# keep-starknet-strange/frieda

Hardware: AMD Instinct MI355X
Metric: M31 field-elems/s committed (NTT+FRI+Merkle) (higher is better)
Workload: dtype u32

## Files before the change

### frieda_amd/csrc/codec.hip

```cpp
#include <hip/hip_runtime.h>

#include <cstdlib>

#include "kernels.h"

namespace frieda {
namespace k {

namespace {

__device__ __forceinline__ uint32_t load_dword_guarded(const uint8_t* in, size_t len, size_t d) {
    size_t b = d * 4;
    if (b + 4 <= len) return *reinterpret_cast<const uint32_t*>(in + b);
    uint32_t v = 0;
    for (int i = 0; i < 4; i++)
        if (b + i < len) v |= (uint32_t)in[b + i] << (8 * i);
    return v;
}

template <int O>
__device__ __forceinline__ uint4 extract4(const uint32_t (&w)[5]) {
    uint32_t f[4];
#pragma unroll
    for (int j = 0; j < 4; j++) {
        const int pos = O + 30 * j, q = pos >> 5, r = pos & 31;
        uint64_t pair = ((uint64_t)w[q + 1] << 32) | w[q];
        f[j] = (uint32_t)(pair >> r) & 0x3fffffffu;
    }
    return make_uint4(f[0], f[1], f[2], f[3]);
}

template <int T>
__global__ __launch_bounds__(256) void unpack30_aligned_kernel(const uint8_t* __restrict__ in, size_t len,
                                                               uint32_t* __restrict__ out, size_t n_quads, size_t in_bstride,
                                                               size_t out_bstride) {
    in += blockIdx.y * in_bstride;
    out = reinterpret_cast<uint32_t*>(reinterpret_cast<char*>(out) + blockIdx.y * out_bstride);
    constexpr uint32_t DW = 960u * T;
    __shared__ __attribute__((aligned(16))) uint32_t stage[DW + 4];
    const size_t d_base = (size_t)blockIdx.x * DW;
    if ((reinterpret_cast<uintptr_t>(in) & 15) == 0 && (d_base + DW + 4) * 4 <= len) {
        const uint4* src = reinterpret_cast<const uint4*>(in + 4 * d_base);
#pragma unroll
        for (uint32_t u = threadIdx.x; u < 240u * T; u += 256) reinterpret_cast<uint4*>(stage)[u] = src[u];
        if (threadIdx.x < 4) stage[DW + threadIdx.x] = reinterpret_cast<const uint32_t*>(in)[d_base + DW + threadIdx.x];
    } else {
        for (uint32_t i = threadIdx.x; i < DW + 4; i += 256) stage[i] = load_dword_guarded(in, len, d_base + i);
    }
    __syncthreads();
#pragma unroll
    for (int i = 0; i < T; i++) {
        const uint32_t local = (uint32_t)i * 256u + threadIdx.x;
        const size_t t = (size_t)blockIdx.x * (256u * T) + local;
        if (t >= n_quads) return;
        const uint32_t byte0 = 15u * local;
        const uint32_t d0 = byte0 >> 2;
        uint32_t w[5];
#pragma unroll
        for (int j = 0; j < 5; j++) w[j] = stage[d0 + j];
        uint4 v;
        switch (byte0 & 3) {
            case 0: v = extract4<0>(w); break;
            case 1: v = extract4<8>(w); break;
            case 2: v = extract4<16>(w); break;
            default: v = extract4<24>(w); break;
        }
        reinterpret_cast<uint4*>(out)[t] = v;
    }
}

__global__ __launch_bounds__(256) void unpack30_bytes_kernel(const uint8_t* __restrict__ in, size_t len,
                                                             uint32_t* __restrict__ out, size_t n_out, size_t in_bstride,
                                                             size_t out_bstride) {
    in += blockIdx.y * in_bstride;
    out = reinterpret_cast<uint32_t*>(reinterpret_cast<char*>(out) + blockIdx.y * out_bstride);
    size_t kf = (size_t)blockIdx.x * blockDim.x + threadIdx.x;
    if (kf >= n_out) return;
    size_t bit0 = 30 * kf, byte0 = bit0 >> 3;
    uint32_t sh = (uint32_t)(bit0 & 7);
    uint64_t acc = 0;
    for (int i = 0; i < 5; i++)
        if (byte0 + i < len) acc |= (uint64_t)in[byte0 + i] << (8 * i);
    out[kf] = (uint32_t)(acc >> sh) & 0x3fffffffu;
}

}

void unpack30(const Launch& L, const uint8_t* d_bytes, size_t len, uint32_t* d_out, size_t n_out, size_t src_bstride) {
    if (n_out == 0) return;
    hipStream_t s = L.stream;
    Scope scope(L, "unpack30", (double)len + 4.0 * (double)n_out);
    bool aligned = ((reinterpret_cast<uintptr_t>(d_bytes) & 3) == 0) && ((reinterpret_cast<uintptr_t>(d_out) & 15) == 0) &&
                   (n_out % 4 == 0) && (src_bstride % 4 == 0) && (L.bstride % 16 == 0);
    if (aligned) {
        size_t quads = n_out / 4;
        const int tiles = (int)L.tune->unpack_tiles;
        const int T = quads >= 8192 ? tiles : 1;
        dim3 grid((unsigned)((quads + 256 * (size_t)T - 1) / (256 * (size_t)T)), L.batch);
        if (T == 8)
            unpack30_aligned_kernel<8><<<grid, 256, 0, s>>>(d_bytes, len, d_out, quads, src_bstride, L.bstride);
        else if (T == 4)
            unpack30_aligned_kernel<4><<<grid, 256, 0, s>>>(d_bytes, len, d_out, quads, src_bstride, L.bstride);
        else if (T == 2)
            unpack30_aligned_kernel<2><<<grid, 256, 0, s>>>(d_bytes, len, d_out, quads, src_bstride, L.bstride);
        else
            unpack30_aligned_kernel<1><<<grid, 256, 0, s>>>(d_bytes, len, d_out, quads, src_bstride, L.bstride);
    } else {
        dim3 grid((unsigned)((n_out + 255) / 256), L.batch);
        unpack30_bytes_kernel<<<grid, 256, 0, s>>>(d_bytes, len, d_out, n_out, src_bstride, L.bstride);
    }
}

}
}
```

### frieda_amd/csrc/context.cpp

```cpp
#include <cstring>
#include <cstdlib>
#include <string.h>

#include <cstdio>

#include <algorithm>
#include <mutex>

#include "host.h"

extern char** environ;

namespace frieda {

static constexpr uint32_t IDX_MASK = 0x7fffffffu;

CPoint point_from_index(uint32_t index) {
    static const std::array<CPoint, 31> pow2 = [] {
        std::array<CPoint, 31> t{};
        CPoint cur{CIRCLE_GEN_X, CIRCLE_GEN_Y};
        for (auto& e : t) {
            e = cur;
            cur = cp_double(cur);
        }
        return t;
    }();
    CPoint res{1, 0};
    index &= IDX_MASK;
    for (uint32_t b = 0; index; b++, index >>= 1)
        if (index & 1u) res = cp_add(res, pow2[b]);
    return res;
}

Coset Coset::half_odds(uint32_t log_size) {
    Coset c;
    c.initial = 1u << (31 - (log_size + 2));
    c.step = log_size == 0 ? 0u : (1u << (31 - log_size));
    c.log_size = log_size;
    return c;
}
Coset Coset::doubled() const { return Coset{(initial * 2u) & IDX_MASK, (step * 2u) & IDX_MASK, log_size - 1}; }
uint32_t Coset::index_at(uint32_t i) const { return (initial + (uint32_t)((uint64_t)step * i)) & IDX_MASK; }
CPoint Coset::at(uint32_t i) const { return point_from_index(index_at(i)); }

Coset line_coset(uint32_t n, uint32_t m) {
    Coset c = Coset::half_odds(n - 1);
    while (c.log_size > m) c = c.doubled();
    return c;
}

CodecShape codec_shape(size_t len) {
    CodecShape s;
    s.n_felts = (8 * len + 29) / 30;
    uint32_t e = 2;
    while (((size_t)1 << e) < s.n_felts) e++;
    s.n_padded = (size_t)1 << e;
    s.log_size = e - 2;
    return s;
}

struct KernelTimerImpl {
    struct Span {
        const char* name;
        double alg_bytes;
        hipEvent_t start, stop;
    };
    std::vector<Span> spans;
    std::vector<hipEvent_t> pool;
    size_t used = 0;
    hipEvent_t next() {
        if (used == pool.size()) {
            hipEvent_t e;
            (void)hipEventCreate(&e);
            pool.push_back(e);
        }
        return pool[used++];
    }
    ~KernelTimerImpl() {
        for (auto e : pool) (void)hipEventDestroy(e);
    }
};

namespace k {
void timer_begin(KernelTimer* t, hipStream_t s, const char* name, double alg_bytes) {
    auto* ti = reinterpret_cast<KernelTimerImpl*>(t);
    KernelTimerImpl::Span sp{name, alg_bytes, ti->next(), ti->next()};
    (void)hipEventRecord(sp.start, s);
    ti->spans.push_back(sp);
}
void timer_end(KernelTimer* t, hipStream_t s) {
    auto* ti = reinterpret_cast<KernelTimerImpl*>(t);
    (void)hipEventRecord(ti->spans.back().stop, s);
}
}

k::Launch Ctx::launch() const {
    k::Launch l{stream, reinterpret_cast<k::KernelTimer*>(timer)};
    l.tune = &tuning;
    return l;
}

namespace k {
namespace {
struct KnobDesc {
    const char* name;
    long lo, hi;
    bool (*set)(Tuning&, long);
};
const KnobDesc KNOBS[] = {
    {"FRIEDA_T5_WIDE_LOG", 16, 24, [](Tuning& t, long v) { t.t5_wide_log = (uint32_t)v; return true; }},
    {"FRIEDA_T5_REG3_LOG", 0, 30, [](Tuning& t, long v) { t.t5_reg3_log = (uint32_t)v; return true; }},
    {"FRIEDA_T9_MAX_LOG", 8, 19, [](Tuning& t, long v) { t.t9_max_log = (uint32_t)v; return true; }},
    {"FRIEDA_TOP_MAX_LOG", 9, 11, [](Tuning& t, long v) { t.top_max_log = (uint32_t)v; return true; }},
    {"FRIEDA_NTT_CPW", 1, 4, [](Tuning& t, long v) {
         if (v == 4 && !t.lds_opt_in_ok) return false;
         t.ntt_cpw = (uint32_t)v;
         return true;
     }},
    {"FRIEDA_NTT_CPW_SMALL", 1, 4, [](Tuning& t, long v) { t.ntt_cpw_small = (uint32_t)v; return true; }},
    {"FRIEDA_NTT_REP", 0, 2, [](Tuning& t, long v) { t.ntt_rep = (uint32_t)v; return true; }},
    {"FRIEDA_NTT_NO_CP", 0, 1, [](Tuning& t, long v) { t.ntt_no_cp = v != 0; return true; }},
    {"FRIEDA_NTT_NO_PAD8", 0, 1, [](Tuning& t, long v) { t.ntt_no_pad8 = v != 0; return true; }},
    {"FRIEDA_NTT_TREE_REG_ONLY", 0, 1, [](Tuning& t, long v) { t.ntt_tree_reg_only = v != 0; return true; }},
    {"FRIEDA_NO_ENCODE_TREE_FUSION", 0, 1, [](Tuning& t, long v) { t.no_encode_tree_fusion = v != 0; return true; }},
    {"FRIEDA_ENCODE_TREE_FUSION_PROVE", 0, 1, [](Tuning& t, long v) { t.encode_tree_fusion_prove = v != 0; return true; }},
    {"FRIEDA_NO_SMALL_FUSED", 0, 1, [](Tuning& t, long v) { t.no_small_fused = v != 0; return true; }},
    {"FRIEDA_UNPACK_TILES", 1, 8, [](Tuning& t, long v) {
         if (v != 1 && v != 2 && v != 4 && v != 8) return false;
         t.unpack_tiles = (uint32_t)v;
         return true;
     }},
    {"FRIEDA_INTT_GENERIC", 0, 1, [](Tuning& t, long v) { t.intt_generic = v != 0; return true; }},
    {"FRIEDA_ERASURE_TREE_MIN_LOG", 6, 32, [](Tuning& t, long v) { t.erasure_tree_min_log = (uint32_t)v; return true; }},
    {"FRIEDA_TAIL_RUN_LOG", 4, 11, [](Tuning& t, long v) { t.tail_run_log = (uint32_t)v; return true; }},
    {"FRIEDA_HOST_DECOMMIT", 0, 1, [](Tuning& t, long v) { t.host_decommit = v != 0; return true; }},
    {"FRIEDA_GATHER_COPY", 0, 1, [](Tuning& t, long v) { t.gather_copy = v != 0; return true; }},
    {"FRIEDA_VERIFY_DEVICE_MIN", 0, 2147483648L, [](Tuning& t, long v) { t.verify_device_min = (uint32_t)v; return true; }},
    {"FRIEDA_OPEN_SMALL_MAX", 0, 512, [](Tuning& t, long v) { t.open_small_max = (uint32_t)v; return true; }},
    {"FRIEDA_TREE_SKIP_LOG", 10, 40, [](Tuning& t, long v) { t.tree_skip_log = (uint32_t)v; return true; }},
    {"FRIEDA_TREE_SKIP_LONE_LOG", 10, 40, [](Tuning& t, long v) { t.tree_skip_lone_log = (uint32_t)v; return true; }},
    {"FRIEDA_SEEDS_FOLD_GROUP", 0, 64, [](Tuning& t, long v) { t.seeds_fold_group = (uint32_t)v; return true; }},
    {"FRIEDA_TP_MIN_WGS", 0, 1 << 30, [](Tuning& t, long v) { t.tp_min_wgs = (uint32_t)v; return true; }},
    {"FRIEDA_GRIND_ITERS", 0, 64, [](Tuning& t, long v) { t.grind_iters = (uint32_t)v; return true; }},
    {"FRIEDA_BATCH_BUDGET_MB", 0, 262144, [](Tuning& t, long v) { t.batch_budget_mb = (uint32_t)v; return true; }},
    {"FRIEDA_BATCH_CALLS_PER_CTX", 1, 64, [](Tuning& t, long v) { t.batch_calls_per_ctx = (uint32_t)v; return true; }},
};
}

bool tuning_set(Tuning& t, const char* name, long value) {
    if (!name) return false;
    for (const KnobDesc& k : KNOBS) {
        if (strcmp(k.name, name) == 0) {
            if (value < k.lo || value > k.hi) return false;
            return k.set(t, value);
        }
    }
    return false;
}

static const char* const PROCESS_VARS[] = {"FRIEDA_HIP_LIB", "FRIEDA_RCCL_PATH", "FRIEDA_MULTI_FORCE_RCCL", "FRIEDA_MULTI_NO_PREFETCH",
                                           "FRIEDA_MULTI_NO_NUMA_PIN", "FRIEDA_BENCH_FORCE_DIST", "FRIEDA_BENCH_CPU_THREADS", "FRIEDA_TEST_"};
static void warn_unknown_env_once() {
    static std::once_flag once;
    std::call_once(once, [] {
        for (char** e = ::environ; e && *e; e++) {
            if (strncmp(*e, "FRIEDA_", 7) != 0) continue;
            const char* eq = strchr(*e, '=');
            const size_t len = eq ? (size_t)(eq - *e) : strlen(*e);
            bool known = false;
            for (const KnobDesc& k : KNOBS) known = known || (strlen(k.name) == len && strncmp(k.name, *e, len) == 0);
            for (const char* pv : PROCESS_VARS) known = known || strncmp(pv, *e, strlen(pv)) == 0;
            if (!known) fprintf(stderr, "libfrieda_hip: note: environment variable %.*s is not an option of this library (ignored)\n", (int)len, *e);
        }
    });
}

Tuning tuning_from_env() {
    Tuning t;
    warn_unknown_env_once();
    for (const KnobDesc& k : KNOBS) {
        const char* e = getenv(k.name);
        if (!e) continue;
        char* end = nullptr;
        long v = strtol(e, &end, 10);
        if (end == e) v = 1;
        (void)tuning_set(t, k.name, v);
    }
    return t;
}

const Tuning& tuning_defaults() {
    static const Tuning d;
    return d;
}
}

int Ctx::set_kernel_timing(bool enabled) {
    if (enabled && !timer) timer = new KernelTimerImpl();
    if (!enabled && timer) {
        (void)hipStreamSynchronize(stream);
        delete timer;
        timer = nullptr;
    }
    return FRIEDA_OK;
}

std::string Ctx::kernel_timing_report(bool reset) {
    std::string out = "{\"kernels\": [";
    if (timer) {
        (void)hipStreamSynchronize(stream);
        struct Agg {
            const char* name;
            size_t launches;
            double ms, bytes;
        };
        std::vector<Agg> agg;
        for (auto& sp : timer->spans) {
            float ms = 0.f;
            if (hipEventElapsedTime(&ms, sp.start, sp.stop) != hipSuccess) continue;
            Agg* a = nullptr;
            for (auto& x : agg)
                if (strcmp(x.name, sp.name) == 0) a = &x;
            if (!a) {
                agg.push_back(Agg{sp.name, 0, 0.0, 0.0});
                a = &agg.back();
            }
            a->launches++;
            a->ms += ms;
            a->bytes += sp.alg_bytes;
        }
        bool first = true;
        for (auto& a : agg) {
            char buf[256];
            snprintf(buf, sizeof buf, "%s{\"name\": \"%s\", \"launches\": %zu, \"total_ms\": %.6f, \"alg_bytes\": %.1f}", first ? "" : ", ",
                     a.name, a.launches, a.ms, a.bytes);
            out += buf;
            first = false;
        }
        if (reset) {
            timer->spans.clear();
            timer->used = 0;
        }
    }
    out += "]}";
    return out;
}

int Ctx::fail(int code, const std::string& what) {
    err = what;
    return code;
}
int Ctx::hip_fail(hipError_t e, const char* what) {
    err = std::string(what) + ": " + hipGetErrorString(e);
    return FRIEDA_ERR_HIP;
}

int Ctx::ensure_arena(size_t bytes) {
    if (tuning.test_arena_limit && bytes > tuning.test_arena_limit) {
        err = "workspace of " + std::to_string(bytes) + " B refused by the test limit";
        return FRIEDA_ERR_NOMEM;
    }
    if (bytes <= arena_bytes) return FRIEDA_OK;
    if (arena) {
        FR_HIP(this, hipStreamSynchronize(stream));
        FR_HIP(this, hipFree(arena));
        arena = nullptr;
        arena_bytes = 0;
    }
    size_t want = (bytes + ((size_t)1 << 20) - 1) & ~(((size_t)1 << 20) - 1);
    hipError_t e = hipMalloc((void**)&arena, want);
    if (e != hipSuccess) {
        err = std::string("hipMalloc(workspace ") + std::to_string(want) + " B): " + hipGetErrorString(e);
        return FRIEDA_ERR_NOMEM;
    }
    arena_bytes = want;
    return FRIEDA_OK;
}

void Ctx::drop_twiddles() {
    for (auto& kv : twiddles) {
        if (kv.second.d_tw) (void)hipFree(kv.second.d_tw);
        if (kv.second.d_itw) (void)hipFree(kv.second.d_itw);
        if (kv.second.d_scratch) (void)hipFree(kv.second.d_scratch);
    }
    twiddles.clear();
}

int Ctx::get_twiddles(uint32_t n, TwiddleSet& out) {
    auto it = twiddles.find(n);
    if (it != twiddles.end() && cache_twiddles) {
        out = it->second;
        return FRIEDA_OK;
    }
    TwiddleSet ts;
    if (it != twiddles.end()) {
        ts = it->second;
    } else {
        size_t bytes = sizeof(uint32_t) << (n - 1);
        hipError_t e = hipMalloc((void**)&ts.d_tw, bytes);
        if (e == hipSuccess) e = hipMalloc((void**)&ts.d_itw, bytes);
        if (e == hipSuccess) e = hipMalloc((void**)&ts.d_scratch, 8192);
        if (e != hipSuccess) {
            if (ts.d_tw) (void)hipFree(ts.d_tw);
            if (ts.d_itw) (void)hipFree(ts.d_itw);
            err = std::string("hipMalloc(twiddles, 2 x ") + std::to_string(bytes) + " B): " + hipGetErrorString(e);
            return FRIEDA_ERR_NOMEM;
        }
        twiddles[n] = ts;
    }
    Coset h = Coset::half_odds(n - 1);
    k::TwiddleSeeds seeds;
    memset(&seeds, 0, sizeof seeds);
    seeds.p0 = point_from_index(h.initial);
    if (n >= 3) {
        CPoint sp = point_from_index(h.step);
        for (uint32_t b = 0; b + 2 < n; b++) {
            seeds.step[b] = sp;
            sp = cp_double(sp);
        }
    }
    ts.ds.init_x = seeds.p0.x;
    ts.ds.init_y = seeds.p0.y;
    ts.ds.inv_init_x = m31_inv(seeds.p0.x);
    ts.ds.inv_init_y = m31_inv(seeds.p0.y);
    k::gen_twiddles(launch(), n, seeds, ts.d_tw, ts.d_itw, ts.d_scratch);
    if (const hipError_t e = hipGetLastError(); e != hipSuccess) {
        (void)hipStreamSynchronize(stream);
        (void)hipFree(ts.d_tw);
        (void)hipFree(ts.d_itw);
        (void)hipFree(ts.d_scratch);
        twiddles.erase(n);
        return hip_fail(e, "gen_twiddles");
    }
    twiddles[n] = ts;
    out = ts;
    return FRIEDA_OK;
}

Ctx::~Ctx() {
    (void)hipSetDevice(device);
    if (stream) (void)hipStreamSynchronize(stream);
    drop_twiddles();
    delete timer;
    if (arena) (void)hipFree(arena);
    if (pinned) (void)hipHostFree(pinned);
    if (pinned_in) (void)hipHostFree(pinned_in);
    if (own_stream && stream) (void)hipStreamDestroy(stream);
}

}
```

### frieda_amd/csrc/kernels.h

```cpp
#pragma once
#include <hip/hip_runtime.h>
#include <stddef.h>
#include <stdint.h>

#include "field.h"

namespace frieda {
namespace k {

inline size_t tw_level_offset(uint32_t n, uint32_t lv) { return ((size_t)1 << (n - 1)) - ((size_t)1 << (n - 1 - lv)); }
__device__ __forceinline__ size_t tw_level_offset_dev(uint32_t n, uint32_t lv) {
    return ((size_t)1 << (n - 1)) - ((size_t)1 << (n - 1 - lv));
}

struct KernelTimer;
struct Tuning {
    uint32_t t5_wide_log = 18;
    uint32_t t5_reg3_log = 0;
    uint32_t t9_max_log = 17;
    uint32_t top_max_log = 9;
    uint32_t ntt_cpw = 4;
    uint32_t ntt_cpw_small = 1;
    uint32_t ntt_rep = 2;
    bool ntt_no_pad8 = false;
    bool ntt_no_cp = false;
    bool ntt_tree_reg_only = false;
    bool no_encode_tree_fusion = false;
    bool encode_tree_fusion_prove = false;
    bool no_small_fused = false;
    uint32_t unpack_tiles = 4;
    bool intt_generic = false;
    uint32_t erasure_tree_min_log = 15;
    uint32_t tail_run_log = 9;
    bool host_decommit = false;
    bool gather_copy = false;
    uint32_t verify_device_min = 1;
    uint32_t open_small_max = 512;
    uint32_t test_grind_first_log = 0;
    uint32_t batch_budget_mb = 0;
    uint32_t tree_skip_log = 18;
    uint32_t tree_skip_lone_log = 23;
    uint32_t tp_min_wgs = 768;
    uint32_t grind_iters = 0;
    uint32_t seeds_fold_group = 0;
    uint32_t batch_calls_per_ctx = 1;
    uint64_t device_mem_bytes = 0;
    bool lds_opt_in_ok = true;
    uint64_t test_arena_limit = 0;
};
inline uint32_t tree_skip_threshold(const Tuning& t, uint32_t batch) {
    return batch >= 2 ? t.tree_skip_log : (t.tree_skip_lone_log > t.tree_skip_log ? t.tree_skip_lone_log : t.tree_skip_log);
}
Tuning tuning_from_env();
bool tuning_set(Tuning& t, const char* name, long value);
const Tuning& tuning_defaults();

struct Launch {
    hipStream_t stream;
    KernelTimer* timer;
    uint32_t batch = 1;
    size_t bstride = 0;
    const Tuning* tune = &tuning_defaults();
};
void timer_begin(KernelTimer* t, hipStream_t s, const char* name, double alg_bytes);
void timer_end(KernelTimer* t, hipStream_t s);
struct Scope {
    const Launch& l;
    Scope(const Launch& l_, const char* name, double alg_bytes) : l(l_) {
        if (l.timer) timer_begin(l.timer, l.stream, name, alg_bytes * l.batch);
    }
    ~Scope() {
        if (l.timer) timer_end(l.timer, l.stream);
    }
};

struct DomainScalars {
    uint32_t init_x, init_y;
    uint32_t inv_init_x, inv_init_y;
};

void unpack30(const Launch& L, const uint8_t* d_bytes, size_t len, uint32_t* d_out, size_t n_out, size_t src_bstride = 0);

int blake2s_ceiling(hipStream_t s, uint32_t* d_scratch, double* leaf_per_s, double* node_per_s, double* clock = nullptr);
size_t blake2s_ceiling_scratch_bytes();

void bit_reverse_columns(const Launch& L, uint32_t* d_cols, size_t stride, uint32_t ncols, uint32_t log_size);

struct TwiddleSeeds {
    CPoint p0;
    CPoint step[32];
};
void gen_twiddles(const Launch& L, uint32_t n, const TwiddleSeeds& seeds, uint32_t* d_tw, uint32_t* d_itw, void* d_scratch8k);

void circle_evaluate(const Launch& L_, const uint32_t* d_coef, size_t coef_stride, uint32_t ncols, uint32_t L, uint32_t n,
                     const uint32_t* d_tw, DomainScalars ds, uint32_t* d_out, size_t out_stride);
void circle_evaluate_prefix(const Launch& L_, const uint32_t* d_coef, size_t coef_stride, uint32_t ncols, uint32_t L, uint32_t n, uint32_t out_log,
                            const uint32_t* d_tw, DomainScalars ds, uint32_t* d_out, size_t out_stride);

struct EncodeTreeSink {
    uint8_t* layers;
    uint8_t* last_out;
};
constexpr uint32_t ENCODE_TREE_LEVELS = 7;
hipError_t ntt_opt_in_dynamic_lds();
struct EncodeFoldSink {
    const uint32_t* itw;
    uint32_t alpha0[4], alpha1[4];
    bool accumulate;
    uint32_t* line1;
    uint32_t* line2;
};
bool circle_evaluate_fold2(const Launch& L_, const uint32_t* d_coef, size_t coef_stride, uint32_t L, uint32_t n, const uint32_t* d_tw,
                           DomainScalars ds, uint32_t* d_out, size_t out_stride, const EncodeFoldSink& fs, hipError_t* err);
uint32_t circle_evaluate_into_tree(const Launch& L_, const uint32_t* d_coef, size_t coef_stride, uint32_t ncols, uint32_t L, uint32_t n,
                               const uint32_t* d_tw, DomainScalars ds, uint32_t* d_out, size_t out_stride, const EncodeTreeSink* sink);

void circle_interpolate_block(const Launch& L_, const uint32_t* d_block, size_t in_stride, uint32_t ncols, uint32_t L, uint32_t n,
                              uint32_t block, const uint32_t* d_itw, DomainScalars ds, uint32_t* d_coef, size_t out_stride);
void cells_combine(const Launch& L_, const uint32_t* d_w, const uint32_t* d_vinv, uint32_t R, uint32_t ncols, uint32_t m, uint32_t* d_coef,
                   size_t coef_stride, size_t vinv_pitch = 0);
size_t cells_inverse_scratch_bytes(uint32_t R);
uint32_t* cells_inverse_index_buffer(uint8_t* d_scratch, uint32_t R);
void cells_matrix_inverse_device(const Launch& L_, const uint32_t* d_cell_index, uint32_t R, uint32_t j_bits, uint32_t m, uint32_t n,
                                 const uint32_t* d_tw, uint8_t* d_scratch, const uint32_t** d_vinv_out, size_t* pitch_out,
                                 const uint32_t** d_state_out);
void pack30(const Launch& L_, const uint32_t* d_felts, size_t n_felts, uint8_t* d_out, size_t len);

struct ErasureDomain {
    CPoint init;
    CPoint step_pow[32];
    uint32_t n;
};
void erasure_points(const Launch& L_, const ErasureDomain& g, const uint32_t* d_pos, uint32_t count, uint32_t* d_px, uint32_t* d_py);
void erasure_lines(const Launch& L_, const ErasureDomain& g, const uint32_t* d_pos, uint32_t n_lines, uint32_t* d_la, uint32_t* d_lb,
                   uint32_t* d_lc);
size_t erasure_zpart_chunks(uint32_t count, uint32_t n_lines);
void erasure_zeval(const Launch& L_, const uint32_t* d_px, const uint32_t* d_py, uint32_t count, const uint32_t* d_la, const uint32_t* d_lb,
                   const uint32_t* d_lc, uint32_t n_lines, bool own, uint32_t* d_zpart, uint32_t* d_z);
void erasure_known_weights(const Launch& L_, const uint32_t* d_px, const uint32_t* d_py, uint32_t count, uint32_t n, uint32_t* d_z);
void erasure_cellconst(const Launch& L_, const ErasureDomain& g, const uint32_t* d_cell_pos, uint32_t n_cells, uint32_t m, uint32_t* d_kc);
void erasure_zeval_cells(const Launch& L_, const uint32_t* d_px, uint32_t count, uint32_t m, const uint32_t* d_kc, uint32_t n_cells, bool own,
                         uint32_t* d_zpart, uint32_t* d_z);
void erasure_known_weights_cells(const Launch& L_, const uint32_t* d_px, uint32_t count, uint32_t n, uint32_t m, uint32_t* d_z);
size_t erasure_sample_lists_chunks(uint32_t n_cells);
hipError_t erasure_sample_lists(const Launch& L_, const uint32_t* d_idx, uint32_t n_cells, uint32_t domain_cells, uint32_t ncols, uint32_t log_cell,
                          uint32_t* d_owner, uint32_t* d_chunk_sum, uint32_t* d_chunk_off, uint32_t* d_first_cell, uint32_t* d_first_row,
                          uint32_t* d_state, uint32_t* d_pos, uint32_t* d_src);
void erasure_cell_firsts(const Launch& L_, const uint32_t* d_pos, uint32_t n_cells, uint32_t log_cell, uint32_t* d_out);
void erasure_lines32(const Launch& L_, const uint32_t* d_px128, const uint32_t* d_py128, const uint32_t* d_la, const uint32_t* d_lb, const uint32_t* d_lc,
                     uint32_t n_lines, uint32_t nodes, uint32_t* d_out);
void erasure_pairmul(const Launch& L_, const uint32_t* d_ext, uint32_t n_nodes, uint32_t size, uint32_t* d_out);
void erasure_ze(const Launch& L_, const ErasureDomain& g1, const uint32_t* d_zs, uint32_t count, uint32_t n, uint32_t* d_ze);
void erasure_fold_prefix(const Launch& L_, const uint32_t* d_in, size_t in_stride, uint32_t ncols, uint32_t out_log, uint32_t cnt, const uint32_t* d_tw,
                         uint32_t dom_n, uint32_t* d_out, size_t out_stride);
void erasure_gather(const Launch& L_, const uint32_t* d_src, const uint32_t* d_pos, uint32_t count, uint32_t* d_out);
void erasure_scatter(const Launch& L_, const uint32_t* d_cells, const uint32_t* d_src, const uint32_t* d_pos, const uint32_t* d_z, uint32_t count,
                     uint32_t ncols, uint32_t log_cell, uint32_t* d_w, size_t w_stride);
void erasure_divide(const Launch& L_, const uint32_t* d_ev, size_t ev_stride, const uint32_t* d_z, const uint32_t* d_px, uint32_t count, uint32_t ncols,
                    uint32_t n, uint32_t* d_block, size_t block_stride);
void erasure_check(const Launch& L_, const uint32_t* d_cells, const uint32_t* d_src, const uint32_t* d_pos, uint32_t count, uint32_t ncols,
                   uint32_t log_cell, const uint32_t* d_ev, size_t ev_stride, uint32_t* d_mismatch);

void merkle_leaf4(const Launch& L, const uint32_t* c0, const uint32_t* c1, const uint32_t* c2, const uint32_t* c3, size_t n,
                  uint8_t* d_out);
void merkle_node(const Launch& L, const uint8_t* d_prev, size_t n, uint8_t* d_out);
void merkle_layer_generic(const Launch& L, const uint8_t* d_prev, const uint32_t* const* d_col_ptrs, uint32_t ncols, size_t n,
                          uint8_t* d_out);
void merkle_tree4(const Launch& L, const uint32_t* c0, const uint32_t* c1, const uint32_t* c2, const uint32_t* c3, uint32_t m,
                  uint8_t* d_layers);
size_t merkle_root_scratch_bytes(uint32_t m);
void merkle_root4(const Launch& L, const uint32_t* c0, const uint32_t* c1, const uint32_t* c2, const uint32_t* c3, uint32_t m,
                  uint8_t* d_scratch, uint8_t* d_root);
inline size_t merkle_layer_offset(uint32_t log_size, uint32_t layer_log) {
    return ((size_t)64 << log_size) - ((size_t)64 << layer_log);
}

}
struct DevTranscript;
namespace k {
void tree_first_layer(const Launch& L, const uint32_t* cols, size_t stride, uint32_t m, uint8_t* d_layers, DevTranscript* tr,
                      const DevTranscript* tr_init = nullptr, size_t tr_init_pitch = 0);
bool small_domain_shape(const Tuning& tn, uint32_t Lc, uint32_t n);
bool small_first_opt_in();
void small_encode_and_first_tree(const Launch& L, const uint8_t* d_data, size_t len, size_t data_stride, uint32_t Lc, uint32_t n,
                                 const uint32_t* d_tw, DomainScalars ds, uint32_t* d_eval, size_t eval_stride, uint8_t* d_layers,
                                 uint8_t* d_scratch, uint8_t* d_root, DevTranscript* tr, const DevTranscript* tr_init, size_t tr_init_pitch);
void encode_and_first_tree(const Launch& L, const uint32_t* d_coef, size_t coef_stride, uint32_t Lc, uint32_t n, const uint32_t* d_tw,
                           DomainScalars ds, uint32_t* d_eval, size_t eval_stride, uint8_t* d_layers, uint8_t* d_scratch, uint8_t* d_root,
                           DevTranscript* tr, const DevTranscript* tr_init = nullptr, size_t tr_init_pitch = 0);
void fold_and_tree(const Launch& L, bool circle, const uint32_t* src, size_t src_stride, uint32_t src_log, uint32_t n,
                   const uint32_t* d_itw, DomainScalars ds, uint32_t* dst_vals, uint8_t* d_layers, DevTranscript* tr, bool shared_src = false,
                   uint32_t seeds_group = 0);
void channel_after_shared_root(const Launch& L, const uint8_t* d_root, DevTranscript* tr, const DevTranscript* tr_init, size_t tr_init_pitch);
constexpr uint32_t TAIL_LOG = 11;
void fri_tail(const Launch& L, const uint32_t* src, size_t src_stride, uint32_t src_log, bool src_is_circle, uint32_t n,
              const uint32_t* d_itw, DomainScalars ds, uint32_t last_log, uint32_t last, uint32_t n_layers, uint32_t* const* vals,
              uint8_t* const* trees, DevTranscript* tr, uint32_t* d_gnext = nullptr, bool shared_src = false);
constexpr uint32_t GRIND_NEXT_STRIDE = 32;
void grind_dev(const Launch& L, DevTranscript* tr, uint32_t* d_next, uint32_t pow_bits, uint64_t base, uint64_t count,
               bool next_zeroed = false);

constexpr uint32_t DECOMMIT_MAX_QUERIES = 1024;
constexpr uint32_t DECOMMIT_MAX_LOG_DOMAIN = 27;
constexpr uint32_t DECOMMIT_MAX_LAYERS = 40;
constexpr uint32_t DECOMMIT_HEADER_BYTES = 256;
enum DecommitStatus : uint32_t { DECOMMIT_OK = 0, DECOMMIT_NO_NONCE = 1, DECOMMIT_OVERFLOW = 2 };
struct DecommitArgs {
    const DevTranscript* tr;
    uint32_t n, n_layers, n_queries;
    size_t bstride;
    uint8_t* out;
    size_t out_stride;
    size_t words_off, hashes_off;
    uint32_t max_words, max_hashes;
    const uint32_t* vals[DECOMMIT_MAX_LAYERS];
    const uint8_t* trees[DECOMMIT_MAX_LAYERS];
    uint32_t skip_log;
    uint32_t first_shared, skip_log0;
};
void decommit(const Launch& L, const DecommitArgs& a, uint32_t wgs_per_blob);

constexpr uint32_t VERIFY_MAX_QUERIES = DECOMMIT_MAX_QUERIES;
enum VerifyStatus : uint32_t { VERIFY_REJECTED = 0, VERIFY_ACCEPTED = 1, VERIFY_INVARIANT = 2, VERIFY_WRONG_COMMITMENT = 3 };
struct VerifyHeader {
    uint32_t off_words;
    uint32_t n, n_inner, n_queries, pow_bits;
    uint32_t has_seed, seed_lo, seed_hi, nonce_lo, nonce_hi;
    uint32_t n_last, n_evals;
    uint32_t off_last, off_evals;
    uint32_t pad_[2];
};
struct VerifyArgs {
    const uint32_t* img;
    uint32_t* out;
    uint32_t q_cap;
};
size_t verify_many_lds_bytes(uint32_t q_cap);
hipError_t verify_many_init(const CPoint (&gen_pow2)[31]);
void verify_many(const Launch& L, const VerifyArgs& a, uint32_t n_proofs);

constexpr uint32_t OPEN_BAD_WORD = 0xFFFFFFFFu;
constexpr uint32_t OPEN_BAD_COUNT = 0xFFFFFFFFu;
constexpr uint32_t OPEN_MAX_LOG = 28;
constexpr uint32_t OPEN_SMALL_MAX_LIMIT = 512;
void gather_rows(const Launch& L, const uint32_t* d_cols, size_t stride, uint32_t ncols, const uint64_t* d_idx, size_t n, uint32_t* d_out);
void gather_hashes(const Launch& L, const uint8_t* d_layer, size_t layer_len, const uint64_t* d_idx, size_t n, uint8_t* d_out);
struct OpenTree {
    const uint8_t* layers[OPEN_MAX_LOG + 1];
};
struct DecommitOpen {
    OpenTree tree;
    uint32_t log_size, n, ncols;
    const uint32_t* pos;
    const uint32_t* cols;
    size_t stride;
    uint32_t* values;
    uint4* hashes;
    uint64_t max_hashes;
    uint32_t* count;
};
uint64_t decommit_hash_bound(uint64_t n_pos, uint32_t log_size);
bool decommit_small_route(uint32_t n_pos, uint32_t log_size, uint32_t small_max);
size_t decommit_scratch_bytes(uint32_t n_pos, uint32_t log_size);
void merkle_decommit(const Launch& L, const DecommitOpen& a, uint32_t small_max, void* d_scratch);

struct EvalFactors {
    QM31 f[32];
};
void circle_extend(const Launch& L, const uint32_t* d_coef, uint32_t ncols, uint32_t log_coef, uint32_t log_size, uint32_t* d_out);
size_t eval_at_point_scratch_bytes(uint32_t ncols, uint32_t log_coef);
const uint32_t* circle_eval_at_point(const Launch& L, const uint32_t* d_coef, uint32_t ncols, uint32_t log_coef, const EvalFactors& f, uint32_t* d_scratch);
size_t decompose_scratch_bytes(uint32_t log_size);
void fri_decompose(const Launch& L, const uint32_t* d_eval, uint32_t log_size, uint32_t* d_g, uint32_t* d_scratch);

struct Alpha {
    uint32_t v[4];
};
void fold_circle_into_line(const Launch& L, uint32_t* d_dst, size_t dst_stride, const uint32_t* d_src, size_t src_stride,
                           uint32_t n, const uint32_t* d_itw, DomainScalars ds, Alpha alpha);
void fold_line(const Launch& L, const uint32_t* d_src, size_t src_stride, uint32_t m, uint32_t n, const uint32_t* d_itw,
               DomainScalars ds, Alpha alpha, uint32_t* d_dst, size_t dst_stride);
constexpr uint64_t GATHER_ALT = (uint64_t)1 << 63;
void gather(const Launch& L, const uint32_t* d_base, const uint64_t* d_word_idx, size_t n_words, uint32_t* d_out_words,
            const uint64_t* d_hash_idx, size_t n_hashes, uint8_t* d_out_hashes, const uint32_t* d_alt_words = nullptr,
            const uint8_t* d_alt_hashes = nullptr);
void grind_scan(const Launch& L, const uint32_t digest[8], uint32_t pow_bits, uint64_t base, uint64_t count,
                unsigned long long* d_result);

}
}
```

### frieda_amd/csrc/ntt.hip

```cpp
#include <hip/hip_runtime.h>

#include <type_traits>

#include <cstdlib>

#include "clock_stamps.h"
#include "kernels.h"
#include "tree_dev.h"

namespace frieda {
namespace k {

namespace {
using namespace treedev;

constexpr int NTT_THREADS = 256;
constexpr uint32_t TILE_LOG = 12;
#ifndef FRIEDA_NTT_PAD32
constexpr uint32_t TILE_WORDS = (1u << TILE_LOG) + (1u << (TILE_LOG - 4));
#else
constexpr uint32_t TILE_WORDS = (1u << TILE_LOG) + (1u << (TILE_LOG - 5));
#endif
constexpr uint32_t MAX_COLS_PER_WG = 4;
constexpr uint32_t MID_LOG_W = 4;

#ifndef FRIEDA_NTT_PAD32
__device__ __forceinline__ uint32_t pad(uint32_t e) { return e + (e >> 4); }
#else
__device__ __forceinline__ uint32_t pad(uint32_t e) { return e + (e >> 5); }
#endif
__device__ __forceinline__ uint32_t stage_group_base(uint32_t g, uint32_t lo) {
#ifdef FRIEDA_NTT_PAD32
    if (lo == 4) {
        const uint32_t t = g >> 4;
        const uint32_t h = (t & ~3u) | ((t & 1u) << 1) | ((t >> 1) & 1u);
        return (h << 8) | (g & 15u);
    }
#endif
    return ((g >> lo) << (lo + 4)) | (g & ((1u << lo) - 1));
}

#ifndef FRIEDA_NTT_IDLE
#define FRIEDA_NTT_IDLE 0x200
#endif
#ifndef FRIEDA_NTT_GROUP
#define FRIEDA_NTT_GROUP 8
#endif
#ifndef FRIEDA_NTT_GROUP_FUSED
#define FRIEDA_NTT_GROUP_FUSED 4
#endif
#ifndef FRIEDA_NTT_OUTER_PRIO
#define FRIEDA_NTT_OUTER_PRIO 3
#endif
__device__ __forceinline__ void ntt_enter() {
    if constexpr (FRIEDA_NTT_OUTER_PRIO != 0 && ((FRIEDA_NTT_IDLE >> 8) & 3) != 0) __builtin_amdgcn_s_setprio(FRIEDA_NTT_OUTER_PRIO);
}
template <int N, int G, int SET = -1>
__device__ __forceinline__ void ntt_pin(uint32_t (&a)[G]) {
    static_assert(N >= 0 && N <= 5 && (G == 4 || G == 8) && SET >= -1 && SET <= 3, "idle states 0 .. 5, groups of 4 or 8, priorities 0 .. 3");
#define FR_PIN_OPS4 "+v"(a[0]), "+v"(a[1]), "+v"(a[2]), "+v"(a[3])
#define FR_PIN_OPS8 "+v"(a[0]), "+v"(a[1]), "+v"(a[2]), "+v"(a[3]), "+v"(a[4]), "+v"(a[5]), "+v"(a[6]), "+v"(a[7])
#define FR_PIN_N(PRE, ...)                                               \
    do {                                                                 \
        if constexpr (N <= 1) asm volatile(PRE : __VA_ARGS__);           \
        if constexpr (N == 2) asm volatile(PRE "s_nop 0" : __VA_ARGS__); \
        if constexpr (N == 3) asm volatile(PRE "s_nop 1" : __VA_ARGS__); \
        if constexpr (N == 4) asm volatile(PRE "s_nop 2" : __VA_ARGS__); \
        if constexpr (N == 5) asm volatile(PRE "s_nop 3" : __VA_ARGS__); \
    } while (0)
#define FR_PIN_SET(...)                                                   \
    do {                                                                  \
        if constexpr (SET < 0 && N >= 1) FR_PIN_N("", __VA_ARGS__);       \
        if constexpr (SET == 0) FR_PIN_N("s_setprio 0\n\t", __VA_ARGS__); \
        if constexpr (SET == 1) FR_PIN_N("s_setprio 1\n\t", __VA_ARGS__); \
        if constexpr (SET == 2) FR_PIN_N("s_setprio 2\n\t", __VA_ARGS__); \
        if constexpr (SET == 3) FR_PIN_N("s_setprio 3\n\t", __VA_ARGS__); \
    } while (0)
    if constexpr (G == 8)
        FR_PIN_SET(FR_PIN_OPS8);
    else
        FR_PIN_SET(FR_PIN_OPS4);
#undef FR_PIN_SET
#undef FR_PIN_N
#undef FR_PIN_OPS4
#undef FR_PIN_OPS8
}
template <int IDLE, int Q, int G, int K0, typename TW>
__device__ __forceinline__ void radix16_group(uint32_t (&x)[16], const TW& tw) {
    constexpr int bit = 3 - Q, NA = (IDLE >> 4) & 15, NB = IDLE & 15, PRIO = (IDLE >> 8) & 3;
    constexpr int LO = PRIO ? 0 : -1, HI = PRIO ? PRIO : -1;
    constexpr int LOW[4][8] = {{0, 1, 2, 3, 4, 5, 6, 7}, {0, 1, 2, 3, 8, 9, 10, 11}, {0, 1, 4, 5, 8, 9, 12, 13}, {0, 2, 4, 6, 8, 10, 12, 14}};
    uint32_t hi[G], lo[G], d[G];
#pragma unroll
    for (int k = 0; k < G; k++) {
        const int r = LOW[Q][K0 + k];
        const uint64_t p = (uint64_t)x[r | (1 << bit)] * tw[(1 << Q) - 1 + (r >> (bit + 1))];
        hi[k] = (uint32_t)(p >> 32);
        lo[k] = (uint32_t)p;
    }
    ntt_pin<NA, G, LO>(hi);
#pragma unroll
    for (int k = 0; k < G; k++) {
        lo[k] >>= 1;
        lo[k] += hi[k];
        hi[k] = lo[k] - P31;
    }
    ntt_pin<NB, G, HI>(hi);
#pragma unroll
    for (int k = 0; k < G; k++) lo[k] = umin32(lo[k], hi[k]);
    ntt_pin<NA, G, LO>(lo);
#pragma unroll
    for (int k = 0; k < G; k++) {
        const int r = LOW[Q][K0 + k];
        const uint32_t w = x[r];
        d[k] = w - lo[k];
        x[r] = w + lo[k];
        hi[k] = d[k] + P31;
        lo[k] = x[r] - P31;
    }
    ntt_pin<NB, G, HI>(lo);
#pragma unroll
    for (int k = 0; k < G; k++) {
        const int r = LOW[Q][K0 + k];
        x[r] = umin32(x[r], lo[k]);
        x[r | (1 << bit)] = umin32(d[k], hi[k]);
    }
}
template <int IDLE, int Q, int G, typename TW>
__device__ __forceinline__ void radix16_layer(uint32_t (&x)[16], const TW& tw) {
    radix16_group<IDLE, Q, G, 0>(x, tw);
    if constexpr (G == 4) radix16_group<IDLE, Q, G, 4>(x, tw);
}
template <int G = FRIEDA_NTT_GROUP, typename TW>
__device__ __forceinline__ void radix16_stage(uint32_t (&x)[16], const TW& tw) {
    if constexpr (FRIEDA_NTT_IDLE != 0) {
        radix16_layer<FRIEDA_NTT_IDLE, 0, G>(x, tw);
        radix16_layer<FRIEDA_NTT_IDLE, 1, G>(x, tw);
        radix16_layer<FRIEDA_NTT_IDLE, 2, G>(x, tw);
        radix16_layer<FRIEDA_NTT_IDLE, 3, G>(x, tw);
        if constexpr (((FRIEDA_NTT_IDLE >> 8) & 3) != 0) {
            if constexpr (FRIEDA_NTT_OUTER_PRIO == 0) asm volatile("s_setprio 0" : "+v"(x[0]), "+v"(x[8]), "+v"(x[7]), "+v"(x[15]));
            if constexpr (FRIEDA_NTT_OUTER_PRIO == 1) asm volatile("s_setprio 1" : "+v"(x[0]), "+v"(x[8]), "+v"(x[7]), "+v"(x[15]));
            if constexpr (FRIEDA_NTT_OUTER_PRIO == 2) asm volatile("s_setprio 2" : "+v"(x[0]), "+v"(x[8]), "+v"(x[7]), "+v"(x[15]));
            if constexpr (FRIEDA_NTT_OUTER_PRIO == 3) asm volatile("s_setprio 3" : "+v"(x[0]), "+v"(x[8]), "+v"(x[7]), "+v"(x[15]));
        }
    } else {
#pragma unroll
        for (int q = 0; q < 4; q++) {
            const int bit = 3 - q;
#pragma unroll
            for (int r = 0; r < 16; r++) {
                if (r & (1 << bit)) continue;
                const int u = r >> (bit + 1);
                const uint32_t t = m31_mul(x[r | (1 << bit)], tw[(1 << q) - 1 + u] >> 1);
                const uint32_t v = x[r];
                x[r] = m31_add(v, t);
                x[r | (1 << bit)] = m31_sub(v, t);
            }
        }
    }
}

__device__ __forceinline__ uint32_t circle_twiddle(const uint32_t* __restrict__ tw, uint32_t n, uint32_t h, uint32_t init_y) {
    if (n < 3) return (h & 1u) ? m31_neg(init_y) : init_y;
    uint32_t j = h >> 2, r = h & 3u;
    uint32_t v = tw[2 * j + (r < 2 ? 1 : 0)];
    return (r == 1 || r == 2) ? m31_neg(v) : v;
}

struct NttArgs {
    const uint32_t* in;
    size_t in_stride;
    uint32_t in_mask;
    uint32_t in_limit;
    uint32_t* out;
    size_t out_stride;
    const uint32_t* tw;
    uint32_t n, i_hi, i_lo, log_w, init_y;
    uint32_t ncols;
    uint32_t n_stages;
    uint32_t stage_r[3];
    size_t bstride_w;
    uint32_t rep_log;
};

template <int R, int LO>
__device__ __forceinline__ void run_stage(uint32_t* lds, const NttArgs& a, uint32_t tb, uint32_t lo_rt, uint32_t hblk) {
    constexpr int E = 1 << R;
    const uint32_t lo = LO >= 0 ? (uint32_t)LO : lo_rt;
    const uint32_t n_groups = 1u << (tb - R);
    for (uint32_t g = threadIdx.x; g < n_groups; g += NTT_THREADS) {
        const uint32_t base = ((g >> lo) << (lo + R)) | (g & ((1u << lo) - 1));
        const uint32_t pbase = pad(base);
        uint32_t twd[E - 1];
#pragma unroll
        for (int q = 0; q < R; q++) {
            const uint32_t b = lo + R - 1 - q;
            const uint32_t i = a.i_lo + b - a.log_w;
            const uint32_t hbase = (hblk << (a.i_hi - i)) | (base >> (b + 1));
            if (i >= 1) {
                const uint32_t* lvl = a.tw + tw_level_offset_dev(a.n, i - 1) + hbase;
#pragma unroll
                for (int u = 0; u < (1 << q); u++) twd[(1 << q) - 1 + u] = lvl[u];
            } else {
#pragma unroll
                for (int u = 0; u < (1 << q); u++) twd[(1 << q) - 1 + u] = circle_twiddle(a.tw, a.n, hbase + (uint32_t)u, a.init_y);
            }
        }
        for (uint32_t c = 0; c < a.ncols; c++) {
            uint32_t* col = lds + c * TILE_WORDS + pbase;
            uint32_t x[E];
#pragma unroll
            for (int r = 0; r < E; r++) x[r] = col[pad((uint32_t)r << lo)];
#pragma unroll
            for (int q = 0; q < R; q++) {
                const int bit = R - 1 - q;
#pragma unroll
                for (int r = 0; r < E; r++) {
                    if (r & (1 << bit)) continue;
                    const int u = r >> (bit + 1);
                    const uint32_t t = m31_mul(x[r | (1 << bit)], twd[(1 << q) - 1 + u]);
                    const uint32_t v = x[r];
                    x[r] = m31_add(v, t);
                    x[r | (1 << bit)] = m31_sub(v, t);
                }
            }
#pragma unroll
            for (int r = 0; r < E; r++) col[pad((uint32_t)r << lo)] = x[r];
        }
    }
}

__global__ __launch_bounds__(NTT_THREADS) void ntt_tile_kernel(NttArgs a) {
    extern __shared__ uint32_t lds[];
    const uint32_t t = a.i_hi - a.i_lo + 1;
    const uint32_t tb = t + a.log_w;
    const uint32_t tile = 1u << tb;
    const uint32_t wmask = (1u << a.log_w) - 1;
    const uint32_t nwb_log = a.i_lo - a.log_w;
    const uint32_t wblk = blockIdx.x & ((1u << nwb_log) - 1);
    const uint32_t hblk = blockIdx.x >> nwb_log;
    const uint32_t gbase = (hblk << (a.i_hi + 1)) | (wblk << a.log_w);
    const size_t col0 = (size_t)blockIdx.y * a.ncols;
    const uint32_t* in = a.in + col0 * a.in_stride + blockIdx.z * a.bstride_w;
    uint32_t* out = a.out + col0 * a.out_stride + blockIdx.z * a.bstride_w;
    const bool vec = tb >= 2 && (a.log_w == 0 || a.log_w >= 2) && ((a.in_stride | a.out_stride) & 3) == 0 &&
                     ((reinterpret_cast<uintptr_t>(a.in) | reinterpret_cast<uintptr_t>(a.out)) & 15) == 0 && (a.in_mask & 3u) == 3u &&
                     (a.bstride_w & 3) == 0;

    for (uint32_t c = 0; c < a.ncols; c++) {
        uint32_t* col = lds + c * TILE_WORDS;
        const uint32_t* src = in + c * a.in_stride;
        if (vec) {
            for (uint32_t e = 4 * threadIdx.x; e < tile; e += 4 * NTT_THREADS) {
                uint32_t g = gbase | ((e >> a.log_w) << a.i_lo) | (e & wmask);
                uint4 v = *reinterpret_cast<const uint4*>(src + (g & a.in_mask));
                uint32_t p = pad(e);
                col[p] = v.x;
                col[p + 1] = v.y;
                col[p + 2] = v.z;
                col[p + 3] = v.w;
            }
        } else {
            for (uint32_t e = threadIdx.x; e < tile; e += NTT_THREADS) {
                uint32_t g = gbase | ((e >> a.log_w) << a.i_lo) | (e & wmask);
                col[pad(e)] = src[g & a.in_mask];
            }
        }
    }
    __syncthreads();

    uint32_t top = tb;
    for (uint32_t s = 0; s < a.n_stages; s++) {
        const uint32_t r = a.stage_r[s], lo = top - r;
        if (r == 4 && lo == 8)
            run_stage<4, 8>(lds, a, tb, lo, hblk);
        else if (r == 4 && lo == 4)
            run_stage<4, 4>(lds, a, tb, lo, hblk);
        else if (r == 4 && lo == 0)
            run_stage<4, 0>(lds, a, tb, lo, hblk);
        else if (r == 4)
            run_stage<4, -1>(lds, a, tb, lo, hblk);
        else if (r == 3)
            run_stage<3, -1>(lds, a, tb, lo, hblk);
        else if (r == 2)
            run_stage<2, -1>(lds, a, tb, lo, hblk);
        else
            run_stage<1, -1>(lds, a, tb, lo, hblk);
        top = lo;
        __syncthreads();
    }

    for (uint32_t c = 0; c < a.ncols; c++) {
        const uint32_t* col = lds + c * TILE_WORDS;
        uint32_t* dst = out + c * a.out_stride;
        if (vec) {
            for (uint32_t e = 4 * threadIdx.x; e < tile; e += 4 * NTT_THREADS) {
                uint32_t g = gbase | ((e >> a.log_w) << a.i_lo) | (e & wmask);
                uint32_t p = pad(e);
                *reinterpret_cast<uint4*>(dst + g) = make_uint4(col[p], col[p + 1], col[p + 2], col[p + 3]);
            }
        } else {
            for (uint32_t e = threadIdx.x; e < tile; e += NTT_THREADS) {
                uint32_t g = gbase | ((e >> a.log_w) << a.i_lo) | (e & wmask);
                dst[g] = col[pad(e)];
            }
        }
    }
}

template <int NS, int LOG_W>
__global__ __launch_bounds__(NTT_THREADS) void ntt_tile12_kernel(NttArgs a) {
    ntt_enter();
    __shared__ uint32_t lds[TILE_WORDS];
    const uint32_t g = threadIdx.x;
    const uint32_t nwb_log = a.i_lo - LOG_W;
    const uint32_t wblk = blockIdx.x & ((1u << nwb_log) - 1);
    const uint32_t hblk = blockIdx.x >> nwb_log;
    const uint32_t gbase = (hblk << (a.i_hi + 1)) | (wblk << LOG_W);
    constexpr uint32_t wmask = (1u << LOG_W) - 1;
    const size_t col0 = (size_t)blockIdx.y * a.ncols;
    const uint32_t* in = a.in + col0 * a.in_stride + blockIdx.z * a.bstride_w;
    uint32_t* out = a.out + col0 * a.out_stride + blockIdx.z * a.bstride_w;

    uint32_t pbase[NS];
    uint32_t twd[NS][15];
#pragma unroll
    for (int s = 0; s < NS; s++) {
        const uint32_t lo = 8 - 4 * s;
        const uint32_t base = stage_group_base(g, lo);
        pbase[s] = pad(base);
#pragma unroll
        for (int q = 0; q < 4; q++) {
            const uint32_t b = lo + 3 - q;
            const uint32_t i = a.i_lo + b - LOG_W;
            const uint32_t hbase = (hblk << (a.i_hi - i)) | (base >> (b + 1));
            if (LOG_W == 0 && s == NS - 1 && q == 3) {
#pragma unroll
                for (int u = 0; u < 8; u++) twd[s][7 + u] = 2u * circle_twiddle(a.tw, a.n, hbase + (uint32_t)u, a.init_y);
            } else {
                const uint32_t* lvl = a.tw + tw_level_offset_dev(a.n, i - 1) + hbase;
#pragma unroll
                for (int u = 0; u < (1 << q); u++) {
                    uint32_t v = lvl[u];
                    if (s == 0) v = (uint32_t)__builtin_amdgcn_readfirstlane((int)v);
                    twd[s][(1 << q) - 1 + u] = 2u * v;
                }
            }
        }
    }

    auto piece_e = [&](int kk) { return 4u * g + 1024u * (uint32_t)kk; };
    auto global_of = [&](uint32_t e) { return gbase | ((e >> LOG_W) << a.i_lo) | (e & wmask); };

    auto load4 = [&](const uint32_t* src, uint32_t gidx) {
        const uint32_t idx = gidx & a.in_mask;
        return idx < a.in_limit ? *reinterpret_cast<const uint4*>(src + idx) : make_uint4(0u, 0u, 0u, 0u);
    };
    uint4 pre[4];
#pragma unroll
    for (int kk = 0; kk < 4; kk++) pre[kk] = load4(in, global_of(piece_e(kk)));

    for (uint32_t c = 0; c < a.ncols; c++) {
#pragma unroll
        for (int kk = 0; kk < 4; kk++) {
            const uint32_t p = pad(piece_e(kk));
            lds[p] = pre[kk].x;
            lds[p + 1] = pre[kk].y;
            lds[p + 2] = pre[kk].z;
            lds[p + 3] = pre[kk].w;
        }
        __syncthreads();
        if (c + 1 < a.ncols) {
            const uint32_t* src = in + (size_t)(c + 1) * a.in_stride;
#pragma unroll
            for (int kk = 0; kk < 4; kk++) pre[kk] = load4(src, global_of(piece_e(kk)));
        }
        uint32_t x[16];
#pragma unroll
        for (int s = 0; s < NS; s++) {
            const uint32_t lo = 8 - 4 * s;
            uint32_t* col = lds + pbase[s];
#pragma unroll
            for (int r = 0; r < 16; r++) x[r] = col[pad((uint32_t)r << lo)];
            radix16_stage(x, twd[s]);
            if (s + 1 < NS || LOG_W != 0) {
#pragma unroll
                for (int r = 0; r < 16; r++) col[pad((uint32_t)r << lo)] = x[r];
            }
            if (LOG_W == 0 && NS == 3 && s == 1)
                __builtin_amdgcn_wave_barrier();
            else
                __syncthreads();
        }
        uint32_t* dst = out + (size_t)c * a.out_stride;
        if (LOG_W == 0) {
            uint4* o = reinterpret_cast<uint4*>(dst + gbase + 16u * g);
            o[0] = make_uint4(x[0], x[1], x[2], x[3]);
            o[1] = make_uint4(x[4], x[5], x[6], x[7]);
            o[2] = make_uint4(x[8], x[9], x[10], x[11]);
            o[3] = make_uint4(x[12], x[13], x[14], x[15]);
        } else {
#pragma unroll
            for (int kk = 0; kk < 4; kk++) {
                const uint32_t e = piece_e(kk), p = pad(e);
                *reinterpret_cast<uint4*>(dst + global_of(e)) = make_uint4(lds[p], lds[p + 1], lds[p + 2], lds[p + 3]);
            }
            __syncthreads();
        }
    }
}

template <int COLS>
__global__ __launch_bounds__(NTT_THREADS) void ntt_tile12_rep_kernel(NttArgs a) {
    ntt_enter();
    constexpr int NS = 2;
    constexpr uint32_t LOG_W = MID_LOG_W;
    __shared__ uint32_t lds[TILE_WORDS];
    const uint32_t g = threadIdx.x;
    const uint32_t nwb_log = a.i_lo - LOG_W;
    const uint32_t wblk = blockIdx.x & ((1u << nwb_log) - 1);
    const uint32_t hblk0 = (blockIdx.x >> nwb_log) << a.rep_log;
    constexpr uint32_t wmask = (1u << LOG_W) - 1;
    const size_t col0 = (size_t)blockIdx.y * COLS;
    const uint32_t* in = a.in + col0 * a.in_stride + blockIdx.z * a.bstride_w;
    uint32_t* out = a.out + col0 * a.out_stride + blockIdx.z * a.bstride_w;

    auto piece_e = [&](int kk) { return 4u * g + 1024u * (uint32_t)kk; };
    auto low_of = [&](uint32_t e) { return (wblk << LOG_W) | ((e >> LOG_W) << a.i_lo) | (e & wmask); };

    uint4 src[COLS][4];
#pragma unroll
    for (int c = 0; c < COLS; c++) {
#pragma unroll
        for (int kk = 0; kk < 4; kk++) {
            const uint32_t idx = low_of(piece_e(kk)) & a.in_mask;
            src[c][kk] = idx < a.in_limit ? *reinterpret_cast<const uint4*>(in + (size_t)c * a.in_stride + idx) : make_uint4(0u, 0u, 0u, 0u);
        }
    }
    uint32_t pbase[NS];
#pragma unroll
    for (int s = 0; s < NS; s++) {
        const uint32_t lo = 8 - 4 * s;
        pbase[s] = pad(stage_group_base(g, lo));
    }

#pragma unroll 1
    for (uint32_t h = 0; h < (1u << a.rep_log); h++) {
        const uint32_t hblk = hblk0 + h;
        const uint32_t gbase = hblk << (a.i_hi + 1);
        uint32_t twd[NS][15];
#pragma unroll
        for (int s = 0; s < NS; s++) {
            const uint32_t lo = 8 - 4 * s;
            const uint32_t base = stage_group_base(g, lo);
#pragma unroll
            for (int q = 0; q < 4; q++) {
                const uint32_t b = lo + 3 - q;
                const uint32_t i = a.i_lo + b - LOG_W;
                const uint32_t hbase = (hblk << (a.i_hi - i)) | (base >> (b + 1));
                const uint32_t* lvl = a.tw + tw_level_offset_dev(a.n, i - 1) + hbase;
#pragma unroll
                for (int u = 0; u < (1 << q); u++) {
                    uint32_t v = lvl[u];
                    if (s == 0) v = (uint32_t)__builtin_amdgcn_readfirstlane((int)v);
                    twd[s][(1 << q) - 1 + u] = 2u * v;
                }
            }
        }
#pragma unroll
        for (int c = 0; c < COLS; c++) {
#pragma unroll
            for (int kk = 0; kk < 4; kk++) {
                const uint32_t p = pad(piece_e(kk));
                lds[p] = src[c][kk].x;
                lds[p + 1] = src[c][kk].y;
                lds[p + 2] = src[c][kk].z;
                lds[p + 3] = src[c][kk].w;
            }
            __syncthreads();
            uint32_t x[16];
#pragma unroll
            for (int s = 0; s < NS; s++) {
                const uint32_t lo = 8 - 4 * s;
                uint32_t* col = lds + pbase[s];
#pragma unroll
                for (int r = 0; r < 16; r++) x[r] = col[pad((uint32_t)r << lo)];
                radix16_stage(x, twd[s]);
#pragma unroll
                for (int r = 0; r < 16; r++) col[pad((uint32_t)r << lo)] = x[r];
                __syncthreads();
            }
            uint32_t* dst = out + (size_t)c * a.out_stride + gbase;
#pragma unroll
            for (int kk = 0; kk < 4; kk++) {
                const uint32_t e = piece_e(kk), p = pad(e);
                *reinterpret_cast<uint4*>(dst + low_of(e)) = make_uint4(lds[p], lds[p + 1], lds[p + 2], lds[p + 3]);
            }
            __syncthreads();
        }
    }
}

struct NttTreeArgs {
    NttArgs a;
    uint8_t* layers;
    uint8_t* last_out;
    size_t bstride;
};


template <bool STORE_ALL>
__device__ __forceinline__ void last_pass_four_columns(const NttArgs& a, uint32_t* lds, uint32_t g, uint32_t hblk, const uint32_t* in, uint32_t* out,
                                                       uint32_t (&v)[4][16]) {
    const uint32_t gbase = hblk << TILE_LOG;
    uint32_t pbase[3];
    uint32_t twd[3][15];
#pragma unroll
    for (int s = 0; s < 3; s++) {
        const uint32_t lo = 8 - 4 * s;
        const uint32_t base = stage_group_base(g, lo);
        pbase[s] = pad(base);
#pragma unroll
        for (int q = 0; q < 4; q++) {
            const uint32_t b = lo + 3 - q;
            const uint32_t hbase = (hblk << (11 - b)) | (base >> (b + 1));
            if (s == 2 && q == 3) {
#pragma unroll
                for (int u = 0; u < 8; u++) twd[s][7 + u] = 2u * circle_twiddle(a.tw, a.n, hbase + (uint32_t)u, a.init_y);
            } else {
                const uint32_t* lvl = a.tw + tw_level_offset_dev(a.n, b - 1) + hbase;
#pragma unroll
                for (int u = 0; u < (1 << q); u++) {
                    uint32_t v = lvl[u];
                    if (s == 0) v = (uint32_t)__builtin_amdgcn_readfirstlane((int)v);
                    twd[s][(1 << q) - 1 + u] = 2u * v;
                }
            }
        }
    }
    auto piece_e = [&](int kk) { return 4u * g + 1024u * (uint32_t)kk; };

    uint4 pre[4];
#pragma unroll
    for (int kk = 0; kk < 4; kk++) pre[kk] = *reinterpret_cast<const uint4*>(in + ((gbase | piece_e(kk)) & a.in_mask));

#pragma unroll
    for (int c = 0; c < 4; c++) {
#pragma unroll
        for (int kk = 0; kk < 4; kk++) {
            const uint32_t p = pad(piece_e(kk));
            lds[p] = pre[kk].x;
            lds[p + 1] = pre[kk].y;
            lds[p + 2] = pre[kk].z;
            lds[p + 3] = pre[kk].w;
        }
        __syncthreads();
        if (c + 1 < 4) {
            const uint32_t* src = in + (size_t)(c + 1) * a.in_stride;
#pragma unroll
            for (int kk = 0; kk < 4; kk++) pre[kk] = *reinterpret_cast<const uint4*>(src + ((gbase | piece_e(kk)) & a.in_mask));
        }
#pragma unroll
        for (int s = 0; s < 3; s++) {
            const uint32_t lo = 8 - 4 * s;
            uint32_t* col = lds + pbase[s];
            uint32_t* x = v[c];
#pragma unroll
            for (int r = 0; r < 16; r++) x[r] = col[pad((uint32_t)r << lo)];
            radix16_stage<FRIEDA_NTT_GROUP_FUSED>(*reinterpret_cast<uint32_t(*)[16]>(x), twd[s]);
            if (s < 2) {
#pragma unroll
                for (int r = 0; r < 16; r++) col[pad((uint32_t)r << lo)] = x[r];
            }
            if (s == 1)
                __builtin_amdgcn_wave_barrier();
            else
                __syncthreads();
        }
        if (STORE_ALL) {
            uint4* o = reinterpret_cast<uint4*>(out + (size_t)c * a.out_stride + gbase + 16u * g);
            o[0] = make_uint4(v[c][0], v[c][1], v[c][2], v[c][3]);
            o[1] = make_uint4(v[c][4], v[c][5], v[c][6], v[c][7]);
            o[2] = make_uint4(v[c][8], v[c][9], v[c][10], v[c][11]);
            o[3] = make_uint4(v[c][12], v[c][13], v[c][14], v[c][15]);
        }
    }

}

FR_CLOCK_DECL(g_clock_ntt_last_tree)
template <bool STORE_ALL, bool REG_ONLY, bool TP>
__global__ __launch_bounds__(NTT_THREADS) void ntt_last_tree_kernel(NttTreeArgs A) {
    ntt_enter();
    __shared__ uint32_t lds[TILE_WORDS];
    __shared__ __attribute__((aligned(16))) uint32_t RC[8 * (256 + 4)];
    __shared__ __attribute__((aligned(16))) uint32_t RD[8 * (128 + 4)];
    const NttArgs& a = A.a;
    uint32_t g_tie = threadIdx.x;
    FR_CLOCK_BEGIN(g_tie)
    const uint32_t g = g_tie;
    const uint32_t hblk = blockIdx.x;
    const uint32_t gbase = hblk << TILE_LOG;
    const uint32_t* in = a.in + blockIdx.z * a.bstride_w;
    uint32_t* out = a.out + blockIdx.z * a.bstride_w;

    uint32_t v[4][16];
    last_pass_four_columns<STORE_ALL>(a, lds, g, hblk, in, out, v);

    const uint32_t m = a.n;
    uint8_t* layers = A.layers + blockIdx.z * A.bstride;
    uint8_t* out_b = STORE_ALL ? layers + layer_off(m, m - 1) : nullptr;
    uint8_t* out_c = STORE_ALL ? layers + layer_off(m, m - 2) : nullptr;
    uint8_t* out_d = STORE_ALL ? layers + layer_off(m, m - 3) : nullptr;
    uint8_t* out_e = STORE_ALL ? layers + layer_off(m, m - 4) : (REG_ONLY ? A.last_out + blockIdx.z * A.bstride : nullptr);
    const size_t leaf0 = (size_t)gbase + 16u * g;
    uint32_t hprev[8], hdprev[8];
#pragma unroll 1
    for (int it = 0; it < 4; it++) {
        const size_t l0 = leaf0 + 4u * (uint32_t)it;
        uint32_t hb[2][8];
        auto half_ab = [&](auto half_c) {
            constexpr int half = decltype(half_c)::value;
            uint32_t ha[2][8];
            leaf_hash<TP ? FRIEDA_B2_IDLE_NTT_LEAF : B2_LAT>(v[0][2 * half], v[1][2 * half], v[2][2 * half], v[3][2 * half], ha[0]);
            leaf_hash<TP ? FRIEDA_B2_IDLE_NTT_LEAF : B2_LAT>(v[0][2 * half + 1], v[1][2 * half + 1], v[2][2 * half + 1], v[3][2 * half + 1], ha[1]);
            uint32_t mm[16];
#pragma unroll
            for (int w = 0; w < 8; w++) mm[w] = ha[0][w], mm[8 + w] = ha[1][w];
            b2_merkle_block<TP ? FRIEDA_B2_IDLE_NTT_NODE : B2_LAT>(mm, hb[half]);
        };
        half_ab(std::integral_constant<int, 0>{});
        half_ab(std::integral_constant<int, 1>{});
        if (STORE_ALL) {
            store_hash(out_b, l0 >> 1, hb[0]);
            store_hash(out_b, (l0 >> 1) + 1, hb[1]);
        }
        uint32_t hc[8];
        {
            uint32_t mm[16];
#pragma unroll
            for (int w = 0; w < 8; w++) mm[w] = hb[0][w], mm[8 + w] = hb[1][w];
            b2_merkle_block<TP ? FRIEDA_B2_IDLE_NTT_NODE : B2_LAT>(mm, hc);
        }
        if (STORE_ALL) store_hash(out_c, l0 >> 2, hc);
        if ((it & 1) == 0) {
#pragma unroll
            for (int w = 0; w < 8; w++) hprev[w] = hc[w];
        } else {
            uint32_t hd[8], mm[16];
#pragma unroll
            for (int w = 0; w < 8; w++) mm[w] = hprev[w], mm[8 + w] = hc[w];
            b2_merkle_block<TP ? FRIEDA_B2_IDLE_NTT_NODE : B2_LAT>(mm, hd);
            if (STORE_ALL) store_hash(out_d, l0 >> 3, hd);
            if (it == 1) {
#pragma unroll
                for (int w = 0; w < 8; w++) hdprev[w] = hd[w];
            } else {
                uint32_t he[8];
#pragma unroll
                for (int w = 0; w < 8; w++) mm[w] = hdprev[w], mm[8 + w] = hd[w];
                b2_merkle_block<TP ? FRIEDA_B2_IDLE_NTT_NODE : B2_LAT>(mm, he);
                if (STORE_ALL || REG_ONLY) store_hash(out_e, l0 >> 4, he);
                if (!REG_ONLY) lds_put(RC, 256 + 4, g, he);
            }
        }
#pragma unroll
        for (int c = 0; c < 4; c++) {
#pragma unroll
            for (int r = 0; r < 12; r++) v[c][r] = v[c][r + 4];
        }
    }
    if (REG_ONLY) return;
    __syncthreads();
    const size_t wg_e = (size_t)gbase >> 4;
    if (g < 128) {
        uint32_t mm[16], h[8];
        lds_children(RC, 256 + 4, g, mm);
        b2_merkle_block<TP ? FRIEDA_B2_IDLE_NTT_NODE : B2_LAT>(mm, h);
        if (STORE_ALL) store_hash(layers + layer_off(m, m - 5), (wg_e >> 1) + g, h);
        lds_put(RD, 128 + 4, g, h);
    }
    __syncthreads();
    if (g < 64) {
        uint32_t mm[16], h[8];
        lds_children(RD, 128 + 4, g, mm);
        b2_merkle_block<TP ? FRIEDA_B2_IDLE_NTT_NODE : B2_LAT>(mm, h);
        uint8_t* dst = STORE_ALL ? layers + layer_off(m, m - 6) : A.last_out + blockIdx.z * A.bstride;
        store_hash(dst, (wg_e >> 2) + g, h);
        FR_CLOCK_END(g_clock_ntt_last_tree, h[0])
    }
}

__global__ void ntt_broadcast_kernel(const uint32_t* __restrict__ in, size_t in_stride, uint32_t* __restrict__ out,
                                     size_t out_stride, size_t n_out, size_t bstride_w) {
    size_t i = (size_t)blockIdx.x * blockDim.x + threadIdx.x;
    if (i < n_out) out[blockIdx.z * bstride_w + (size_t)blockIdx.y * out_stride + i] = in[blockIdx.z * bstride_w + (size_t)blockIdx.y * in_stride];
}

void set_stages(NttArgs& a, uint32_t t) {
    uint32_t ns = (t + 3) / 4;
    a.n_stages = ns;
    uint32_t left = t;
    for (uint32_t s = 0; s < ns; s++) {
        uint32_t r = (left + (ns - s) - 1) / (ns - s);
        a.stage_r[s] = r;
        left -= r;
    }
}

struct NttFoldArgs {
    NttArgs a;
    const uint32_t* itw;
    uint32_t inv_init_y;
    uint32_t alpha0[4], alpha1[4];
    uint32_t* line1;
    uint32_t* line2;
};

template <bool ACC>
__global__ __launch_bounds__(NTT_THREADS) void ntt_last_fold_kernel(NttFoldArgs A) {
    ntt_enter();
    __shared__ uint32_t lds[TILE_WORDS];
    const NttArgs& a = A.a;
    const uint32_t g = threadIdx.x, hblk = blockIdx.x;
    uint32_t v[4][16];
    last_pass_four_columns<true>(a, lds, g, hblk, a.in, a.out, v);
    const uint32_t n = a.n;
    const size_t e0 = ((size_t)hblk << TILE_LOG) + 16u * g;
    const QM31Mat am0 = qm_matrix({A.alpha0[0], A.alpha0[1], A.alpha0[2], A.alpha0[3]});
    const QM31Mat am1 = qm_matrix({A.alpha1[0], A.alpha1[1], A.alpha1[2], A.alpha1[3]});
    const uint4 t0 = *reinterpret_cast<const uint4*>(A.itw + (e0 >> 2));
    const uint32_t ix[2] = {t0.x, t0.z}, iy[2] = {t0.y, t0.w};
    const uint32_t il[4] = {t0.x, t0.y, t0.z, t0.w};
    const size_t s1 = (size_t)1 << (n - 1), s2 = (size_t)1 << (n - 2);
    QM31 l1[8];
#pragma unroll
    for (int k = 0; k < 8; k++) {
        const int pr = k >> 2, r = k & 3;
        const uint32_t it = r == 0 ? iy[pr] : (r == 1 ? m31_neg(iy[pr]) : (r == 2 ? m31_neg(ix[pr]) : ix[pr]));
        l1[k] = qm_fold_pair(QM31{v[0][2 * k], v[1][2 * k], v[2][2 * k], v[3][2 * k]},
                             QM31{v[0][2 * k + 1], v[1][2 * k + 1], v[2][2 * k + 1], v[3][2 * k + 1]}, it, am0);
    }
    uint32_t* d1 = A.line1 + (e0 >> 1);
    if (ACC) {
        const QM31 al = {A.alpha0[0], A.alpha0[1], A.alpha0[2], A.alpha0[3]};
        const QM31 asq = qm_mul(al, al);
        uint4 o[4][2];
#pragma unroll
        for (int c = 0; c < 4; c++) o[c][0] = reinterpret_cast<const uint4*>(d1 + c * s1)[0], o[c][1] = reinterpret_cast<const uint4*>(d1 + c * s1)[1];
#pragma unroll
        for (int k = 0; k < 8; k++) {
            auto w = [&](int c) { const uint4 q4 = o[c][k >> 2]; return (k & 3) == 0 ? q4.x : ((k & 3) == 1 ? q4.y : ((k & 3) == 2 ? q4.z : q4.w)); };
            l1[k] = qm_add(qm_mul(QM31{w(0), w(1), w(2), w(3)}, asq), l1[k]);
        }
    }
    {
        uint4* p0 = reinterpret_cast<uint4*>(d1);
        uint4* p1 = reinterpret_cast<uint4*>(d1 + s1);
        uint4* p2 = reinterpret_cast<uint4*>(d1 + 2 * s1);
        uint4* p3 = reinterpret_cast<uint4*>(d1 + 3 * s1);
        p0[0] = make_uint4(l1[0].a, l1[1].a, l1[2].a, l1[3].a), p0[1] = make_uint4(l1[4].a, l1[5].a, l1[6].a, l1[7].a);
        p1[0] = make_uint4(l1[0].b, l1[1].b, l1[2].b, l1[3].b), p1[1] = make_uint4(l1[4].b, l1[5].b, l1[6].b, l1[7].b);
        p2[0] = make_uint4(l1[0].c, l1[1].c, l1[2].c, l1[3].c), p2[1] = make_uint4(l1[4].c, l1[5].c, l1[6].c, l1[7].c);
        p3[0] = make_uint4(l1[0].d, l1[1].d, l1[2].d, l1[3].d), p3[1] = make_uint4(l1[4].d, l1[5].d, l1[6].d, l1[7].d);
    }
    QM31 l2[4];
#pragma unroll
    for (int k = 0; k < 4; k++) l2[k] = qm_fold_pair(l1[2 * k], l1[2 * k + 1], il[k], am1);
    uint32_t* d2 = A.line2 + (e0 >> 2);
    *reinterpret_cast<uint4*>(d2) = make_uint4(l2[0].a, l2[1].a, l2[2].a, l2[3].a);
    *reinterpret_cast<uint4*>(d2 + s2) = make_uint4(l2[0].b, l2[1].b, l2[2].b, l2[3].b);
    *reinterpret_cast<uint4*>(d2 + 2 * s2) = make_uint4(l2[0].c, l2[1].c, l2[2].c, l2[3].c);
    *reinterpret_cast<uint4*>(d2 + 3 * s2) = make_uint4(l2[0].d, l2[1].d, l2[2].d, l2[3].d);
}

constexpr int NTT_CP_THREADS = 1024;
template <bool ACC>
__global__ __launch_bounds__(NTT_CP_THREADS) void ntt_last_fold_cp_kernel(NttFoldArgs A) {
    ntt_enter();
    extern __shared__ uint32_t cp_lds[];
    const NttArgs& a = A.a;
    const uint32_t c = threadIdx.x >> 8, g = threadIdx.x & 255u, hblk = blockIdx.x;
    const uint32_t gbase = hblk << TILE_LOG;
    uint32_t* lds = cp_lds + c * TILE_WORDS;
    const uint32_t* in = a.in + (size_t)c * a.in_stride;
    uint4 pre[4];
#pragma unroll
    for (int kk = 0; kk < 4; kk++) pre[kk] = *reinterpret_cast<const uint4*>(in + ((gbase | (4u * g + 1024u * (uint32_t)kk)) & a.in_mask));
    uint32_t twd[3][15], pbase[3];
#pragma unroll
    for (int s = 0; s < 3; s++) {
        const uint32_t lo = 8 - 4 * s;
        const uint32_t base = stage_group_base(g, lo);
        pbase[s] = pad(base);
#pragma unroll
        for (int q = 0; q < 4; q++) {
            const uint32_t b = lo + 3 - q;
            const uint32_t hbase = (hblk << (11 - b)) | (base >> (b + 1));
            if (s == 2 && q == 3) {
#pragma unroll
                for (int u = 0; u < 8; u++) twd[s][7 + u] = 2u * circle_twiddle(a.tw, a.n, hbase + (uint32_t)u, a.init_y);
            } else {
                const uint32_t* lvl = a.tw + tw_level_offset_dev(a.n, b - 1) + hbase;
#pragma unroll
                for (int u = 0; u < (1 << q); u++) twd[s][(1 << q) - 1 + u] = 2u * lvl[u];
            }
        }
    }
#pragma unroll
    for (int kk = 0; kk < 4; kk++) {
        const uint32_t p = pad(4u * g + 1024u * (uint32_t)kk);
        lds[p] = pre[kk].x;
        lds[p + 1] = pre[kk].y;
        lds[p + 2] = pre[kk].z;
        lds[p + 3] = pre[kk].w;
    }
    __syncthreads();
    uint32_t x[16];
#pragma unroll
    for (int s = 0; s < 3; s++) {
        const uint32_t lo = 8 - 4 * s;
        uint32_t* col = lds + pbase[s];
#pragma unroll
        for (int r = 0; r < 16; r++) x[r] = col[pad((uint32_t)r << lo)];
        radix16_stage<FRIEDA_NTT_GROUP_FUSED>(x, twd[s]);
        if (s < 2) {
#pragma unroll
            for (int r = 0; r < 16; r++) col[pad((uint32_t)r << lo)] = x[r];
        }
        if (s == 1)
            __builtin_amdgcn_wave_barrier();
        else if (s == 0)
            __syncthreads();
    }
    {
        uint4* o = reinterpret_cast<uint4*>(a.out + (size_t)c * a.out_stride + gbase + 16u * g);
        o[0] = make_uint4(x[0], x[1], x[2], x[3]);
        o[1] = make_uint4(x[4], x[5], x[6], x[7]);
        o[2] = make_uint4(x[8], x[9], x[10], x[11]);
        o[3] = make_uint4(x[12], x[13], x[14], x[15]);
        uint32_t* mine = lds + pad(16u * g);
#pragma unroll
        for (int r = 0; r < 16; r++) mine[r] = x[r];
    }
    __syncthreads();
    const uint32_t T = threadIdx.x, n = a.n;
    const size_t e0 = (size_t)gbase + 4u * T;
    uint32_t v[4][4];
#pragma unroll
    for (int cc = 0; cc < 4; cc++) {
        const uint32_t* t4 = cp_lds + cc * TILE_WORDS + pad(4u * T);
#pragma unroll
        for (int k = 0; k < 4; k++) v[cc][k] = t4[k];
    }
    const QM31Mat am0 = qm_matrix({A.alpha0[0], A.alpha0[1], A.alpha0[2], A.alpha0[3]});
    const QM31Mat am1 = qm_matrix({A.alpha1[0], A.alpha1[1], A.alpha1[2], A.alpha1[3]});
    const size_t i0 = e0 >> 1;
    const uint2 xy = *reinterpret_cast<const uint2*>(A.itw + 2 * (i0 >> 2));
    const uint32_t it0 = (i0 & 2) ? m31_neg(xy.x) : xy.y, it1 = (i0 & 2) ? xy.x : m31_neg(xy.y);
    const uint32_t il = A.itw[e0 >> 2];
    QM31 l1[2];
    l1[0] = qm_fold_pair(QM31{v[0][0], v[1][0], v[2][0], v[3][0]}, QM31{v[0][1], v[1][1], v[2][1], v[3][1]}, it0, am0);
    l1[1] = qm_fold_pair(QM31{v[0][2], v[1][2], v[2][2], v[3][2]}, QM31{v[0][3], v[1][3], v[2][3], v[3][3]}, it1, am0);
    const size_t s1 = (size_t)1 << (n - 1), s2 = (size_t)1 << (n - 2);
    uint32_t* d1 = A.line1 + i0;
    if (ACC) {
        const QM31 al = {A.alpha0[0], A.alpha0[1], A.alpha0[2], A.alpha0[3]};
        const QM31 asq = qm_mul(al, al);
        uint2 o[4];
#pragma unroll
        for (int cc = 0; cc < 4; cc++) o[cc] = *reinterpret_cast<const uint2*>(d1 + cc * s1);
        l1[0] = qm_add(qm_mul(QM31{o[0].x, o[1].x, o[2].x, o[3].x}, asq), l1[0]);
        l1[1] = qm_add(qm_mul(QM31{o[0].y, o[1].y, o[2].y, o[3].y}, asq), l1[1]);
    }
    *reinterpret_cast<uint2*>(d1) = make_uint2(l1[0].a, l1[1].a);
    *reinterpret_cast<uint2*>(d1 + s1) = make_uint2(l1[0].b, l1[1].b);
    *reinterpret_cast<uint2*>(d1 + 2 * s1) = make_uint2(l1[0].c, l1[1].c);
    *reinterpret_cast<uint2*>(d1 + 3 * s1) = make_uint2(l1[0].d, l1[1].d);
    const QM31 l2 = qm_fold_pair(l1[0], l1[1], il, am1);
    uint32_t* d2 = A.line2 + (e0 >> 2);
    d2[0] = l2.a;
    d2[s2] = l2.b;
    d2[2 * s2] = l2.c;
    d2[3 * s2] = l2.d;
}

}

FR_CLOCK_READER(frieda_debug_clock_ntt_last_tree, g_clock_ntt_last_tree)

namespace {
uint32_t evaluate_plan(const Launch& L_, const uint32_t* d_coef, size_t coef_stride, uint32_t ncols, uint32_t L, uint32_t n, uint32_t out_log,
                       const uint32_t* d_tw, DomainScalars ds, uint32_t* d_out, size_t out_stride, const EncodeTreeSink* sink,
                       const EncodeFoldSink* fsink = nullptr);
}

void circle_evaluate(const Launch& L_, const uint32_t* d_coef, size_t coef_stride, uint32_t ncols, uint32_t L, uint32_t n,
                     const uint32_t* d_tw, DomainScalars ds, uint32_t* d_out, size_t out_stride) {
    (void)evaluate_plan(L_, d_coef, coef_stride, ncols, L, n, n, d_tw, ds, d_out, out_stride, nullptr);
}

void circle_evaluate_prefix(const Launch& L_, const uint32_t* d_coef, size_t coef_stride, uint32_t ncols, uint32_t L, uint32_t n, uint32_t out_log,
                            const uint32_t* d_tw, DomainScalars ds, uint32_t* d_out, size_t out_stride) {
    (void)evaluate_plan(L_, d_coef, coef_stride, ncols, L, n, out_log < L ? L : (out_log > n ? n : out_log), d_tw, ds, d_out, out_stride, nullptr);
}

uint32_t circle_evaluate_into_tree(const Launch& L_, const uint32_t* d_coef, size_t coef_stride, uint32_t ncols, uint32_t L, uint32_t n,
                               const uint32_t* d_tw, DomainScalars ds, uint32_t* d_out, size_t out_stride, const EncodeTreeSink* sink) {
    return evaluate_plan(L_, d_coef, coef_stride, ncols, L, n, n, d_tw, ds, d_out, out_stride, sink);
}

hipError_t ntt_opt_in_dynamic_lds() {
    const int bytes = (int)(MAX_COLS_PER_WG * TILE_WORDS * sizeof(uint32_t));
    hipError_t e = hipFuncSetAttribute(reinterpret_cast<const void*>(ntt_tile_kernel), hipFuncAttributeMaxDynamicSharedMemorySize, bytes);
    if (e != hipSuccess) return e;
    e = hipFuncSetAttribute(reinterpret_cast<const void*>(ntt_last_fold_cp_kernel<false>), hipFuncAttributeMaxDynamicSharedMemorySize, bytes);
    if (e != hipSuccess) return e;
    return hipFuncSetAttribute(reinterpret_cast<const void*>(ntt_last_fold_cp_kernel<true>), hipFuncAttributeMaxDynamicSharedMemorySize, bytes);
}

bool circle_evaluate_fold2(const Launch& L_, const uint32_t* d_coef, size_t coef_stride, uint32_t L, uint32_t n, const uint32_t* d_tw,
                           DomainScalars ds, uint32_t* d_out, size_t out_stride, const EncodeFoldSink& fs, hipError_t* err) {
    *err = hipSuccess;
    if (evaluate_plan(L_, d_coef, coef_stride, 4, L, n, n, d_tw, ds, d_out, out_stride, nullptr, &fs)) return true;
    if (!fs.accumulate) {
        *err = hipMemsetAsync(fs.line1, 0, sizeof(uint32_t) * ((size_t)4 << (n - 1)), L_.stream);
        if (*err != hipSuccess) return false;
    }
    fold_circle_into_line(L_, fs.line1, (size_t)1 << (n - 1), d_out, out_stride, n, fs.itw, ds, Alpha{{fs.alpha0[0], fs.alpha0[1], fs.alpha0[2], fs.alpha0[3]}});
    fold_line(L_, fs.line1, (size_t)1 << (n - 1), n - 1, n, fs.itw, ds, Alpha{{fs.alpha1[0], fs.alpha1[1], fs.alpha1[2], fs.alpha1[3]}}, fs.line2,
              (size_t)1 << (n - 2));
    return false;
}

namespace {
uint32_t evaluate_plan(const Launch& L_, const uint32_t* d_coef, size_t coef_stride, uint32_t ncols, uint32_t L, uint32_t n, uint32_t out_log,
                       const uint32_t* d_tw, DomainScalars ds, uint32_t* d_out, size_t out_stride, const EncodeTreeSink* sink,
                       const EncodeFoldSink* fsink) {
    const size_t N = (size_t)1 << out_log;
    hipStream_t s = L_.stream;
    const double enc_bytes = 4.0 * ncols * ((double)N + (double)((size_t)1 << L));
    if (L == 0) {
        Scope scope(L_, "ntt_broadcast", enc_bytes);
        dim3 grid((unsigned)((N + 255) / 256), ncols, L_.batch);
        ntt_broadcast_kernel<<<grid, 256, 0, s>>>(d_coef, coef_stride, d_out, out_stride, N, L_.bstride / 4);
        return 0;
    }
    const uint32_t cpw_max = L_.tune->ntt_cpw <= MAX_COLS_PER_WG ? L_.tune->ntt_cpw : MAX_COLS_PER_WG;
    uint32_t cpw = cpw_max;
    while (ncols % cpw) cpw--;
    const size_t lds_bytes = (size_t)cpw * TILE_WORDS * sizeof(uint32_t);

    const uint32_t last_t = L < TILE_LOG ? L : TILE_LOG;
    uint32_t rest = L - last_t;
    const uint32_t mid_max = TILE_LOG - MID_LOG_W;
    const uint32_t n_mid_generic = (rest + mid_max - 1) / mid_max;
    uint32_t n_mid_fast = 0;
    NttArgs a{};
    a.in = d_coef;
    a.in_stride = coef_stride;
    a.in_mask = (uint32_t)(((size_t)1 << L) - 1);
    a.out = d_out;
    a.out_stride = out_stride;
    a.tw = d_tw;
    a.n = n;
    a.init_y = ds.init_y;
    a.bstride_w = L_.bstride / 4;
    uint32_t cpw4 = MAX_COLS_PER_WG;
    const uint32_t cpw_small = L_.tune->ntt_cpw_small;
    if ((N >> TILE_LOG) * (size_t)L_.batch < 512) cpw4 = cpw_small;
    while (ncols % cpw4) cpw4--;
    uint32_t fused_levels = 0;
    auto launch_pass = [&](uint32_t t, const char* name) {
        const bool aligned = ((a.in_stride | a.out_stride) & 3) == 0 && (a.in_mask & 3u) == 3u &&
                             ((reinterpret_cast<uintptr_t>(a.in) | reinterpret_cast<uintptr_t>(a.out) | L_.bstride) & 15) == 0;
        if (sink && aligned && a.log_w == 0 && t == 12 && ncols == 4 && n >= TILE_LOG && out_log == n) {
            NttTreeArgs ta{};
            ta.a = a;
            ta.a.ncols = 4;
            ta.layers = sink->layers;
            ta.last_out = sink->last_out;
            ta.bstride = L_.bstride;
            const bool reg_only = L_.tune->ntt_tree_reg_only;
            const uint32_t levels = reg_only ? 5u : ENCODE_TREE_LEVELS;
            double bytes = enc_bytes / ((n_mid_fast ? n_mid_fast : n_mid_generic) + 1) + 48.0 * (double)N;
            for (uint32_t l = 1; l < levels; l++) bytes += 96.0 * (double)(N >> l);
            Scope scope(L_, reg_only ? "ntt_last_tree5" : "ntt_last_tree7", bytes);
            const dim3 grid((unsigned)(N >> TILE_LOG), 1, L_.batch);
            const bool tp = (size_t)grid.x * grid.z >= L_.tune->tp_min_wgs;
#define FR_LAUNCH_LAST_TREE(SA, RO)                                                      \
    do {                                                                                 \
        if (tp)                                                                          \
            ntt_last_tree_kernel<SA, RO, true><<<grid, NTT_THREADS, 0, s>>>(ta);         \
        else                                                                             \
            ntt_last_tree_kernel<SA, RO, false><<<grid, NTT_THREADS, 0, s>>>(ta);        \
    } while (0)
            if (sink->layers && reg_only)
                FR_LAUNCH_LAST_TREE(true, true);
            else if (sink->layers)
                FR_LAUNCH_LAST_TREE(true, false);
            else if (reg_only)
                FR_LAUNCH_LAST_TREE(false, true);
            else
                FR_LAUNCH_LAST_TREE(false, false);
#undef FR_LAUNCH_LAST_TREE
            fused_levels = levels;
            return;
        }
        if (fsink && aligned && a.log_w == 0 && t == 12 && ncols == 4 && n >= TILE_LOG + 2 && out_log == n && L_.batch == 1 &&
            ((reinterpret_cast<uintptr_t>(fsink->line1) | reinterpret_cast<uintptr_t>(fsink->line2) | reinterpret_cast<uintptr_t>(fsink->itw)) & 15) == 0) {
            NttFoldArgs fa{};
            fa.a = a;
            fa.a.ncols = 4;
            fa.itw = fsink->itw;
            fa.inv_init_y = ds.inv_init_y;
            for (int i = 0; i < 4; i++) fa.alpha0[i] = fsink->alpha0[i], fa.alpha1[i] = fsink->alpha1[i];
            fa.line1 = fsink->line1;
            fa.line2 = fsink->line2;
            Scope scope(L_, "ntt_last_fold2", enc_bytes / ((n_mid_fast ? n_mid_fast : n_mid_generic) + 1) + 36.0 * (double)N);
            const dim3 grid((unsigned)(N >> TILE_LOG), 1, 1);
            const bool side_by_side = (N >> TILE_LOG) < 512 && L_.tune->lds_opt_in_ok && L_.tune->ntt_cpw == 4 && !L_.tune->ntt_no_cp;
            const size_t cp_lds = (size_t)4 * TILE_WORDS * sizeof(uint32_t);
            if (side_by_side && fsink->accumulate)
                ntt_last_fold_cp_kernel<true><<<grid, NTT_CP_THREADS, cp_lds, s>>>(fa);
            else if (side_by_side)
                ntt_last_fold_cp_kernel<false><<<grid, NTT_CP_THREADS, cp_lds, s>>>(fa);
            else if (fsink->accumulate)
                ntt_last_fold_kernel<true><<<grid, NTT_THREADS, 0, s>>>(fa);
            else
                ntt_last_fold_kernel<false><<<grid, NTT_THREADS, 0, s>>>(fa);
            fused_levels = 1;
            return;
        }
        Scope scope(L_, name, enc_bytes / ((n_mid_fast ? n_mid_fast : n_mid_generic) + 1));
        const uint32_t hb_log = n - 1 - a.i_hi;
        const uint64_t rep_wgs = (uint64_t)((N >> TILE_LOG) >> (hb_log < 3 ? hb_log : 3)) * (ncols / 2) * L_.batch;
        const bool use_rep = L_.tune->ntt_rep == 1 || (L_.tune->ntt_rep == 2 && rep_wgs >= 1024);
        if (use_rep && out_log == n && aligned && t == 8 && a.log_w == MID_LOG_W && hb_log >= 1 && ((uint64_t)a.in_mask >> (a.i_hi + 1)) == 0 && ncols % 2 == 0) {
            a.rep_log = hb_log < 3 ? hb_log : 3;
            a.ncols = 2;
            dim3 grid((unsigned)((N >> TILE_LOG) >> a.rep_log), ncols / 2, L_.batch);
            ntt_tile12_rep_kernel<2><<<grid, NTT_THREADS, 0, s>>>(a);
            a.rep_log = 0;
        } else if (aligned && t + a.log_w == TILE_LOG && (t == 12 || t == 8 || t == 4)) {
            a.ncols = cpw4;
            dim3 grid((unsigned)(N >> TILE_LOG), ncols / cpw4, L_.batch);
            if (t == 12)
                ntt_tile12_kernel<3, 0><<<grid, NTT_THREADS, 0, s>>>(a);
            else if (t == 8)
                ntt_tile12_kernel<2, MID_LOG_W><<<grid, NTT_THREADS, 0, s>>>(a);
            else
                ntt_tile12_kernel<1, 8><<<grid, NTT_THREADS, 0, s>>>(a);
        } else {
            a.ncols = cpw;
            set_stages(a, t);
            dim3 grid((unsigned)(N >> (t + a.log_w)), ncols / cpw, L_.batch);
            ntt_tile_kernel<<<grid, NTT_THREADS, lds_bytes, s>>>(a);
        }
    };
    a.in_limit = a.in_mask + 1;
    uint32_t i_hi = L - 1;
    const bool no_pad8 = L_.tune->ntt_no_pad8;
    const uint32_t units = (rest + 3) / 4, padz = 4 * units - rest;
    const bool base_aligned = ((a.in_stride | a.out_stride) & 3) == 0 &&
                              ((reinterpret_cast<uintptr_t>(a.in) | reinterpret_cast<uintptr_t>(a.out) | L_.bstride) & 15) == 0;
    if (rest > 0 && base_aligned && padz <= out_log - L && L >= 4 && (!no_pad8 || (padz == 0 && (units & 1) == 0))) {
        n_mid_fast = (units + 1) / 2;
        uint32_t top = L - 1 + padz, left = units;
        bool first = true;
        while (left) {
            const uint32_t t = (left & 1) ? 4u : 8u;
            a.i_hi = top;
            a.i_lo = top + 1 - t;
            a.log_w = TILE_LOG - t;
            if (first) {
                a.in_mask = (uint32_t)(((size_t)1 << (L + padz)) - 1);
                a.in_limit = (uint32_t)1 << L;
            }
            launch_pass(t, "ntt_pass_mid");
            a.in = d_out;
            a.in_stride = out_stride;
            a.in_mask = (uint32_t)(N - 1);
            a.in_limit = (uint32_t)N;
            top -= t;
            left -= t / 4;
            first = false;
        }
        rest = 0;
        i_hi = last_t - 1;
    }
    const uint32_t n_mid = n_mid_generic;
    for (uint32_t p = 0; p < n_mid && rest; p++) {
        uint32_t t = (rest + (n_mid - p) - 1) / (n_mid - p);
        a.i_hi = i_hi;
        a.i_lo = i_hi + 1 - t;
        a.log_w = t >= mid_max ? MID_LOG_W : TILE_LOG - t;
        launch_pass(t, "ntt_pass_mid");
        a.in = d_out;
        a.in_stride = out_stride;
        a.in_mask = (uint32_t)(N - 1);
        a.in_limit = (uint32_t)N;
        rest -= t;
        i_hi = a.i_lo - 1;
    }
    a.i_hi = i_hi;
    a.i_lo = 0;
    a.log_w = 0;
    launch_pass(last_t, "ntt_pass_last");
    return fused_levels;
}
}

}
}
```

### frieda_amd/csrc/prover.cpp

```cpp
#include <string.h>

#include <algorithm>
#include <chrono>
#include <cstdlib>

#include <stddef.h>

#include "dev_transcript.h"
#include "host.h"

namespace frieda {

namespace {

void hash_to_words(const uint8_t* h, uint32_t (&w)[8]) {
    for (int i = 0; i < 8; i++)
        w[i] = (uint32_t)h[4 * i] | ((uint32_t)h[4 * i + 1] << 8) | ((uint32_t)h[4 * i + 2] << 16) | ((uint32_t)h[4 * i + 3] << 24);
}

}

int ensure_pinned(Ctx* ctx, size_t bytes) {
    if (ctx->pinned_bytes >= bytes) return FRIEDA_OK;
    if (ctx->pinned) FR_HIP(ctx, hipHostFree(ctx->pinned));
    ctx->pinned = nullptr;
    ctx->pinned_bytes = 0;
    FR_HIP(ctx, hipHostMalloc(&ctx->pinned, bytes, hipHostMallocDefault));
    ctx->pinned_bytes = bytes;
    return FRIEDA_OK;
}

namespace {

constexpr size_t SMALL_HOST_IN_BYTES = 7680;
int ensure_pinned_in(Ctx* ctx) {
    if (ctx->pinned_in) return FRIEDA_OK;
    FR_HIP(ctx, hipHostMalloc(&ctx->pinned_in, SMALL_HOST_IN_BYTES, hipHostMallocDefault));
    return FRIEDA_OK;
}

struct Shape {
    CodecShape cs;
    uint32_t L, B, n;
    size_t N;
};

int make_shape(Ctx* ctx, size_t len, uint32_t B, Shape& sh) {
    if (B > FRIEDA_MAX_LOG_DOMAIN) return ctx->fail(FRIEDA_ERR_ARG, "log_blowup_factor larger than FRIEDA_MAX_LOG_DOMAIN");
    if (len > ((size_t)1 << 40)) return ctx->fail(FRIEDA_ERR_ARG, "blob larger than 2^40 bytes");
    sh.cs = codec_shape(len);
    sh.L = sh.cs.log_size;
    sh.B = B;
    if ((uint64_t)sh.L + B < 1) return ctx->fail(FRIEDA_ERR_INVARIANT, "log_size + log_blowup_factor must be >= 1");
    if ((uint64_t)sh.L + B > FRIEDA_MAX_LOG_DOMAIN) return ctx->fail(FRIEDA_ERR_ARG, "domain larger than FRIEDA_MAX_LOG_DOMAIN");
    sh.n = sh.L + B;
    sh.N = (size_t)1 << sh.n;
    return FRIEDA_OK;
}

void line_interpolate(std::vector<QM31>& v, Coset c) {
    const uint32_t lg = c.log_size;
    const size_t n = v.size();
    for (uint32_t i = 0; i < n; i++) {
        uint32_t j = bit_reverse(i, lg);
        if (i < j) std::swap(v[i], v[j]);
    }
    for (Coset d = c; d.log_size > 0; d = d.doubled()) {
        const size_t sz = (size_t)1 << d.log_size, half = sz / 2;
        std::vector<uint32_t> ix(half);
        CPoint p = point_from_index(d.initial), st = point_from_index(d.step);
        for (size_t i = 0; i < half; i++) {
            ix[i] = m31_inv(p.x);
            p = cp_add(p, st);
        }
        for (size_t base = 0; base < n; base += sz)
            for (size_t i = 0; i < half; i++) {
                QM31 a = v[base + i], b = v[base + half + i];
                v[base + i] = qm_add(a, b);
                v[base + half + i] = qm_scale(qm_sub(a, b), ix[i]);
            }
    }
    uint32_t len_inv = m31_inv((uint32_t)n);
    for (auto& q : v) q = qm_scale(q, len_inv);
}

void bit_reverse_vec(std::vector<QM31>& v, size_t count, uint32_t lg) {
    for (uint32_t i = 0; i < count; i++) {
        uint32_t j = bit_reverse(i, lg);
        if (i < j) std::swap(v[i], v[j]);
    }
}

}

int commit_device(Ctx* ctx, const uint8_t* d_data, size_t len, uint32_t log_blowup, uint8_t* d_root, bool data_in_arena) {
    FR_NO_JOB(ctx);
    Shape sh;
    int rc = make_shape(ctx, len, log_blowup, sh);
    if (rc) return rc;
    FR_HIP(ctx, hipSetDevice(ctx->device));

    ArenaPlan plan;
    size_t o_data = plan.take(data_in_arena ? len : 0);
    size_t o_coef = plan.take(sizeof(uint32_t) * sh.cs.n_padded);
    size_t o_eval = plan.take(sizeof(uint32_t) * 4 * sh.N);
    size_t o_scr = plan.take(k::merkle_root_scratch_bytes(sh.n));
    (void)o_data;
    if (!data_in_arena) {
        rc = ctx->ensure_arena(plan.off);
        if (rc) return rc;
    } else if (plan.off > ctx->arena_bytes) {
        return ctx->fail(FRIEDA_ERR_ARG, "internal: arena not sized by caller");
    }
    TwiddleSet tw;
    rc = ctx->get_twiddles(sh.n, tw);
    if (rc) return rc;

    uint32_t* coef = reinterpret_cast<uint32_t*>(ctx->arena + o_coef);
    uint32_t* eval = reinterpret_cast<uint32_t*>(ctx->arena + o_eval);
    if (k::small_domain_shape(ctx->tuning, sh.L, sh.n)) {
        k::small_encode_and_first_tree(ctx->launch(), d_data, len, 0, sh.L, sh.n, tw.d_tw, tw.ds, nullptr, 0, nullptr, ctx->arena + o_scr, d_root,
                                       nullptr, nullptr, 0);
    } else {
        k::unpack30(ctx->launch(), d_data, len, coef, sh.cs.n_padded);
        k::encode_and_first_tree(ctx->launch(), coef, (size_t)1 << sh.L, sh.L, sh.n, tw.d_tw, tw.ds, eval, sh.N, nullptr, ctx->arena + o_scr, d_root,
                                 nullptr);
    }
    FR_HIP(ctx, hipGetLastError());
    return FRIEDA_OK;
}

int commit_host(Ctx* ctx, const uint8_t* data, size_t len, uint32_t log_blowup, uint8_t out_root[32]) {
    FR_NO_JOB(ctx);
    Shape sh;
    int rc = make_shape(ctx, len, log_blowup, sh);
    if (rc) return rc;
    FR_HIP(ctx, hipSetDevice(ctx->device));
    ArenaPlan plan;
    size_t o_data = plan.take(len);
    plan.take(sizeof(uint32_t) * sh.cs.n_padded);
    plan.take(sizeof(uint32_t) * 4 * sh.N);
    plan.take(k::merkle_root_scratch_bytes(sh.n));
    size_t o_root = plan.take(32);
    rc = ctx->ensure_arena(plan.off);
    if (rc) return rc;
    rc = ensure_pinned(ctx, 4096);
    if (rc) return rc;
    if (k::small_domain_shape(ctx->tuning, sh.L, sh.n) && len <= SMALL_HOST_IN_BYTES) {
        rc = ensure_pinned_in(ctx);
        if (rc) return rc;
        if (len) memcpy(ctx->pinned_in, data, len);
        rc = commit_device(ctx, static_cast<const uint8_t*>(ctx->pinned_in), len, log_blowup, static_cast<uint8_t*>(ctx->pinned), true);
        if (rc) return rc;
        FR_HIP(ctx, hipStreamSynchronize(ctx->stream));
        memcpy(out_root, ctx->pinned, 32);
        return FRIEDA_OK;
    }
    if (len) FR_HIP(ctx, hipMemcpyAsync(ctx->arena + o_data, data, len, hipMemcpyHostToDevice, ctx->stream));
    rc = commit_device(ctx, ctx->arena + o_data, len, log_blowup, ctx->arena + o_root, true);
    if (rc) return rc;
    FR_HIP(ctx, hipMemcpyAsync(ctx->pinned, ctx->arena + o_root, 32, hipMemcpyDeviceToHost, ctx->stream));
    FR_HIP(ctx, hipStreamSynchronize(ctx->stream));
    memcpy(out_root, ctx->pinned, 32);
    return FRIEDA_OK;
}

int commit_batch(Ctx* ctx, const uint8_t* data, size_t data_stride, size_t len, uint32_t count, bool data_on_device, uint32_t log_blowup,
                 uint8_t* out_roots, const uint8_t* const* host_ptrs) {
    int rc = commit_batch_begin(ctx, data, data_stride, len, count, data_on_device, log_blowup, host_ptrs);
    if (rc) return rc;
    return commit_batch_finish(ctx, out_roots);
}

int commit_batch_finish(Ctx* ctx, uint8_t* out_roots) {
    if (!ctx->commit_pending) return ctx->fail(FRIEDA_ERR_ARG, "no commit batch in flight on this context");
    const uint32_t count = ctx->commit_pending;
    ctx->commit_pending = 0;
    FR_HIP(ctx, hipSetDevice(ctx->device));
    FR_HIP(ctx, hipStreamSynchronize(ctx->stream));
    FR_HIP(ctx, hipGetLastError());
    memcpy(out_roots, ctx->pinned, 32 * (size_t)count);
    return FRIEDA_OK;
}

int commit_batch_begin(Ctx* ctx, const uint8_t* data, size_t data_stride, size_t len, uint32_t count, bool data_on_device, uint32_t log_blowup,
                       const uint8_t* const* host_ptrs) {
    FR_NO_JOB(ctx);
    if (count == 0 || count > 65535) return ctx->fail(FRIEDA_ERR_ARG, "batch count out of range");
    if (count > 1 && data_stride < len) return ctx->fail(FRIEDA_ERR_ARG, "batch stride smaller than the blob length");
    Shape sh;
    int rc = make_shape(ctx, len, log_blowup, sh);
    if (rc) return rc;
    FR_HIP(ctx, hipSetDevice(ctx->device));
    ArenaPlan plan;
    const size_t o_data = plan.take(data_on_device ? 0 : len);
    const size_t o_coef = plan.take(sizeof(uint32_t) * sh.cs.n_padded);
    const size_t o_eval = plan.take(sizeof(uint32_t) * 4 * sh.N);
    const size_t o_scr = plan.take(k::merkle_root_scratch_bytes(sh.n));
    const size_t o_root = plan.take(32);
    const size_t bstride = plan.off;
    rc = ctx->ensure_arena(bstride * count);
    if (rc) return rc;
    rc = ensure_pinned(ctx, 32 * (size_t)count + 4096);
    if (rc) return rc;
    TwiddleSet tw;
    rc = ctx->get_twiddles(sh.n, tw);
    if (rc) return rc;
    hipStream_t s = ctx->stream;
    uint8_t* A = ctx->arena;
    k::Launch LN = ctx->launch();
    LN.batch = count;
    LN.bstride = count > 1 ? bstride : 0;
    const uint8_t* d_data = data;
    size_t d_stride = data_stride;
    if (!data_on_device) {
        if (len && host_ptrs) {
            for (uint32_t b = 0; b < count; b++) FR_HIP(ctx, hipMemcpyAsync(A + o_data + (size_t)b * bstride, host_ptrs[b], len, hipMemcpyHostToDevice, s));
        } else if (len) {
            FR_HIP(ctx, hipMemcpy2DAsync(A + o_data, bstride, data, count > 1 ? data_stride : len, len, count, hipMemcpyHostToDevice, s));
        }
        d_data = A + o_data;
        d_stride = bstride;
    }
    uint32_t* coef = reinterpret_cast<uint32_t*>(A + o_coef);
    uint32_t* eval = reinterpret_cast<uint32_t*>(A + o_eval);
    if (k::small_domain_shape(ctx->tuning, sh.L, sh.n)) {
        k::small_encode_and_first_tree(LN, d_data, len, d_stride, sh.L, sh.n, tw.d_tw, tw.ds, nullptr, 0, nullptr, A + o_scr, A + o_root, nullptr,
                                       nullptr, 0);
    } else {
        k::unpack30(LN, d_data, len, coef, sh.cs.n_padded, d_stride);
        k::encode_and_first_tree(LN, coef, (size_t)1 << sh.L, sh.L, sh.n, tw.d_tw, tw.ds, eval, sh.N, nullptr, A + o_scr, A + o_root, nullptr);
    }
    FR_HIP(ctx, hipMemcpy2DAsync(ctx->pinned, 32, A + o_root, bstride, 32, count, hipMemcpyDeviceToHost, s));
    FR_HIP(ctx, hipGetLastError());
    ctx->commit_pending = count;
    return FRIEDA_OK;
}

namespace {

struct FriLayerDev {
    size_t o_vals;
    size_t o_tree;
    uint32_t log;
};

struct GatherPlan {
    std::vector<uint64_t> word_idx;
    std::vector<uint64_t> hash_idx;
};

std::vector<uint32_t> plan_witness(const std::vector<uint32_t>& queries, const FriLayerDev& lay, GatherPlan& g, size_t& n_witness, uint64_t tag = 0) {
    std::vector<uint32_t> pos;
    n_witness = 0;
    const size_t stride = (size_t)1 << lay.log;
    for (size_t i = 0; i < queries.size();) {
        size_t j = i;
        while (j < queries.size() && (queries[j] >> 1) == (queries[i] >> 1)) j++;
        uint32_t start = (queries[i] >> 1) << 1;
        size_t kq = i;
        for (uint32_t p = start; p < start + 2; p++) {
            pos.push_back(p);
            if (kq < j && queries[kq] == p) {
                kq++;
                continue;
            }
            for (int c = 0; c < 4; c++) g.word_idx.push_back((lay.o_vals / 4 + (size_t)c * stride + p) | tag);
            n_witness++;
        }
        i = j;
    }
    return pos;
}

size_t plan_merkle_decommit(const std::vector<uint32_t>& positions, const FriLayerDev& lay, GatherPlan& g, uint64_t tag = 0) {
    static thread_local std::vector<uint32_t> buf_a, buf_b;
    std::vector<uint32_t>* below = &buf_a;
    std::vector<uint32_t>* here = &buf_b;
    below->assign(positions.begin(), positions.end());
    size_t n_hashes = 0;
    for (int layer = (int)lay.log - 1; layer >= 0; layer--) {
        const size_t child_base = (lay.o_tree + k::merkle_layer_offset(lay.log, (uint32_t)layer + 1)) / 32;
        here->clear();
        const uint32_t* c = below->data();
        const size_t nc = below->size();
        for (size_t i = 0; i < nc;) {
            const uint32_t node = c[i] >> 1;
            const bool has_left = c[i] == 2 * node;
            if (has_left) i++;
            const bool has_right = i < nc && c[i] == 2 * node + 1;
            if (has_right) i++;
            if (!has_left) {
                g.hash_idx.push_back((child_base + 2 * (size_t)node) | tag);
                n_hashes++;
            }
            if (!has_right) {
                g.hash_idx.push_back((child_base + 2 * (size_t)node + 1) | tag);
                n_hashes++;
            }
            here->push_back(node);
        }
        std::swap(below, here);
    }
    return n_hashes;
}

}

struct ProveJob {
    frieda_pcs_config cfg{};
    Shape sh{};
    uint32_t n = 0, last = 0, last_log = 0, n_inner = 0;
    size_t N = 0;
    FriLayerDev first{};
    std::vector<FriLayerDev> inner;
    size_t o_lastv = 0, o_nonce = 0, o_tr = 0, o_gnext = 0, o_widx = 0, o_hidx = 0, o_wout = 0, o_hout = 0;
    size_t max_words = 0, max_hashes = 0, tr_host_pitch = 0;
    bool dev_channel = false;
    bool dev_decommit = false;
    size_t dec_off = 0, dec_stride = 0, dec_words_off = 0, dec_hashes_off = 0;
    uint32_t dec_max_words = 0, dec_max_hashes = 0;
    uint32_t count = 1;
    size_t bstride = 0;
    uint32_t skip_log = 0;
    const Encoded* enc = nullptr;
    uint32_t first_skip_log = 0;
    struct Blob {
        Channel ch{};
        std::vector<Hash32> roots;
        std::vector<std::array<uint32_t, 4>> alphas;
        std::vector<QM31> lastv;
        uint64_t nonce = ~0ull;
        uint32_t digest_before_grind[8] = {0};
    };
    std::vector<Blob> blobs;
    uint64_t grind_base = 0, grind_chunk = 0;
    std::chrono::steady_clock::time_point t_start;
};

void ProveJobDeleter::operator()(ProveJob* j) const { delete j; }

namespace {
void plan_prove_blob(ArenaPlan& plan, const Shape& sh, uint32_t last_log, size_t host_len, size_t& o_data, size_t& o_coef, FriLayerDev& first,
                     std::vector<FriLayerDev>& inner, size_t& o_lastv, size_t& o_nonce, bool shared_first = false) {
    const uint32_t n = sh.n, n_inner = (n - 1) - last_log;
    if (shared_first) {
        o_data = o_coef = 0;
        first = FriLayerDev{0, 0, n};
    } else {
        o_data = plan.take(host_len);
        o_coef = plan.take(sizeof(uint32_t) * sh.cs.n_padded);
        first = FriLayerDev{plan.take(sizeof(uint32_t) * 4 * sh.N), 0, n};
        first.o_tree = plan.take(k::merkle_layer_offset(n, 0) + 32);
    }
    inner.resize(n_inner);
    for (uint32_t kx = 0; kx < n_inner; kx++) {
        uint32_t lg = n - 1 - kx;
        inner[kx].log = lg;
        inner[kx].o_vals = plan.take(sizeof(uint32_t) * 4 << lg);
        inner[kx].o_tree = plan.take(k::merkle_layer_offset(lg, 0) + 32);
    }
    o_lastv = plan.take(sizeof(uint32_t) * 4 << last_log);
    o_nonce = plan.take(8);
}
}

size_t opening_max_words(uint32_t n_queries, uint32_t n_inner) { return (size_t)n_queries * 4 * (1 + (n_inner + 1)); }
size_t opening_max_hashes(uint32_t n_queries, uint32_t n, uint32_t n_inner, bool seeds) {
    if (!seeds) return (size_t)n_queries * 2 * (size_t)(n + 1) * (n_inner + 1);
    size_t h = 0;
    for (uint32_t li = 0; li <= n_inner; li++) h += (size_t)n_queries * (n - li);
    return h;
}

size_t workspace_bytes_per_blob(size_t len, uint32_t log_blowup, uint32_t log_last_layer, bool prove, bool data_on_device) {
    if (log_blowup > FRIEDA_MAX_LOG_DOMAIN || len > ((size_t)1 << 40)) return 0;
    Shape sh;
    sh.cs = codec_shape(len);
    sh.L = sh.cs.log_size;
    sh.B = log_blowup;
    if ((uint64_t)sh.L + log_blowup < 1 || (uint64_t)sh.L + log_blowup > FRIEDA_MAX_LOG_DOMAIN) return 0;
    sh.n = sh.L + log_blowup;
    sh.N = (size_t)1 << sh.n;
    ArenaPlan plan;
    if (!prove) {
        plan.take(data_on_device ? 0 : len);
        plan.take(sizeof(uint32_t) * sh.cs.n_padded);
        plan.take(sizeof(uint32_t) * 4 * sh.N);
        plan.take(k::merkle_root_scratch_bytes(sh.n));
        plan.take(32);
        return plan.off;
    }
    if (log_last_layer > 10 || sh.n < 2 || sh.L < 1 + log_last_layer || log_last_layer + log_blowup > sh.n - 1) return 0;
    size_t a, b, c, d;
    FriLayerDev first;
    std::vector<FriLayerDev> inner;
    plan_prove_blob(plan, sh, log_last_layer + log_blowup, data_on_device ? 0 : len, a, b, first, inner, c, d);
    return plan.off;
}

uint64_t batch_budget_bytes(const k::Tuning& t) {
    if (t.batch_budget_mb) {
        const uint64_t b = (uint64_t)t.batch_budget_mb << 20;
        return t.device_mem_bytes ? std::min<uint64_t>(b, t.device_mem_bytes / 100 * 45) : b;
    }
    if (t.device_mem_bytes) return std::min<uint64_t>(batch_budget_bytes(k::tuning_defaults()), t.device_mem_bytes / 100 * 16);
    static const uint64_t sixteen_headline = 16 * (uint64_t)workspace_bytes_per_blob((size_t)15 << 20, 4, 0, true, true);
    return sixteen_headline;
}

uint32_t batch_per_call(const k::Tuning& t, size_t ws_per_blob, uint32_t count, uint32_t in_flight) {
    if (count == 0) return 1;
    if (in_flight == 0) in_flight = 1;
    uint64_t per = ws_per_blob ? batch_budget_bytes(t) / ws_per_blob : 1;
    const uint64_t ways = (uint64_t)std::max<uint32_t>(1, t.batch_calls_per_ctx) * in_flight;
    const uint64_t spread = (count + ways - 1) / ways;
    per = std::min<uint64_t>(per, spread);
    per = std::min<uint64_t>(per, 4096);
    return (uint32_t)std::max<uint64_t>(per, 1);
}

void batch_cut(uint32_t count, uint32_t per_call, uint32_t in_flight, std::vector<uint32_t>& calls) {
    calls.clear();
    if (count == 0) return;
    if (per_call == 0) per_call = 1;
    if (in_flight == 0) in_flight = 1;
    const uint64_t round = (uint64_t)per_call * in_flight;
    uint64_t n = (uint64_t)in_flight * ((count + round - 1) / round);
    n = std::min<uint64_t>(n, count);
    const uint32_t base = (uint32_t)(count / n), extra = (uint32_t)(count % n);
    calls.assign((size_t)n, base);
    for (uint32_t i = 0; i < extra; i++) calls[i] = base + 1;
}


static double ms_since(std::chrono::steady_clock::time_point t0) {
    return std::chrono::duration<double, std::milli>(std::chrono::steady_clock::now() - t0).count();
}

static int download_transcripts(Ctx* ctx, const ProveJob& J) {
    const size_t bytes = offsetof(DevTranscript, last_poly) + ((size_t)16 << J.last);
    const uint8_t* d_tr = ctx->arena + J.o_tr;
    if (J.count == 1) {
        FR_HIP(ctx, hipMemcpyAsync(ctx->pinned, d_tr, bytes, hipMemcpyDeviceToHost, ctx->stream));
    } else {
        FR_HIP(ctx, hipMemcpy2DAsync(ctx->pinned, J.tr_host_pitch, d_tr, sizeof(DevTranscript), bytes, J.count, hipMemcpyDeviceToHost, ctx->stream));
    }
    return FRIEDA_OK;
}

static void launch_decommit(Ctx* ctx, const ProveJob& J, const k::Launch& LN) {
    uint8_t* A = ctx->arena;
    k::DecommitArgs a{};
    a.tr = reinterpret_cast<const DevTranscript*>(A + J.o_tr);
    a.n = J.n;
    a.n_layers = 1 + J.n_inner;
    a.n_queries = J.cfg.n_queries;
    a.bstride = J.count > 1 ? J.bstride : 0;
    a.out = static_cast<uint8_t*>(ctx->pinned) + J.dec_off;
    a.out_stride = J.dec_stride;
    a.words_off = J.dec_words_off;
    a.hashes_off = J.dec_hashes_off;
    a.max_words = J.dec_max_words;
    a.max_hashes = J.dec_max_hashes;
    a.skip_log = J.skip_log;
    a.skip_log0 = J.first_skip_log;
    a.first_shared = J.enc ? 1 : 0;
    a.vals[0] = J.enc ? J.enc->eval() : reinterpret_cast<const uint32_t*>(A + J.first.o_vals);
    a.trees[0] = J.enc ? J.enc->tree() : A + J.first.o_tree;
    for (uint32_t kx = 0; kx < J.n_inner; kx++) {
        a.vals[1 + kx] = reinterpret_cast<const uint32_t*>(A + J.inner[kx].o_vals);
        a.trees[1 + kx] = A + J.inner[kx].o_tree;
    }
    const uint32_t wgs = J.count >= 8 ? 1u : (J.count >= 2 ? 2u : (J.n >= 16 ? 8u : 2u));
    k::decommit(LN, a, wgs);
}

int prove_begin(Ctx* ctx, const uint8_t* data, size_t len, bool data_on_device, const uint64_t* seed, frieda_pcs_config cfg) {
    return prove_begin_batch(ctx, data, 0, len, 1, data_on_device, seed, cfg);
}

int prove_begin_batch_ptrs(Ctx* ctx, const uint8_t* const* blobs, size_t len, uint32_t count, const uint64_t* seeds, frieda_pcs_config cfg) {
    if (!blobs || count == 0) return ctx->fail(FRIEDA_ERR_ARG, "null blob table");
    return prove_begin_batch(ctx, blobs[0], len, len, count, false, seeds, cfg, blobs);
}

static int prove_begin_impl(Ctx* ctx, const uint8_t* data, size_t data_stride, size_t len, uint32_t count, bool data_on_device,
                            const uint64_t* seeds, frieda_pcs_config cfg, const uint8_t* const* host_ptrs, const Encoded* enc);

int prove_begin_batch(Ctx* ctx, const uint8_t* data, size_t data_stride, size_t len, uint32_t count, bool data_on_device,
                      const uint64_t* seeds, frieda_pcs_config cfg, const uint8_t* const* host_ptrs) {
    return prove_begin_impl(ctx, data, data_stride, len, count, data_on_device, seeds, cfg, host_ptrs, nullptr);
}

int prove_seeds_begin(Ctx* ctx, const Encoded* enc, const uint64_t* seeds, uint32_t n_seeds, frieda_pcs_config cfg) {
    if (!enc || !enc->d) return ctx->fail(FRIEDA_ERR_ARG, "null encoded blob");
    if (!seeds) return ctx->fail(FRIEDA_ERR_ARG, "null seeds");
    if (n_seeds == 0 || n_seeds > 65535) return ctx->fail(FRIEDA_ERR_ARG, "n_seeds out of range");
    if (cfg.log_blowup_factor != enc->log_blowup) return ctx->fail(FRIEDA_ERR_ARG, "log_blowup_factor differs from the one the blob was encoded with");
    if (enc->device != ctx->device) return ctx->fail(FRIEDA_ERR_ARG, "the encoded blob lives on another device");
    return prove_begin_impl(ctx, nullptr, 0, enc->len, n_seeds, true, seeds, cfg, nullptr, enc);
}

static int prove_begin_impl(Ctx* ctx, const uint8_t* data, size_t data_stride, size_t len, uint32_t count, bool data_on_device,
                            const uint64_t* seeds, frieda_pcs_config cfg, const uint8_t* const* host_ptrs, const Encoded* enc) {
    const auto t_entry = std::chrono::steady_clock::now();
    FR_NO_JOB(ctx);
    if (count == 0 || count > 65535) return ctx->fail(FRIEDA_ERR_ARG, "batch count out of range");
    if (!enc && count > 1 && data_stride < len) return ctx->fail(FRIEDA_ERR_ARG, "batch stride smaller than the blob length");
    const uint32_t B = cfg.log_blowup_factor, last = cfg.log_last_layer_degree_bound;
    if (last > 10) return ctx->fail(FRIEDA_ERR_ARG, "log_last_layer_degree_bound > 10");
    if (B > FRIEDA_MAX_LOG_DOMAIN) return ctx->fail(FRIEDA_ERR_ARG, "log_blowup_factor larger than FRIEDA_MAX_LOG_DOMAIN");
    std::unique_ptr<ProveJob, ProveJobDeleter> jp(new ProveJob());
    ProveJob& J = *jp;
    Shape& sh = J.sh;
    int rc = make_shape(ctx, len, B, sh);
    if (rc) return rc;
    if (sh.n < 2 || sh.L < 1 + last) return ctx->fail(FRIEDA_ERR_INVARIANT, "polynomial too small for the FRI configuration");
    if (cfg.n_queries == 0 || cfg.n_queries > 4096) return ctx->fail(FRIEDA_ERR_ARG, "n_queries out of range");
    if (cfg.pow_bits > 48) return ctx->fail(FRIEDA_ERR_ARG, "pow_bits > 48");
    FR_HIP(ctx, hipSetDevice(ctx->device));
    J.cfg = cfg;
    J.last = last;
    J.count = count;
    J.skip_log = k::tree_skip_threshold(ctx->tuning, count);
    J.enc = enc;
    J.first_skip_log = enc ? enc->skip_log : J.skip_log;
    J.blobs.resize(count);
    const uint32_t n = J.n = sh.n, last_log = J.last_log = last + B;
    const size_t N = J.N = sh.N;
    const uint32_t n_inner = J.n_inner = (n - 1) - last_log;

    ArenaPlan plan;
    size_t o_data = 0, o_coef = 0;
    FriLayerDev& first = J.first;
    std::vector<FriLayerDev>& inner = J.inner;
    plan_prove_blob(plan, sh, last_log, data_on_device ? 0 : len, o_data, o_coef, first, inner, J.o_lastv, J.o_nonce, enc != nullptr);
    const size_t o_lastv = J.o_lastv, o_nonce = J.o_nonce;
    const size_t bstride = J.bstride = plan.off;
    plan.off = bstride * count;
    const size_t o_tr = J.o_tr = plan.take(sizeof(DevTranscript) * count);
    J.o_gnext = plan.take(sizeof(uint32_t) * k::GRIND_NEXT_STRIDE * count);
    J.max_words = opening_max_words(cfg.n_queries, n_inner) * count;
    J.max_hashes = opening_max_hashes(cfg.n_queries, n, n_inner, enc != nullptr) * count;
    J.o_widx = plan.take(8 * J.max_words);
    J.o_hidx = plan.take(8 * J.max_hashes);
    J.o_wout = plan.take(4 * J.max_words);
    J.o_hout = plan.take(32 * J.max_hashes);
    rc = ctx->ensure_arena(plan.off);
    if (rc) return rc;
    const size_t tr_host_pitch = J.tr_host_pitch = (offsetof(DevTranscript, last_poly) + ((size_t)16 << last) + 63) & ~(size_t)63;
    J.dec_max_words = (uint32_t)(J.max_words / count);
    J.dec_max_hashes = (uint32_t)(J.max_hashes / count);
    J.dec_words_off = k::DECOMMIT_HEADER_BYTES;
    J.dec_hashes_off = J.dec_words_off + ((4 * (size_t)J.dec_max_words + 15) & ~(size_t)15);
    J.dec_stride = (J.dec_hashes_off + 32 * (size_t)J.dec_max_hashes + 255) & ~(size_t)255;
    J.dec_off = (tr_host_pitch * count + 255) & ~(size_t)255;
    const size_t pinned_need =
        std::max<size_t>(std::max<size_t>(std::max<size_t>(tr_host_pitch * count, (sizeof(uint32_t) * 4) << last_log),
                                          (4 + 8) * J.max_words + (32 + 8) * J.max_hashes + 512),
                         J.dec_off + J.dec_stride * count);
    rc = ensure_pinned(ctx, pinned_need);
    if (rc) return rc;
    TwiddleSet tw;
    rc = ctx->get_twiddles(n, tw);
    if (rc) return rc;
    hipStream_t s = ctx->stream;
    J.t_start = std::chrono::steady_clock::now();
    for (double& v : ctx->phase_ms) v = 0.0;
    k::Launch LN = ctx->launch();
    LN.batch = count;
    LN.bstride = count > 1 ? bstride : 0;
    uint8_t* A = ctx->arena;
    const bool dev_channel = J.dev_channel = last_log <= k::TAIL_LOG && !ctx->host_channel;
    if (count > 1 && !dev_channel)
        return ctx->fail(FRIEDA_ERR_ARG, "batches need the device channel (last layer <= 2^11 points, host channel policy off)");

    const uint8_t* d_data = data;
    size_t d_data_stride = data_stride;
    const bool small = k::small_domain_shape(ctx->tuning, sh.L, n) && !ctx->host_channel && last_log <= k::TAIL_LOG;
    if (!data_on_device && !enc) {
        if (small && count == 1 && len <= SMALL_HOST_IN_BYTES) {
            rc = ensure_pinned_in(ctx);
            if (rc) return rc;
            const uint8_t* src = host_ptrs ? host_ptrs[0] : data;
            if (len) memcpy(ctx->pinned_in, src, len);
            d_data = static_cast<const uint8_t*>(ctx->pinned_in);
            d_data_stride = 0;
        } else {
            if (len && host_ptrs) {
                for (uint32_t b = 0; b < count; b++) FR_HIP(ctx, hipMemcpyAsync(A + o_data + (size_t)b * bstride, host_ptrs[b], len, hipMemcpyHostToDevice, s));
            } else {
                if (len && count == 1) FR_HIP(ctx, hipMemcpyAsync(A + o_data, data, len, hipMemcpyHostToDevice, s));
                if (len && count > 1) FR_HIP(ctx, hipMemcpy2DAsync(A + o_data, bstride, data, data_stride, len, count, hipMemcpyHostToDevice, s));
            }
            d_data = A + o_data;
            d_data_stride = bstride;
        }
    }
    uint32_t* coef = reinterpret_cast<uint32_t*>(A + o_coef);
    uint32_t* eval = enc ? const_cast<uint32_t*>(enc->eval()) : reinterpret_cast<uint32_t*>(A + first.o_vals);
    if (!small && !enc) k::unpack30(LN, d_data, len, coef, sh.cs.n_padded, d_data_stride);
    ctx->phase_ms[5] = ms_since(t_entry);

    for (uint32_t b = 0; b < count; b++) {
        J.blobs[b].ch.init();
        if (seeds) J.blobs[b].ch.mix_u64(seeds[b]);
        J.blobs[b].roots.assign(1 + n_inner, Hash32{});
    }
    Channel& ch = J.blobs[0].ch;

    auto cols = [&](const FriLayerDev& lay, int c) { return (&lay == &first ? eval : reinterpret_cast<uint32_t*>(A + lay.o_vals)) + ((size_t)c << lay.log); };
    const uint32_t seeds_group = enc ? ctx->tuning.seeds_fold_group : 0;
    std::vector<Hash32>& roots = J.blobs[0].roots;
    std::vector<QM31>& lastv = J.blobs[0].lastv;
    if (dev_channel) {
        DevTranscript* d_tr = reinterpret_cast<DevTranscript*>(A + o_tr);
        const size_t hdr = offsetof(DevTranscript, last_poly);
        {
            for (uint32_t b = 0; b < count; b++) {
                DevTranscript* ht = reinterpret_cast<DevTranscript*>(static_cast<uint8_t*>(ctx->pinned) + b * tr_host_pitch);
                memset(ht, 0, hdr);
                ht->ch = J.blobs[b].ch;
                ht->nonce = ~0ull;
                ht->draw_bound = ctx->test_draw_bound;
            }
        }
        if (enc)
            k::channel_after_shared_root(LN, enc->d + enc->o_root, d_tr, reinterpret_cast<const DevTranscript*>(ctx->pinned), tr_host_pitch);
        else if (small)
            k::small_encode_and_first_tree(LN, d_data, len, d_data_stride, sh.L, n, tw.d_tw, tw.ds, eval, N, A + first.o_tree, nullptr, nullptr, d_tr,
                                           reinterpret_cast<const DevTranscript*>(ctx->pinned), tr_host_pitch);
        else
            k::encode_and_first_tree(LN, coef, (size_t)1 << sh.L, sh.L, n, tw.d_tw, tw.ds, eval, N, A + first.o_tree, nullptr, nullptr, d_tr,
                                     reinterpret_cast<const DevTranscript*>(ctx->pinned), tr_host_pitch);
        const FriLayerDev* cur = &first;
        bool circle = true;
        uint32_t kx = 0;
        const uint32_t tail_run_log = ctx->tuning.tail_run_log;
        while (kx < n_inner && inner[kx].log > tail_run_log) {
            k::fold_and_tree(LN, circle, cols(*cur, 0), (size_t)1 << cur->log, cur->log, n, tw.d_itw, tw.ds, cols(inner[kx], 0),
                             A + inner[kx].o_tree, d_tr, enc && circle, circle ? seeds_group : 0);
            cur = &inner[kx];
            circle = false;
            kx++;
        }
        uint32_t* tvals[16];
        uint8_t* ttrees[16];
        const uint32_t n_tail = (n_inner - kx) + 1;
        if (n_tail > 16) return ctx->fail(FRIEDA_ERR_INVARIANT, "internal: tail too long");
        for (uint32_t i = 0; i + 1 < n_tail; i++) {
            tvals[i] = cols(inner[kx + i], 0);
            ttrees[i] = A + inner[kx + i].o_tree;
        }
        tvals[n_tail - 1] = reinterpret_cast<uint32_t*>(A + o_lastv);
        ttrees[n_tail - 1] = nullptr;
        uint32_t* d_gnext = reinterpret_cast<uint32_t*>(A + J.o_gnext);
        k::fri_tail(LN, cols(*cur, 0), (size_t)1 << cur->log, cur->log, circle, n, tw.d_itw, tw.ds, last_log, last, n_tail, tvals, ttrees,
                    d_tr, d_gnext, enc && circle);
        J.grind_base = 0;
        J.grind_chunk = (uint64_t)1 << std::max<uint32_t>(22, std::min<uint32_t>(cfg.pow_bits, 36) + 4);
        if (ctx->tuning.test_grind_first_log) J.grind_chunk = (uint64_t)1 << ctx->tuning.test_grind_first_log;
        k::grind_dev(LN, d_tr, d_gnext, cfg.pow_bits, J.grind_base, J.grind_chunk, true);
        rc = download_transcripts(ctx, J);
        if (rc) return rc;
        J.dev_decommit = cfg.n_queries <= k::DECOMMIT_MAX_QUERIES && 1 + n_inner <= k::DECOMMIT_MAX_LAYERS && n <= k::DECOMMIT_MAX_LOG_DOMAIN &&
                         !ctx->tuning.host_decommit;
        if (J.dev_decommit) launch_decommit(ctx, J, LN);
        FR_HIP(ctx, hipGetLastError());
        ctx->phase_ms[0] = ms_since(J.t_start);
    } else {
        auto fetch_root = [&](const FriLayerDev& lay, Hash32& root) -> int {
            FR_HIP(ctx, hipMemcpyAsync(ctx->pinned, A + lay.o_tree + k::merkle_layer_offset(lay.log, 0), 32, hipMemcpyDeviceToHost, s));
            FR_HIP(ctx, hipStreamSynchronize(s));
            memcpy(root.data(), ctx->pinned, 32);
            return FRIEDA_OK;
        };

        if (enc) {
            memcpy(roots[0].data(), enc->root, 32);
        } else {
            k::circle_evaluate(LN, coef, (size_t)1 << sh.L, 4, sh.L, n, tw.d_tw, tw.ds, eval, N);
            k::merkle_tree4(LN, cols(first, 0), cols(first, 1), cols(first, 2), cols(first, 3), n, A + first.o_tree);
            rc = fetch_root(first, roots[0]);
            if (rc) return rc;
        }
        uint32_t rw[8];
        hash_to_words(roots[0].data(), rw);
        ch.mix_root(rw);

        QM31 alpha = ch.draw_felt(ctx->test_draw_bound);
        J.blobs[0].alphas.assign(1 + n_inner, std::array<uint32_t, 4>{});
        J.blobs[0].alphas[0] = {alpha.a, alpha.b, alpha.c, alpha.d};
        {
            uint32_t* dst = (n_inner > 0) ? cols(inner[0], 0) : reinterpret_cast<uint32_t*>(A + o_lastv);
            FR_HIP(ctx, hipMemsetAsync(dst, 0, sizeof(uint32_t) * 4 << (n - 1), s));
            k::fold_circle_into_line(LN, dst, (size_t)1 << (n - 1), eval, N, n, tw.d_itw, tw.ds, k::Alpha{{alpha.a, alpha.b, alpha.c, alpha.d}});
        }
        for (uint32_t kx = 0; kx < n_inner; kx++) {
            const FriLayerDev& lay = inner[kx];
            k::merkle_tree4(LN, cols(lay, 0), cols(lay, 1), cols(lay, 2), cols(lay, 3), lay.log, A + lay.o_tree);
            rc = fetch_root(lay, roots[kx + 1]);
            if (rc) return rc;
            hash_to_words(roots[kx + 1].data(), rw);
            ch.mix_root(rw);
            alpha = ch.draw_felt(ctx->test_draw_bound);
            J.blobs[0].alphas[kx + 1] = {alpha.a, alpha.b, alpha.c, alpha.d};
            uint32_t* dst = (kx + 1 < n_inner) ? cols(inner[kx + 1], 0) : reinterpret_cast<uint32_t*>(A + o_lastv);
            k::fold_line(LN, cols(lay, 0), (size_t)1 << lay.log, lay.log, n, tw.d_itw, tw.ds, k::Alpha{{alpha.a, alpha.b, alpha.c, alpha.d}}, dst,
                         (size_t)1 << (lay.log - 1));
        }

        const size_t n_lastdom = (size_t)1 << last_log;
        FR_HIP(ctx, hipMemcpyAsync(ctx->pinned, A + o_lastv, sizeof(uint32_t) * 4 * n_lastdom, hipMemcpyDeviceToHost, s));
        FR_HIP(ctx, hipStreamSynchronize(s));
        lastv.assign(n_lastdom, QM31{0, 0, 0, 0});
        {
            const uint32_t* h = reinterpret_cast<const uint32_t*>(ctx->pinned);
            for (size_t i = 0; i < n_lastdom; i++) lastv[i] = {h[i], h[n_lastdom + i], h[2 * n_lastdom + i], h[3 * n_lastdom + i]};
        }
        line_interpolate(lastv, line_coset(n, last_log));
        bit_reverse_vec(lastv, n_lastdom, last_log);
        const size_t n_poly = (size_t)1 << last;
        for (size_t i = n_poly; i < n_lastdom; i++)
            if (!qm_is_zero(lastv[i])) return ctx->fail(FRIEDA_ERR_INVARIANT, "invalid degree");
        lastv.resize(n_poly);
        bit_reverse_vec(lastv, n_poly, last);
        channel_mix_felts(ch, lastv);
        memcpy(J.blobs[0].digest_before_grind, ch.digest, 32);

        unsigned long long* d_nonce = reinterpret_cast<unsigned long long*>(A + o_nonce);
        {
            FR_HIP(ctx, hipMemsetAsync(d_nonce, 0xFF, 8, s));
            uint64_t base = 0, chunk = (uint64_t)1 << 22;
            for (;;) {
                k::grind_scan(LN, ch.digest, cfg.pow_bits, base, chunk, d_nonce);
                FR_HIP(ctx, hipMemcpyAsync(ctx->pinned, d_nonce, 8, hipMemcpyDeviceToHost, s));
                FR_HIP(ctx, hipStreamSynchronize(s));
                memcpy(&J.blobs[0].nonce, ctx->pinned, 8);
                if (J.blobs[0].nonce != ~0ull) break;
                base += chunk;
                if (chunk < ((uint64_t)1 << 28)) chunk <<= 1;
            }
        }
        ctx->phase_ms[0] = ms_since(J.t_start);
    }
    ctx->job = std::move(jp);
    return FRIEDA_OK;
}

int prove_finish(Ctx* ctx, uint8_t out_commitment[32], ProofData& out) {
    if (ctx->job && ctx->job->count != 1) return ctx->fail(FRIEDA_ERR_ARG, "the proof in flight is a batch: use the batch finish");
    std::vector<ProofData> outs(1);
    outs[0] = std::move(out);
    int rc = prove_finish_batch(ctx, out_commitment, outs);
    if (!outs.empty()) out = std::move(outs[0]);
    return rc;
}

uint32_t job_count(const Ctx* ctx) { return ctx->job ? ctx->job->count : 0; }

int prove_finish_batch(Ctx* ctx, uint8_t* out_commitments, std::vector<ProofData>& outs) {
    if (!ctx->job) return ctx->fail(FRIEDA_ERR_ARG, "no proof in flight on this context");
    std::unique_ptr<ProveJob, ProveJobDeleter> jp = std::move(ctx->job);
    ProveJob& J = *jp;
    FR_HIP(ctx, hipSetDevice(ctx->device));
    hipStream_t s = ctx->stream;
    k::Launch LN = ctx->launch();
    LN.batch = J.count;
    LN.bstride = J.count > 1 ? J.bstride : 0;
    uint8_t* A = ctx->arena;
    const frieda_pcs_config cfg = J.cfg;
    const uint32_t n = J.n, last = J.last, n_inner = J.n_inner, count = J.count;
    const size_t N = J.N;
    const FriLayerDev& first = J.first;
    const std::vector<FriLayerDev>& inner = J.inner;

    if (J.dev_channel) {
        DevTranscript* d_tr = reinterpret_cast<DevTranscript*>(A + J.o_tr);
        const size_t n_poly = (size_t)1 << last;
        auto host_tr = [&](uint32_t b) { return reinterpret_cast<const DevTranscript*>(static_cast<const uint8_t*>(ctx->pinned) + b * J.tr_host_pitch); };
        for (;;) {
            FR_HIP(ctx, hipStreamSynchronize(s));
            bool all_found = true;
            for (uint32_t b = 0; b < count; b++) {
                if (host_tr(b)->status & 1u) return ctx->fail(FRIEDA_ERR_INVARIANT, "invalid degree");
                all_found &= host_tr(b)->nonce != ~0ull;
            }
            if (all_found) break;
            J.grind_base += J.grind_chunk;
            if (J.grind_chunk < ((uint64_t)1 << 28)) J.grind_chunk <<= 1;
            k::grind_dev(LN, d_tr, reinterpret_cast<uint32_t*>(A + J.o_gnext), cfg.pow_bits, J.grind_base, J.grind_chunk);
            int rc = download_transcripts(ctx, J);
            if (rc) return rc;
            if (J.dev_decommit) launch_decommit(ctx, J, LN);
        }
        FR_HIP(ctx, hipGetLastError());
        for (uint32_t b = 0; b < count; b++) {
            const DevTranscript* ht = host_tr(b);
            ProveJob::Blob& bl = J.blobs[b];
            if (ht->n_roots != 1 + n_inner || ht->n_last_poly != n_poly) return ctx->fail(FRIEDA_ERR_INVARIANT, "internal: transcript out of step");
            bl.nonce = ht->nonce;
            bl.ch = ht->ch;
            memcpy(bl.digest_before_grind, ht->ch.digest, 32);
            bl.alphas.resize(1 + n_inner);
            for (uint32_t li = 0; li <= n_inner; li++) {
                for (int w = 0; w < 8; w++)
                    for (int bb = 0; bb < 4; bb++) bl.roots[li][4 * w + bb] = (uint8_t)(ht->roots[li][w] >> (8 * bb));
                bl.alphas[li] = {ht->alphas[li][0], ht->alphas[li][1], ht->alphas[li][2], ht->alphas[li][3]};
            }
            bl.lastv.resize(n_poly);
            for (size_t i = 0; i < n_poly; i++)
                bl.lastv[i] = {ht->last_poly[4 * i], ht->last_poly[4 * i + 1], ht->last_poly[4 * i + 2], ht->last_poly[4 * i + 3]};
        }
    }
    ctx->phase_ms[1] = ms_since(J.t_start);
    ctx->last_transcript.roots = J.blobs[0].roots;
    ctx->last_transcript.alphas = J.blobs[0].alphas;
    memcpy(ctx->last_transcript.digest_before_grind, J.blobs[0].digest_before_grind, 32);

    struct LayerCounts {
        size_t n_witness, n_hashes;
    };
    std::vector<LayerCounts> counts((size_t)count * (1 + n_inner));
    std::vector<size_t> n_evals(count);
    std::vector<const uint32_t*> words_of(count);
    std::vector<const uint8_t*> hashes_of(count);

    bool from_device = J.dev_decommit;
    if (from_device) {
        for (uint32_t b = 0; b < count && from_device; b++) {
            const uint8_t* reg = static_cast<const uint8_t*>(ctx->pinned) + J.dec_off + (size_t)b * J.dec_stride;
            const uint32_t* hdr = reinterpret_cast<const uint32_t*>(reg);
            if (hdr[0] == k::DECOMMIT_OVERFLOW) {
                from_device = false;
                break;
            }
            if (hdr[0] != k::DECOMMIT_OK) return ctx->fail(FRIEDA_ERR_INVARIANT, "internal: device decommit out of step with the grind");
            n_evals[b] = hdr[1];
            words_of[b] = reinterpret_cast<const uint32_t*>(reg + J.dec_words_off);
            hashes_of[b] = reg + J.dec_hashes_off;
            LayerCounts* cnt = &counts[(size_t)b * (1 + n_inner)];
            size_t suffix[40] = {0};
            for (uint32_t sft = n; sft >= 1; sft--) suffix[sft] = suffix[sft + 1] + hdr[3 + sft];
            for (uint32_t li = 0; li <= n_inner; li++) {
                cnt[li].n_witness = hdr[3 + li + 1];
                cnt[li].n_hashes = li + 2 <= n ? suffix[li + 2] : 0;
            }
        }
        ctx->phase_ms[2] = ctx->phase_ms[3] = ms_since(J.t_start);
    }
    if (!from_device) {
        struct TempTree {
            uint8_t* d = nullptr;
            ~TempTree() {
                if (d) (void)hipFree(d);
            }
        } first_full;
        const uint8_t* first_tree_alt = J.enc ? J.enc->tree() : nullptr;
        if (J.enc && first.log >= J.first_skip_log) {
            if (hipMalloc((void**)&first_full.d, k::merkle_layer_offset(n, 0) + 32) != hipSuccess) {
                (void)hipGetLastError();
                return ctx->fail(FRIEDA_ERR_NOMEM, "no device memory for the complete first-layer tree of the host decommitment");
            }
            const uint32_t* c0 = J.enc->eval();
            k::merkle_tree4(ctx->launch(), c0, c0 + N, c0 + 2 * N, c0 + 3 * N, n, first_full.d);
            first_tree_alt = first_full.d;
        }
        {
            k::Launch Lb = ctx->launch();
            for (uint32_t b = 0; b < count; b++) {
                const size_t boff = (size_t)b * J.bstride;
                auto rebuild = [&](const FriLayerDev& lay) {
                    if (lay.log < J.skip_log) return;
                    const uint32_t* c0 = reinterpret_cast<const uint32_t*>(A + lay.o_vals + boff);
                    const size_t cs = (size_t)1 << lay.log;
                    k::merkle_tree4(Lb, c0, c0 + cs, c0 + 2 * cs, c0 + 3 * cs, lay.log, A + lay.o_tree + boff);
                };
                if (!J.enc) rebuild(first);
                for (uint32_t kx = 0; kx < n_inner; kx++) rebuild(inner[kx]);
            }
        }
        static thread_local GatherPlan g;
        g.word_idx.clear();
        g.hash_idx.clear();
        std::vector<size_t> w_begin(count), h_begin(count);
        for (uint32_t b = 0; b < count; b++) {
            ProveJob::Blob& bl = J.blobs[b];
            bl.ch.mix_u64(bl.nonce);
            const std::vector<uint32_t> queries = generate_queries(bl.ch, n, cfg.n_queries);
            n_evals[b] = queries.size();
            w_begin[b] = g.word_idx.size();
            h_begin[b] = g.hash_idx.size();
            const size_t boff = (size_t)b * J.bstride;
            auto shifted = [&](FriLayerDev lay) {
                lay.o_vals += boff;
                lay.o_tree += boff;
                return lay;
            };
            LayerCounts* cnt = &counts[(size_t)b * (1 + n_inner)];
            const uint64_t tag0 = J.enc ? k::GATHER_ALT : 0;
            const FriLayerDev lay0 = J.enc ? first : shifted(first);
            for (uint32_t q : queries)
                for (int c = 0; c < 4; c++) g.word_idx.push_back((lay0.o_vals / 4 + (size_t)c * N + q) | tag0);
            {
                std::vector<uint32_t> pos = plan_witness(queries, lay0, g, cnt[0].n_witness, tag0);
                cnt[0].n_hashes = plan_merkle_decommit(pos, lay0, g, tag0);
            }
            std::vector<uint32_t> lq = fold_queries(queries, 1);
            for (uint32_t kx = 0; kx < n_inner; kx++) {
                const FriLayerDev lay = shifted(inner[kx]);
                std::vector<uint32_t> pos = plan_witness(lq, lay, g, cnt[kx + 1].n_witness);
                cnt[kx + 1].n_hashes = plan_merkle_decommit(pos, lay, g);
                lq = fold_queries(lq, 1);
            }
        }
        ctx->phase_ms[2] = ms_since(J.t_start);
        if (g.word_idx.size() > J.max_words || g.hash_idx.size() > J.max_hashes) return ctx->fail(FRIEDA_ERR_INVARIANT, "internal: gather plan overflow");
        const size_t nw = g.word_idx.size(), nh = g.hash_idx.size();
        const size_t wbytes = 4 * nw, out_bytes = wbytes + 32 * nh;
        uint8_t* hp = reinterpret_cast<uint8_t*>(ctx->pinned);
        uint64_t* hidx = reinterpret_cast<uint64_t*>(hp + ((4 * J.max_words + 32 * J.max_hashes + 255) & ~(size_t)255));
        memcpy(hidx, g.word_idx.data(), 8 * nw);
        memcpy(hidx + nw, g.hash_idx.data(), 8 * nh);
        k::Launch L1 = ctx->launch();
        if (out_bytes <= ((size_t)1 << 20) && !ctx->tuning.gather_copy) {
            k::gather(L1, reinterpret_cast<const uint32_t*>(A), hidx, nw, reinterpret_cast<uint32_t*>(hp), hidx + nw, nh, hp + wbytes,
                      J.enc ? J.enc->eval() : nullptr, first_tree_alt);
        } else {
            FR_HIP(ctx, hipMemcpyAsync(A + J.o_widx, hidx, 8 * (nw + nh), hipMemcpyHostToDevice, s));
            k::gather(L1, reinterpret_cast<const uint32_t*>(A), reinterpret_cast<const uint64_t*>(A + J.o_widx), nw,
                      reinterpret_cast<uint32_t*>(A + J.o_wout), reinterpret_cast<const uint64_t*>(A + J.o_widx) + nw, nh, A + J.o_wout + wbytes,
                      J.enc ? J.enc->eval() : nullptr, first_tree_alt);
            FR_HIP(ctx, hipMemcpyAsync(hp, A + J.o_wout, out_bytes, hipMemcpyDeviceToHost, s));
        }
        FR_HIP(ctx, hipStreamSynchronize(s));
        FR_HIP(ctx, hipGetLastError());
        ctx->phase_ms[3] = ms_since(J.t_start);
        for (uint32_t b = 0; b < count; b++) {
            words_of[b] = reinterpret_cast<const uint32_t*>(hp) + w_begin[b];
            hashes_of[b] = hp + wbytes + 32 * h_begin[b];
        }
    }

    if (outs.size() != count) outs.assign(count, ProofData{});
    for (uint32_t b = 0; b < count; b++) {
        ProveJob::Blob& bl = J.blobs[b];
        ProofData& out = outs[b];
        const LayerCounts* cnt = &counts[(size_t)b * (1 + n_inner)];
        const uint32_t* wv = words_of[b];
        const uint8_t* hv = hashes_of[b];
        size_t wi = 0, hi = 0;
        auto take_qm = [&]() {
            QM31 q{wv[wi], wv[wi + 1], wv[wi + 2], wv[wi + 3]};
            wi += 4;
            return q;
        };
        out.pcs_config = cfg;
        out.log_size_bound = J.sh.L;
        out.proof_of_work = bl.nonce;
        out.last_layer_poly = std::move(bl.lastv);
        out.evaluations.resize(n_evals[b]);
        for (auto& q : out.evaluations) q = take_qm();
        out.inner_layers.resize(n_inner);
        for (uint32_t li = 0; li <= n_inner; li++) {
            LayerProof& lp = li == 0 ? out.first_layer : out.inner_layers[li - 1];
            lp.commitment = bl.roots[li];
            lp.fri_witness.resize(cnt[li].n_witness);
            for (auto& q : lp.fri_witness) q = take_qm();
            lp.hash_witness.resize(cnt[li].n_hashes);
            if (cnt[li].n_hashes) memcpy(lp.hash_witness.data(), hv + 32 * hi, 32 * cnt[li].n_hashes);
            hi += cnt[li].n_hashes;
            lp.column_witness.clear();
        }
        memcpy(out_commitments + 32 * (size_t)b, bl.roots[0].data(), 32);
    }
    ctx->phase_ms[4] = ms_since(J.t_start);
    return FRIEDA_OK;
}

int prove(Ctx* ctx, const uint8_t* data, size_t len, bool data_on_device, const uint64_t* seed, frieda_pcs_config cfg,
          uint8_t out_commitment[32], ProofData& out) {
    int rc = prove_begin(ctx, data, len, data_on_device, seed, cfg);
    if (rc) return rc;
    return prove_finish(ctx, out_commitment, out);
}

size_t encoded_bytes(uint32_t n, size_t* o_tree, size_t* o_root) {
    ArenaPlan plan;
    plan.take(sizeof(uint32_t) * 4 << n);
    const size_t ot = plan.take(k::merkle_layer_offset(n, 0) + 32);
    const size_t orr = plan.take(32);
    if (o_tree) *o_tree = ot;
    if (o_root) *o_root = orr;
    return plan.off;
}

void encoded_release(Encoded& e) {
    if (!e.d) return;
    int cur = 0;
    const bool sw = hipGetDevice(&cur) == hipSuccess && cur != e.device;
    if (sw) (void)hipSetDevice(e.device);
    (void)hipFree(e.d);
    if (sw) (void)hipSetDevice(cur);
    e.d = nullptr;
}
void encoded_free(Encoded* e) {
    if (!e) return;
    encoded_release(*e);
    delete e;
}

int encode_blob(Ctx* ctx, const uint8_t* data, size_t len, bool data_on_device, uint32_t log_blowup, Encoded** out) {
    FR_NO_JOB(ctx);
    Shape sh;
    int rc = make_shape(ctx, len, log_blowup, sh);
    if (rc) return rc;
    FR_HIP(ctx, hipSetDevice(ctx->device));
    ArenaPlan plan;
    const size_t o_data = plan.take(data_on_device ? 0 : len);
    const size_t o_coef = plan.take(sizeof(uint32_t) * sh.cs.n_padded);
    rc = ctx->ensure_arena(plan.off);
    if (rc) return rc;
    rc = ensure_pinned(ctx, 4096);
    if (rc) return rc;
    TwiddleSet tw;
    rc = ctx->get_twiddles(sh.n, tw);
    if (rc) return rc;
    std::unique_ptr<Encoded, void (*)(Encoded*)> e(new Encoded(), encoded_free);
    e->device = ctx->device;
    e->len = len;
    e->log_blowup = log_blowup;
    e->n = sh.n;
    e->L = sh.L;
    e->skip_log = k::tree_skip_threshold(ctx->tuning, 1);
    e->bytes = encoded_bytes(sh.n, &e->o_tree, &e->o_root);
    if (hipMalloc((void**)&e->d, e->bytes) != hipSuccess) {
        (void)hipGetLastError();
        e->d = nullptr;
        return ctx->fail(FRIEDA_ERR_NOMEM, "hipMalloc(encoded blob " + std::to_string(e->bytes) + " B) failed");
    }
    hipStream_t s = ctx->stream;
    uint8_t* A = ctx->arena;
    const uint8_t* d_data = data;
    if (!data_on_device) {
        if (len) FR_HIP(ctx, hipMemcpyAsync(A + o_data, data, len, hipMemcpyHostToDevice, s));
        d_data = A + o_data;
    }
    const k::Launch LN = ctx->launch();
    uint32_t* eval = reinterpret_cast<uint32_t*>(e->d);
    if (k::small_domain_shape(ctx->tuning, sh.L, sh.n)) {
        k::small_encode_and_first_tree(LN, d_data, len, 0, sh.L, sh.n, tw.d_tw, tw.ds, eval, sh.N, e->d + e->o_tree, nullptr, e->d + e->o_root, nullptr,
                                       nullptr, 0);
    } else {
        uint32_t* coef = reinterpret_cast<uint32_t*>(A + o_coef);
        k::unpack30(LN, d_data, len, coef, sh.cs.n_padded);
        k::encode_and_first_tree(LN, coef, (size_t)1 << sh.L, sh.L, sh.n, tw.d_tw, tw.ds, eval, sh.N, e->d + e->o_tree, nullptr, e->d + e->o_root, nullptr);
    }
    FR_HIP(ctx, hipMemcpyAsync(ctx->pinned, e->d + e->o_root, 32, hipMemcpyDeviceToHost, s));
    FR_HIP(ctx, hipStreamSynchronize(s));
    FR_HIP(ctx, hipGetLastError());
    memcpy(e->root, ctx->pinned, 32);
    *out = e.release();
    return FRIEDA_OK;
}

size_t seeds_workspace_bytes(size_t len, frieda_pcs_config cfg, uint32_t n_seeds) {
    const uint32_t B = cfg.log_blowup_factor, last = cfg.log_last_layer_degree_bound;
    if (n_seeds == 0 || n_seeds > 65535 || last > 10 || B > FRIEDA_MAX_LOG_DOMAIN || len > ((size_t)1 << 40)) return 0;
    if (cfg.n_queries == 0 || cfg.n_queries > 4096) return 0;
    Shape sh;
    sh.cs = codec_shape(len);
    sh.L = sh.cs.log_size;
    sh.B = B;
    if ((uint64_t)sh.L + B < 1 || (uint64_t)sh.L + B > FRIEDA_MAX_LOG_DOMAIN) return 0;
    sh.n = sh.L + B;
    sh.N = (size_t)1 << sh.n;
    if (sh.n < 2 || sh.L < 1 + last) return 0;
    const uint32_t n_inner = (sh.n - 1) - (last + B);
    ArenaPlan plan;
    size_t a, b, c, d;
    FriLayerDev first;
    std::vector<FriLayerDev> inner;
    plan_prove_blob(plan, sh, last + B, 0, a, b, first, inner, c, d, true);
    plan.off *= n_seeds;
    plan.take(sizeof(DevTranscript) * n_seeds);
    plan.take(sizeof(uint32_t) * k::GRIND_NEXT_STRIDE * n_seeds);
    const size_t mw = opening_max_words(cfg.n_queries, n_inner) * n_seeds, mh = opening_max_hashes(cfg.n_queries, sh.n, n_inner, true) * n_seeds;
    plan.take(8 * mw);
    plan.take(8 * mh);
    plan.take(4 * mw);
    plan.take(32 * mh);
    return plan.off;
}

}
```

### frieda_amd/csrc/tree.hip

```cpp
#include <hip/hip_runtime.h>

#include <type_traits>

#include <cstdlib>

#include "clock_stamps.h"
#include "blake2s.h"
#include "dev_transcript.h"
#include "kernels.h"
#include "tree_dev.h"

namespace frieda {
namespace k {

namespace {

__device__ __forceinline__ void latency_kernel_priority() {
#ifndef FRIEDA_NO_LATENCY_PRIO
    __builtin_amdgcn_s_setprio(3);
#endif
}

constexpr int T5_THREADS = 256;
constexpr uint32_t T5_UNITS = 1024;
// ... 918 lines not shown
            const uint32_t root_lo = root_lds[q], root_hi = root_lds[4 + q];
            s_alpha[t] = channel_after_root_quad(tr, cr, root_lo, root_hi, QQ, x);
        }
        src = dstv;
        src_stride = cnt;
        src_log = m_new;
        circle = false;
    }

    const uint32_t lg = a.last_log, cnt = 1u << lg;
    uint32_t* V = S0;
    uint32_t* W = S1;
    for (uint32_t i = t; i < cnt; i += WG1_THREADS) {
        uint32_t b = bit_reverse(i, lg);
#pragma unroll
        for (int c = 0; c < 4; c++) W[c * cnt + i] = V[c * cnt + b];
    }
    __syncthreads();
    for (uint32_t kk = lg; kk >= 1; kk--) {
        const uint32_t half = 1u << (kk - 1);
        const uint32_t* lvl = a.itw + tw_level_offset_dev(a.n, a.n - 1 - kk);
        for (uint32_t p = t; p < (cnt >> 1); p += WG1_THREADS) {
            uint32_t i = p & (half - 1), base = (p >> (kk - 1)) << kk;
            uint32_t it = lvl[bit_reverse(i, kk - 1)];
            uint32_t i0 = base + i, i1 = i0 + half;
#pragma unroll
            for (int c = 0; c < 4; c++) {
                uint32_t l = W[c * cnt + i0], r = W[c * cnt + i1];
                W[c * cnt + i0] = m31_add(l, r);
                W[c * cnt + i1] = m31_mul(m31_sub(l, r), it);
            }
        }
        __syncthreads();
    }
    const uint32_t len_inv = (lg == 0) ? 1u : (1u << (31 - lg));
    const uint32_t sh = lg - a.last;
    uint32_t bad = 0;
    for (uint32_t j = t; j < cnt; j += WG1_THREADS) {
        uint32_t v[4];
#pragma unroll
        for (int c = 0; c < 4; c++) v[c] = m31_mul(W[c * cnt + j], len_inv);
        if ((j & ((1u << sh) - 1)) == 0) {
            uint32_t qq = j >> sh;
#pragma unroll
            for (int c = 0; c < 4; c++) {
                MSG[8 + 4 * qq + c] = v[c];
                tr->last_poly[4 * qq + c] = v[c];
            }
        } else if (v[0] | v[1] | v[2] | v[3]) {
            bad = 1;
        }
    }
    if (bad) atomicOr(&tr->status, 1u);
    const uint32_t n_poly = 1u << a.last;
    const uint32_t msg_words = 8 + 4 * n_poly;
    for (uint32_t i = msg_words + t; i < ((msg_words + 15) / 16) * 16; i += WG1_THREADS) MSG[i] = 0;
    __syncthreads();
    if (t == 0) {
        Channel ch = tr->ch;
#pragma unroll
        for (int w = 0; w < 8; w++) MSG[w] = ch.digest[w];
        uint32_t r[8];
        b2s256_words(MSG, 4 * msg_words, r);
        ch.update_digest(r);
        tr->ch = ch;
        tr->n_last_poly = n_poly;
    }
}

constexpr uint32_t GRIND_WINDOW = 1024;

struct GrindArgs {
    DevTranscript* tr;
    uint32_t* next;
    uint32_t pow_bits, batch;
    unsigned long long base;
    uint32_t n_windows;
    uint32_t units;
};

__global__ __launch_bounds__(256) void grind_dev_kernel(GrindArgs a) {
    __shared__ uint32_t s_claim[2];
    const uint32_t t = threadIdx.x;
    uint32_t b = blockIdx.x % a.batch;
    for (;;) {
        if (t < 64) {
            uint32_t got_b = ~0u, got_w = 0, idle = 0;
            while (idle < a.batch) {
                uint32_t bb = b + t;
                if (bb >= a.batch) bb -= a.batch;
                const bool cand = t < a.batch && __hip_atomic_load(&a.tr[bb].nonce, __ATOMIC_RELAXED, __HIP_MEMORY_SCOPE_AGENT) == ~0ull &&
                                  __hip_atomic_load(&a.next[bb * GRIND_NEXT_STRIDE], __ATOMIC_RELAXED, __HIP_MEMORY_SCOPE_AGENT) < a.n_windows;
                const unsigned long long mask = __ballot(cand);
                if (mask == 0) {
                    const uint32_t adv = a.batch < 64 ? a.batch : 64;
                    b += adv;
                    if (b >= a.batch) b -= a.batch;
                    idle += adv;
                    continue;
                }
                const uint32_t l = (uint32_t)__ffsll((long long)mask) - 1;
                uint32_t tb = b + l;
                if (tb >= a.batch) tb -= a.batch;
                uint32_t c = 0;
                if (t == 0) c = atomicAdd(&a.next[tb * GRIND_NEXT_STRIDE], a.units);
                c = (uint32_t)__builtin_amdgcn_readfirstlane((int)c);
                b = tb + 1 == a.batch ? 0 : tb + 1;
                if (c < a.n_windows) {
                    got_b = tb;
                    got_w = c;
                    break;
                }
                idle += l + 1;
            }
            if (t == 0) {
                s_claim[0] = got_b;
                s_claim[1] = got_w;
            }
        }
        __syncthreads();
        const uint32_t cb = s_claim[0], cw = s_claim[1];
        __syncthreads();
        if (cb == ~0u) return;
        DevTranscript* tr = a.tr + cb;
        uint32_t h[8], pre[14];
#pragma unroll
        for (int i = 0; i < 8; i++) h[i] = tr->ch.digest[i];
        b2_grind_prepare(h, pre);
        const uint32_t low_mask = a.pow_bits >= 32 ? 0xFFFFFFFFu : ((1u << a.pow_bits) - 1u);
        const unsigned long long first = a.base + (unsigned long long)cw * GRIND_WINDOW + t;
        const uint32_t my_units = a.n_windows - cw < a.units ? a.n_windows - cw : a.units;
        for (uint32_t i = 0; i < my_units * (GRIND_WINDOW / 256); i++) {
            const unsigned long long nonce = first + 256ull * i;
            if (__hip_atomic_load(&tr->nonce, __ATOMIC_RELAXED, __HIP_MEMORY_SCOPE_AGENT) < nonce) break;
            if ((b2_grind_word0(h, pre, (uint32_t)nonce, (uint32_t)(nonce >> 32)) & low_mask) != 0) continue;
            const uint32_t m[16] = {(uint32_t)nonce, (uint32_t)(nonce >> 32), 0, 0, 0, 0, 0, 0, 0, 0, 0, 0, 0, 0, 0, 0};
            uint32_t r[8];
            b2_compress(h, m, 0, 0, 0, 0, r);
            uint32_t tz;
            if (r[0])
                tz = __ffs(r[0]) - 1;
            else if (r[1])
                tz = 32 + __ffs(r[1]) - 1;
            else if (r[2])
                tz = 64 + __ffs(r[2]) - 1;
            else if (r[3])
                tz = 96 + __ffs(r[3]) - 1;
            else
                tz = 128;
            if (tz >= a.pow_bits) atomicMin(&tr->nonce, nonce);
        }
    }
}

enum TreeKernel { T_WIDE, T_WIDE3, T_NINE, T_SMALL };
bool tp_launch(const Tuning& tn, size_t workgroups) { return workgroups >= tn.tp_min_wgs; }
constexpr uint32_t T9_MIN_LOG = 8;
TreeKernel tree_kernel_for(const Tuning& tn, uint32_t level_a, uint32_t batch, bool aligned16, bool reg3_ok = false) {
    uint32_t batch_log = 0;
    while ((2u << batch_log) <= batch) batch_log++;
    if (reg3_ok && aligned16 && tn.t5_reg3_log && level_a >= 10 && level_a + batch_log >= tn.t5_reg3_log) return T_WIDE3;
    if (aligned16 && level_a >= 10 && level_a + batch_log >= tn.t5_wide_log) return T_WIDE;
    if (level_a >= T9_MIN_LOG && level_a <= tn.t9_max_log) return T_NINE;
    return T_SMALL;
}
uint32_t tree_kernel_levels(TreeKernel k, uint32_t level_a) {
    if (k == T_NINE) return T9_LEVELS;
    if (k == T_WIDE3) return 3;
    const uint32_t in_wg = level_a < (k == T_WIDE ? 10u : 8u) ? level_a : (k == T_WIDE ? 10u : 8u);
    return in_wg + 1 < T5_LEVELS ? in_wg + 1 : T5_LEVELS;
}
bool tree_args_aligned16(const TreeArgs& a) {
    return ((reinterpret_cast<uintptr_t>(a.cols) | reinterpret_cast<uintptr_t>(a.out_vals) | reinterpret_cast<uintptr_t>(a.itw) |
             (a.col_stride * 4) | (a.out_stride * 4)) & 15) == 0;
}

uint32_t launch_tree_a(const Launch& L, int mode, const TreeArgs& a, const char* name, double (*bytes_of)(int, uint32_t, uint32_t)) {
    const size_t total = (size_t)1 << a.level_a;
    const TreeKernel k = tree_kernel_for(*L.tune, a.level_a, L.batch, tree_args_aligned16(a), mode != T_NODE && a.store_all);
    const uint32_t levels = tree_kernel_levels(k, a.level_a);
    const uint32_t units = (k == T_WIDE || k == T_WIDE3) ? T5_UNITS : 256u;
    const dim3 grid((unsigned)((total + units - 1) / units), L.batch);
    Scope scope(L, name, bytes_of(mode, a.level_a, levels));
    const bool tp = tp_launch(*L.tune, (size_t)grid.x * grid.y);
    if (k == T_SMALL) {
        switch (mode) {
            case T_LEAF4: if (tp) tree5_kernel<T_LEAF4, 256, true><<<grid, T5_THREADS, 0, L.stream>>>(a); else tree5_kernel<T_LEAF4, 256, false><<<grid, T5_THREADS, 0, L.stream>>>(a); break;
            case T_NODE: if (tp) tree5_kernel<T_NODE, 256, true><<<grid, T5_THREADS, 0, L.stream>>>(a); else tree5_kernel<T_NODE, 256, false><<<grid, T5_THREADS, 0, L.stream>>>(a); break;
            case T_FOLD_CIRCLE: if (tp) tree5_kernel<T_FOLD_CIRCLE, 256, true><<<grid, T5_THREADS, 0, L.stream>>>(a); else tree5_kernel<T_FOLD_CIRCLE, 256, false><<<grid, T5_THREADS, 0, L.stream>>>(a); break;
            default: if (tp) tree5_kernel<T_FOLD_LINE, 256, true><<<grid, T5_THREADS, 0, L.stream>>>(a); else tree5_kernel<T_FOLD_LINE, 256, false><<<grid, T5_THREADS, 0, L.stream>>>(a); break;
        }
    } else if (k == T_NINE) {
        switch (mode) {
            case T_LEAF4: if (tp) tree9_kernel<T_LEAF4, true><<<grid, 256, 0, L.stream>>>(a); else tree9_kernel<T_LEAF4, false><<<grid, 256, 0, L.stream>>>(a); break;
            case T_NODE: if (tp) tree9_kernel<T_NODE, true><<<grid, 256, 0, L.stream>>>(a); else tree9_kernel<T_NODE, false><<<grid, 256, 0, L.stream>>>(a); break;
            case T_FOLD_CIRCLE: if (tp) tree9_kernel<T_FOLD_CIRCLE, true><<<grid, 256, 0, L.stream>>>(a); else tree9_kernel<T_FOLD_CIRCLE, false><<<grid, 256, 0, L.stream>>>(a); break;
            default: if (tp) tree9_kernel<T_FOLD_LINE, true><<<grid, 256, 0, L.stream>>>(a); else tree9_kernel<T_FOLD_LINE, false><<<grid, 256, 0, L.stream>>>(a); break;
        }
    } else if (k == T_WIDE3) {
        switch (mode) {
            case T_LEAF4: if (tp) tree5r_kernel<T_LEAF4, true, true><<<grid, T5_THREADS, 0, L.stream>>>(a); else tree5r_kernel<T_LEAF4, true, false><<<grid, T5_THREADS, 0, L.stream>>>(a); break;
            case T_FOLD_CIRCLE: if (tp) tree5r_kernel<T_FOLD_CIRCLE, true, true><<<grid, T5_THREADS, 0, L.stream>>>(a); else tree5r_kernel<T_FOLD_CIRCLE, true, false><<<grid, T5_THREADS, 0, L.stream>>>(a); break;
            default: if (tp) tree5r_kernel<T_FOLD_LINE, true, true><<<grid, T5_THREADS, 0, L.stream>>>(a); else tree5r_kernel<T_FOLD_LINE, true, false><<<grid, T5_THREADS, 0, L.stream>>>(a); break;
        }
    } else {
        switch (mode) {
            case T_LEAF4: if (tp) tree5r_kernel<T_LEAF4, false, true><<<grid, T5_THREADS, 0, L.stream>>>(a); else tree5r_kernel<T_LEAF4, false, false><<<grid, T5_THREADS, 0, L.stream>>>(a); break;
            case T_NODE: if (tp) tree5r_kernel<T_NODE, false, true><<<grid, T5_THREADS, 0, L.stream>>>(a); else tree5r_kernel<T_NODE, false, false><<<grid, T5_THREADS, 0, L.stream>>>(a); break;
            case T_FOLD_CIRCLE: if (tp) tree5r_kernel<T_FOLD_CIRCLE, false, true><<<grid, T5_THREADS, 0, L.stream>>>(a); else tree5r_kernel<T_FOLD_CIRCLE, false, false><<<grid, T5_THREADS, 0, L.stream>>>(a); break;
            default: if (tp) tree5r_kernel<T_FOLD_LINE, false, true><<<grid, T5_THREADS, 0, L.stream>>>(a); else tree5r_kernel<T_FOLD_LINE, false, false><<<grid, T5_THREADS, 0, L.stream>>>(a); break;
        }
    }
    return levels;
}

constexpr uint32_t T7Q_MAX_LEVEL_A = 15;

double node_levels_bytes(uint32_t la, uint32_t levels) {
    double b = 0;
    for (uint32_t i = 0; i < levels; i++) b += 96.0 * (double)((size_t)1 << (la - i));
    return b;
}

}

FR_CLOCK_READER(frieda_debug_clock_tree5r, g_clock_tree5r)

void finish_tree(const Launch& L, const TreeArgs& a, uint32_t m, uint32_t cur, const uint8_t* cur_ptr, uint8_t* s0, uint8_t* s1,
                 uint8_t* root_out, DevTranscript* tr, const DevTranscript* tr_init, size_t tr_init_pitch) {
    uint8_t* layers = a.store_all ? a.layers : nullptr;
    auto bytes_of = [](int, uint32_t la, uint32_t levels) -> double { return node_levels_bytes(la, levels); };
    while (cur > L.tune->top_max_log) {
        TreeArgs b = a;
        b.skip_a = 0;
        b.skip_bc = 0;
        b.level_a = cur - 1;
        b.children = cur_ptr;
        b.last_out = (cur_ptr == s0) ? s1 : s0;
        uint32_t l2;
        if (cur - 1 <= T7Q_MAX_LEVEL_A) {
            const uint32_t in_wg = b.level_a < 6 ? b.level_a : 6;
            l2 = in_wg + 1 < T7Q_LEVELS ? in_wg + 1 : T7Q_LEVELS;
            Scope scope(L, "tree7q_node", node_levels_bytes(cur - 1, l2));
            const dim3 grid((unsigned)((((size_t)1 << b.level_a) + T7Q_UNITS - 1) / T7Q_UNITS), L.batch);
            tree7q_kernel<<<grid, 256, 0, L.stream>>>(b);
        } else {
            l2 = launch_tree_a(L, T_NODE, b, "tree5_node", bytes_of);
        }
        cur = cur - l2;
        cur_ptr = layers ? layers + merkle_layer_offset(m, cur) : b.last_out;
    }
    TopArgs tp;
    tp.in = cur_ptr;
    tp.l_in = cur;
    tp.layers = layers;
    tp.tree_log = m;
    tp.root_out = root_out;
    tp.tr = tr;
    tp.bstride = L.bstride;
    tp.tr_init = tr_init;
    tp.tr_init_pitch = tr_init_pitch;
    {
        Scope scope(L, "tree_top", node_levels_bytes(cur > 0 ? cur - 1 : 0, cur));
        top_kernel<<<dim3(1, L.batch), WG1_THREADS, 0, L.stream>>>(tp);
    }
}

void build_tree(const Launch& L, int mode, TreeArgs a, uint32_t m, uint8_t* layers, uint8_t* scratch, uint8_t* root_out,
                DevTranscript* tr, const DevTranscript* tr_init = nullptr, size_t tr_init_pitch = 0, uint32_t seeds_group = 0) {
    a.level_a = m;
    a.tree_log = m;
    a.layers = layers;
    a.store_all = layers != nullptr;
    a.skip_bc = a.store_all && a.skip_a && m >= tree_skip_threshold(*L.tune, L.batch) && mode != T_NODE;
    a.bstride = L.bstride;
    uint8_t* s0 = scratch;
    uint8_t* s1 = scratch ? scratch + ((size_t)32 << (m > 4 ? m - 4 : 0)) : nullptr;
    a.last_out = s0;
    auto bytes_of = [](int md, uint32_t la, uint32_t levels) -> double {
        if (md == T_NODE) return node_levels_bytes(la, levels);
        return (md == T_LEAF4 ? 48.0 : 80.0) * (double)((size_t)1 << la) + node_levels_bytes(la > 0 ? la - 1 : 0, levels - 1);
    };
    const char* nm = mode == T_LEAF4 ? "tree5_leaf" : (mode == T_FOLD_CIRCLE ? "tree5_fold_circle" : "tree5_fold_line");
    uint32_t lv;
    if (seeds_group && mode == T_FOLD_CIRCLE && a.shared_src && a.store_all && a.skip_a &&
        tree_kernel_for(*L.tune, a.level_a, L.batch, tree_args_aligned16(a), true) == T_WIDE) {
        const uint32_t groups = (L.batch + seeds_group - 1) / seeds_group;
        const dim3 grid((unsigned)(((size_t)1 << a.level_a) / T5_UNITS), groups);
        lv = T5_LEVELS;
        Scope scope(L, "tree5s_fold_circle", (32.0 * groups / L.batch + 48.0) * (double)((size_t)1 << a.level_a) + node_levels_bytes(a.level_a - 1, lv - 1));
        if (tp_launch(*L.tune, (size_t)grid.x * L.batch))
            tree5rs_fold_circle_kernel<true><<<grid, T5_THREADS, 0, L.stream>>>(a, L.batch, seeds_group);
        else
            tree5rs_fold_circle_kernel<false><<<grid, T5_THREADS, 0, L.stream>>>(a, L.batch, seeds_group);
    } else {
        lv = launch_tree_a(L, mode, a, nm, bytes_of);
    }
    const uint32_t cur = m - (lv - 1);
    finish_tree(L, a, m, cur, layers ? layers + merkle_layer_offset(m, cur) : s0, s0, s1, root_out, tr, tr_init, tr_init_pitch);
}

void encode_and_first_tree(const Launch& L, const uint32_t* d_coef, size_t coef_stride, uint32_t Lc, uint32_t n, const uint32_t* d_tw,
                           DomainScalars ds, uint32_t* d_eval, size_t eval_stride, uint8_t* d_layers, uint8_t* d_scratch, uint8_t* d_root,
                           DevTranscript* tr, const DevTranscript* tr_init, size_t tr_init_pitch) {
    const bool no_fuse = L.tune->no_encode_tree_fusion  || (((size_t)1 << (n > 12 ? n - 12 : 0)) * L.batch < 256) ||
                         (d_layers != nullptr && !L.tune->encode_tree_fusion_prove );
    uint8_t* s0 = d_scratch;
    uint8_t* s1 = d_scratch ? d_scratch + ((size_t)32 << (n > 4 ? n - 4 : 0)) : nullptr;
    EncodeTreeSink sink{d_layers, s0};
    const uint32_t fused = circle_evaluate_into_tree(L, d_coef, coef_stride, 4, Lc, n, d_tw, ds, d_eval, eval_stride, no_fuse ? nullptr : &sink);
    if (!fused) {
        TreeArgs a{};
        a.cols = d_eval;
        a.col_stride = eval_stride;
        a.skip_a = d_layers != nullptr && n >= 1;
        build_tree(L, T_LEAF4, a, n, d_layers, d_scratch, d_root, tr, tr_init, tr_init_pitch);
        return;
    }
    TreeArgs a{};
    a.tree_log = n;
    a.layers = d_layers;
    a.store_all = d_layers != nullptr;
    a.bstride = L.bstride;
    const uint32_t cur = n - (fused - 1);
    finish_tree(L, a, n, cur, d_layers ? d_layers + merkle_layer_offset(n, cur) : s0, s0, s1, d_root, tr, tr_init, tr_init_pitch);
}

bool small_first_opt_in() {
    int dev = 0, lds_max = 0;
    if (hipGetDevice(&dev) != hipSuccess || hipDeviceGetAttribute(&lds_max, hipDeviceAttributeMaxSharedMemoryPerBlock, dev) != hipSuccess) {
        (void)hipGetLastError();
        return false;
    }
    const size_t dyn = ((((size_t)15 << SMALL_MAX_LOG_COEF) + 3) / 4 + 4 + ((size_t)4 << SMALL_MAX_LOG_COEF)) * sizeof(uint32_t);
    hipFuncAttributes fa{};
    if (hipFuncGetAttributes(&fa, reinterpret_cast<const void*>(small_first_kernel)) != hipSuccess) {
        (void)hipGetLastError();
        return false;
    }
    if (fa.sharedSizeBytes + dyn > (size_t)lds_max) return false;
    if (hipFuncSetAttribute(reinterpret_cast<const void*>(small_first_kernel), hipFuncAttributeMaxDynamicSharedMemorySize, (int)dyn) != hipSuccess) {
        (void)hipGetLastError();
        return false;
    }
    return true;
}

bool small_domain_shape(const Tuning& tn, uint32_t Lc, uint32_t n) {
    return !tn.no_small_fused  && n >= SMALL_MIN_LOG_DOMAIN && n <= SMALL_MAX_LOG_DOMAIN && Lc <= SMALL_MAX_LOG_COEF && Lc <= n;
}

void small_encode_and_first_tree(const Launch& L, const uint8_t* d_data, size_t len, size_t data_stride, uint32_t Lc, uint32_t n,
                                 const uint32_t* d_tw, DomainScalars ds, uint32_t* d_eval, size_t eval_stride, uint8_t* d_layers,
                                 uint8_t* d_scratch, uint8_t* d_root, DevTranscript* tr, const DevTranscript* tr_init, size_t tr_init_pitch) {
    uint8_t* s0 = d_scratch;
    uint8_t* s1 = d_scratch ? d_scratch + ((size_t)32 << (n > 4 ? n - 4 : 0)) : nullptr;
    SmallFirstArgs a{};
    a.data = d_data;
    a.len = len;
    a.data_stride = data_stride;
    a.L = Lc;
    a.n = n;
    a.init_y = ds.init_y;
    a.tw = d_tw;
    a.eval = d_eval;
    a.eval_stride = eval_stride;
    a.tree.tree_log = n;
    a.tree.level_a = n;
    a.tree.layers = d_layers;
    a.tree.store_all = d_layers != nullptr;
    a.tree.skip_a = d_layers != nullptr;
    a.tree.last_out = s0;
    a.tree.bstride = L.bstride;
    const double N = (double)((size_t)1 << n);
    {
        Scope scope(L, "small_first", (double)len + 4.0 * 4.0 * (N + (double)((size_t)1 << Lc)) + 48.0 * N + node_levels_bytes(n - 1, T9_LEVELS - 1));
        const size_t lds_words = (((size_t)15 << Lc) + 3) / 4 + 4 + ((size_t)4 << Lc);
        small_first_kernel<<<dim3(1u << (n - 8), L.batch), 256, lds_words * sizeof(uint32_t), L.stream>>>(a);
    }
    const uint32_t cur = n - (T9_LEVELS - 1);
    finish_tree(L, a.tree, n, cur, d_layers ? d_layers + merkle_layer_offset(n, cur) : s0, s0, s1, d_root, tr, tr_init, tr_init_pitch);
}

void merkle_tree4(const Launch& L, const uint32_t* c0, const uint32_t* c1, const uint32_t* c2, const uint32_t* c3, uint32_t m,
                  uint8_t* d_layers) {
    TreeArgs a{};
    a.cols = c0;
    a.col_stride = (size_t)(c1 - c0);
    (void)c2;
    (void)c3;
    build_tree(L, T_LEAF4, a, m, d_layers, nullptr, nullptr, nullptr);
}

size_t merkle_root_scratch_bytes(uint32_t m) { return ((size_t)64 << (m > 4 ? m - 4 : 0)) + 256; }

void merkle_root4(const Launch& L, const uint32_t* c0, const uint32_t* c1, const uint32_t* c2, const uint32_t* c3, uint32_t m,
                  uint8_t* d_scratch, uint8_t* d_root) {
    TreeArgs a{};
    a.cols = c0;
    a.col_stride = (size_t)(c1 - c0);
    (void)c2;
    (void)c3;
    build_tree(L, T_LEAF4, a, m, nullptr, d_scratch, d_root, nullptr);
}

void tree_first_layer(const Launch& L, const uint32_t* cols, size_t stride, uint32_t m, uint8_t* layers, DevTranscript* tr,
                      const DevTranscript* tr_init, size_t tr_init_pitch) {
    TreeArgs a{};
    a.cols = cols;
    a.col_stride = stride;
    a.skip_a = m >= 1;
    build_tree(L, T_LEAF4, a, m, layers, nullptr, nullptr, tr, tr_init, tr_init_pitch);
}

void fold_and_tree(const Launch& L, bool circle, const uint32_t* src, size_t src_stride, uint32_t src_log, uint32_t n,
                   const uint32_t* d_itw, DomainScalars ds, uint32_t* dst_vals, uint8_t* layers, DevTranscript* tr, bool shared_src,
                   uint32_t seeds_group) {
    const uint32_t m = src_log - 1;
    TreeArgs a{};
    a.cols = src;
    a.col_stride = src_stride;
    a.out_vals = dst_vals;
    a.out_stride = (size_t)1 << m;
    a.itw = circle ? d_itw : d_itw + tw_level_offset(n, n - 1 - src_log);
    a.n = n;
    a.inv_init_y = ds.inv_init_y;
    a.tr = tr;
    a.skip_a = m >= 1;
    a.shared_src = shared_src ? 1 : 0;
    build_tree(L, circle ? T_FOLD_CIRCLE : T_FOLD_LINE, a, m, layers, nullptr, nullptr, tr, nullptr, 0, seeds_group);
}

void channel_after_shared_root(const Launch& L, const uint8_t* d_root, DevTranscript* tr, const DevTranscript* tr_init, size_t tr_init_pitch) {
    TopArgs tp{};
    tp.in = d_root;
    tp.tr = tr;
    tp.tr_init = tr_init;
    tp.tr_init_pitch = tr_init_pitch;
    Scope scope(L, "seeds_first_alpha", 0.0);
    top_kernel<<<dim3(1, L.batch), WG1_THREADS, 0, L.stream>>>(tp);
}

void fri_tail(const Launch& L, const uint32_t* src, size_t src_stride, uint32_t src_log, bool src_is_circle, uint32_t n,
              const uint32_t* d_itw, DomainScalars ds, uint32_t last_log, uint32_t last, uint32_t n_layers, uint32_t* const* vals,
              uint8_t* const* trees, DevTranscript* tr, uint32_t* d_gnext, bool shared_src) {
    TailArgs a{};
    a.gnext = d_gnext;
    a.shared_src = shared_src ? 1 : 0;
    a.src = src;
    a.src_stride = src_stride;
    a.src_log = src_log;
    a.src_is_circle = src_is_circle ? 1 : 0;
    a.n = n;
    a.itw = d_itw;
    a.inv_init_y = ds.inv_init_y;
    a.last_log = last_log;
    a.last = last;
    a.n_layers = n_layers;
    for (uint32_t i = 0; i < n_layers && i < TAIL_MAX_LAYERS; i++) {
        a.vals[i] = vals[i];
        a.trees[i] = trees[i];
    }
    a.tr = tr;
    a.bstride = L.bstride;
    double bytes = 0;
    for (uint32_t i = 0; i < n_layers; i++) bytes += 168.0 * (double)((size_t)1 << (src_log - 1 - i));
    Scope scope(L, "fri_tail", bytes);
    tail_kernel<<<dim3(1, L.batch), WG1_THREADS, 0, L.stream>>>(a);
}

void grind_dev(const Launch& L, DevTranscript* tr, uint32_t* d_next, uint32_t pow_bits, uint64_t base, uint64_t count, bool next_zeroed) {
    GrindArgs a{};
    a.tr = tr;
    a.next = d_next;
    a.pow_bits = pow_bits;
    a.batch = L.batch;
    a.base = base;
    const uint64_t nwin = (count + GRIND_WINDOW - 1) / GRIND_WINDOW;
    a.n_windows = nwin > 0xFFFF0000ull ? 0xFFFF0000u : (uint32_t)nwin;
    if (a.n_windows == 0) return;
    Scope scope(L, "grind", 0.0);
    if (!next_zeroed) (void)hipMemsetAsync(d_next, 0, sizeof(uint32_t) * GRIND_NEXT_STRIDE * L.batch, L.stream);
    const uint32_t iters = L.tune->grind_iters ? L.tune->grind_iters : ((L.batch >= 2 && L.batch < 16) ? 8u : 4u);
    a.units = iters < 4 ? 1u : iters / 4;
    uint64_t want = (((uint64_t)1 << (pow_bits > 40 ? 40 : pow_bits)) / 2 / GRIND_WINDOW) * L.batch;
    if (want < 64) want = 64;
    if (want > 2048) want = 2048;
    if (want > (uint64_t)a.n_windows * L.batch) want = (uint64_t)a.n_windows * L.batch;
    grind_dev_kernel<<<(unsigned)want, 256, 0, L.stream>>>(a);
}

}
}
```

Measured before the change: 47.54 billion.

## Fuse 30-bit unpack into first NTT rep pass reading packed blob directly

Defers the unpack30 launch and, when the first NTT pass is the replicated tile12 kernel with four columns, has that kernel read the packed 30-bit byte blob and extract coefficients in registers. This drops the separate unpack kernel and the write and re-read of the coefficient buffer. It also swaps a 64-bit shift for a funnel shift in extraction, changes the tile piece mapping to be wave-local, and replaces several block-wide syncs with wave barriers. The extra unaligned five-dword loads per quad and the relaxed barriers may cost bandwidth or risk correctness if the wave-local mapping assumption does not hold.

```diff
diff --git a/frieda_amd/csrc/codec.hip b/frieda_amd/csrc/codec.hip
--- a/frieda_amd/csrc/codec.hip
+++ b/frieda_amd/csrc/codec.hip
@@ -2,6 +2,7 @@
 
 #include <cstdlib>
 
+#include "codec_dev.h"
 #include "kernels.h"
 
 namespace frieda {
@@ -9,26 +10,7 @@
 
 namespace {
 
-__device__ __forceinline__ uint32_t load_dword_guarded(const uint8_t* in, size_t len, size_t d) {
-    size_t b = d * 4;
-    if (b + 4 <= len) return *reinterpret_cast<const uint32_t*>(in + b);
-    uint32_t v = 0;
-    for (int i = 0; i < 4; i++)
-        if (b + i < len) v |= (uint32_t)in[b + i] << (8 * i);
-    return v;
-}
-
-template <int O>
-__device__ __forceinline__ uint4 extract4(const uint32_t (&w)[5]) {
-    uint32_t f[4];
-#pragma unroll
-    for (int j = 0; j < 4; j++) {
-        const int pos = O + 30 * j, q = pos >> 5, r = pos & 31;
-        uint64_t pair = ((uint64_t)w[q + 1] << 32) | w[q];
-        f[j] = (uint32_t)(pair >> r) & 0x3fffffffu;
-    }
-    return make_uint4(f[0], f[1], f[2], f[3]);
-}
+using namespace codecdev;
 
 template <int T>
 __global__ __launch_bounds__(256) void unpack30_aligned_kernel(const uint8_t* __restrict__ in, size_t len,
@@ -58,14 +40,7 @@
         uint32_t w[5];
 #pragma unroll
         for (int j = 0; j < 5; j++) w[j] = stage[d0 + j];
-        uint4 v;
-        switch (byte0 & 3) {
-            case 0: v = extract4<0>(w); break;
-            case 1: v = extract4<8>(w); break;
-            case 2: v = extract4<16>(w); break;
-            default: v = extract4<24>(w); break;
-        }
-        reinterpret_cast<uint4*>(out)[t] = v;
+        reinterpret_cast<uint4*>(out)[t] = extract4_at(w, byte0 & 3);
     }
 }
 
diff --git a/frieda_amd/csrc/codec_dev.h b/frieda_amd/csrc/codec_dev.h
--- /dev/null
+++ b/frieda_amd/csrc/codec_dev.h
@@ -0,0 +1,42 @@
+#pragma once
+#include <hip/hip_runtime.h>
+#include <stddef.h>
+#include <stdint.h>
+
+namespace frieda {
+namespace k {
+namespace codecdev {
+
+__device__ __forceinline__ uint32_t load_dword_guarded(const uint8_t* in, size_t len, size_t d) {
+    size_t b = d * 4;
+    if (b + 4 <= len) return *reinterpret_cast<const uint32_t*>(in + b);
+    uint32_t v = 0;
+#pragma unroll
+    for (int i = 0; i < 4; i++)
+        if (b + i < len) v |= (uint32_t)in[b + i] << (8 * i);
+    return v;
+}
+
+template <int O>
+__device__ __forceinline__ uint4 extract4(const uint32_t (&w)[5]) {
+    uint32_t f[4];
+#pragma unroll
+    for (int j = 0; j < 4; j++) {
+        const int pos = O + 30 * j, q = pos >> 5, r = pos & 31;
+        f[j] = __funnelshift_r(w[q], w[q + 1], r) & 0x3fffffffu;
+    }
+    return make_uint4(f[0], f[1], f[2], f[3]);
+}
+
+__device__ __forceinline__ uint4 extract4_at(const uint32_t (&w)[5], uint32_t byte_in_dword) {
+    switch (byte_in_dword) {
+        case 0: return extract4<0>(w);
+        case 1: return extract4<8>(w);
+        case 2: return extract4<16>(w);
+        default: return extract4<24>(w);
+    }
+}
+
+}
+}
+}
diff --git a/frieda_amd/csrc/context.cpp b/frieda_amd/csrc/context.cpp
--- a/frieda_amd/csrc/context.cpp
+++ b/frieda_amd/csrc/context.cpp
@@ -119,6 +119,7 @@
      }},
     {"FRIEDA_NTT_CPW_SMALL", 1, 4, [](Tuning& t, long v) { t.ntt_cpw_small = (uint32_t)v; return true; }},
     {"FRIEDA_NTT_REP", 0, 2, [](Tuning& t, long v) { t.ntt_rep = (uint32_t)v; return true; }},
+    {"FRIEDA_ENCODE_FROM_BLOB", 0, 1, [](Tuning& t, long v) { t.encode_from_blob = v != 0; return true; }},
     {"FRIEDA_NTT_NO_CP", 0, 1, [](Tuning& t, long v) { t.ntt_no_cp = v != 0; return true; }},
     {"FRIEDA_NTT_NO_PAD8", 0, 1, [](Tuning& t, long v) { t.ntt_no_pad8 = v != 0; return true; }},
     {"FRIEDA_NTT_TREE_REG_ONLY", 0, 1, [](Tuning& t, long v) { t.ntt_tree_reg_only = v != 0; return true; }},
diff --git a/frieda_amd/csrc/kernels.h b/frieda_amd/csrc/kernels.h
--- a/frieda_amd/csrc/kernels.h
+++ b/frieda_amd/csrc/kernels.h
@@ -22,6 +22,7 @@
     uint32_t ntt_cpw = 4;
     uint32_t ntt_cpw_small = 1;
     uint32_t ntt_rep = 2;
+    bool encode_from_blob = true;
     bool ntt_no_pad8 = false;
     bool ntt_no_cp = false;
     bool ntt_tree_reg_only = false;
@@ -112,8 +113,14 @@
 };
 bool circle_evaluate_fold2(const Launch& L_, const uint32_t* d_coef, size_t coef_stride, uint32_t L, uint32_t n, const uint32_t* d_tw,
                            DomainScalars ds, uint32_t* d_out, size_t out_stride, const EncodeFoldSink& fs, hipError_t* err);
+struct EncodeBlob {
+    const uint8_t* bytes;
+    size_t len, bstride;
+    uint32_t* coef;
+};
 uint32_t circle_evaluate_into_tree(const Launch& L_, const uint32_t* d_coef, size_t coef_stride, uint32_t ncols, uint32_t L, uint32_t n,
-                               const uint32_t* d_tw, DomainScalars ds, uint32_t* d_out, size_t out_stride, const EncodeTreeSink* sink);
+                               const uint32_t* d_tw, DomainScalars ds, uint32_t* d_out, size_t out_stride, const EncodeTreeSink* sink,
+                               const EncodeBlob* blob = nullptr);
 
 void circle_interpolate_block(const Launch& L_, const uint32_t* d_block, size_t in_stride, uint32_t ncols, uint32_t L, uint32_t n,
                               uint32_t block, const uint32_t* d_itw, DomainScalars ds, uint32_t* d_coef, size_t out_stride);
@@ -187,7 +194,7 @@
                                  uint8_t* d_scratch, uint8_t* d_root, DevTranscript* tr, const DevTranscript* tr_init, size_t tr_init_pitch);
 void encode_and_first_tree(const Launch& L, const uint32_t* d_coef, size_t coef_stride, uint32_t Lc, uint32_t n, const uint32_t* d_tw,
                            DomainScalars ds, uint32_t* d_eval, size_t eval_stride, uint8_t* d_layers, uint8_t* d_scratch, uint8_t* d_root,
-                           DevTranscript* tr, const DevTranscript* tr_init = nullptr, size_t tr_init_pitch = 0);
+                           DevTranscript* tr, const DevTranscript* tr_init = nullptr, size_t tr_init_pitch = 0, const EncodeBlob* blob = nullptr);
 void fold_and_tree(const Launch& L, bool circle, const uint32_t* src, size_t src_stride, uint32_t src_log, uint32_t n,
                    const uint32_t* d_itw, DomainScalars ds, uint32_t* dst_vals, uint8_t* d_layers, DevTranscript* tr, bool shared_src = false,
                    uint32_t seeds_group = 0);
diff --git a/frieda_amd/csrc/ntt.hip b/frieda_amd/csrc/ntt.hip
--- a/frieda_amd/csrc/ntt.hip
+++ b/frieda_amd/csrc/ntt.hip
@@ -5,6 +5,7 @@
 #include <cstdlib>
 
 #include "clock_stamps.h"
+#include "codec_dev.h"
 #include "kernels.h"
 #include "tree_dev.h"
 
@@ -182,7 +183,27 @@
     uint32_t stage_r[3];
     size_t bstride_w;
     uint32_t rep_log;
+    const uint8_t* blob;
+    size_t blob_len, blob_bstride;
+    uint32_t blob_log;
 };
+
+template <bool WAVE_LOCAL>
+__device__ __forceinline__ uint32_t tile_piece(uint32_t g, int kk) {
+    return WAVE_LOCAL ? 1024u * (g >> 6) + 4u * (g & 63u) + 256u * (uint32_t)kk : 4u * g + 1024u * (uint32_t)kk;
+}
+
+__device__ __forceinline__ void blob_quad_dwords(const uint8_t* in, size_t len, size_t quad, uint32_t (&w)[5]) {
+    const size_t d0 = (15 * quad) >> 2;
+    if ((d0 + 5) * 4 <= len) {
+        const uint32_t* p = reinterpret_cast<const uint32_t*>(in) + d0;
+#pragma unroll
+        for (int j = 0; j < 5; j++) w[j] = p[j];
+    } else {
+#pragma unroll
+        for (int j = 0; j < 5; j++) w[j] = codecdev::load_dword_guarded(in, len, d0 + j);
+    }
+}
 
 template <int R, int LO>
 __device__ __forceinline__ void run_stage(uint32_t* lds, const NttArgs& a, uint32_t tb, uint32_t lo_rt, uint32_t hblk) {
@@ -350,7 +371,8 @@
         }
     }
 
-    auto piece_e = [&](int kk) { return 4u * g + 1024u * (uint32_t)kk; };
+    constexpr bool WAVE_FILL = LOG_W == 0 && NS == 3;
+    auto piece_e = [&](int kk) { return tile_piece<WAVE_FILL>(g, kk); };
     auto global_of = [&](uint32_t e) { return gbase | ((e >> LOG_W) << a.i_lo) | (e & wmask); };
 
     auto load4 = [&](const uint32_t* src, uint32_t gidx) {
@@ -388,7 +410,7 @@
 #pragma unroll
                 for (int r = 0; r < 16; r++) col[pad((uint32_t)r << lo)] = x[r];
             }
-            if (LOG_W == 0 && NS == 3 && s == 1)
+            if (WAVE_FILL && s >= 1)
                 __builtin_amdgcn_wave_barrier();
             else
                 __syncthreads();
@@ -411,7 +433,7 @@
     }
 }
 
-template <int COLS>
+template <int COLS, bool BLOB>
 __global__ __launch_bounds__(NTT_THREADS) void ntt_tile12_rep_kernel(NttArgs a) {
     ntt_enter();
     constexpr int NS = 2;
@@ -426,16 +448,42 @@
     const uint32_t* in = a.in + col0 * a.in_stride + blockIdx.z * a.bstride_w;
     uint32_t* out = a.out + col0 * a.out_stride + blockIdx.z * a.bstride_w;
 
-    auto piece_e = [&](int kk) { return 4u * g + 1024u * (uint32_t)kk; };
+    auto piece_e = [&](int kk) { return tile_piece<true>(g, kk); };
     auto low_of = [&](uint32_t e) { return (wblk << LOG_W) | ((e >> LOG_W) << a.i_lo) | (e & wmask); };
 
     uint4 src[COLS][4];
-#pragma unroll
-    for (int c = 0; c < COLS; c++) {
-#pragma unroll
-        for (int kk = 0; kk < 4; kk++) {
-            const uint32_t idx = low_of(piece_e(kk)) & a.in_mask;
-            src[c][kk] = idx < a.in_limit ? *reinterpret_cast<const uint4*>(in + (size_t)c * a.in_stride + idx) : make_uint4(0u, 0u, 0u, 0u);
+    if constexpr (BLOB) {
+        const uint8_t* blob = a.blob + blockIdx.z * a.blob_bstride;
+        uint32_t w[COLS][4][5];
+#pragma unroll
+        for (int c = 0; c < COLS; c++) {
+#pragma unroll
+            for (int kk = 0; kk < 4; kk++) {
+                const uint32_t idx = low_of(piece_e(kk)) & a.in_mask;
+                if (idx < a.in_limit) {
+                    blob_quad_dwords(blob, a.blob_len, ((((size_t)col0 + c) << a.blob_log) + idx) >> 2, w[c][kk]);
+                } else {
+#pragma unroll
+                    for (int j = 0; j < 5; j++) w[c][kk][j] = 0u;
+                }
+            }
+        }
+#pragma unroll
+        for (int c = 0; c < COLS; c++) {
+#pragma unroll
+            for (int kk = 0; kk < 4; kk++) {
+                const size_t quad = ((((size_t)col0 + c) << a.blob_log) + (low_of(piece_e(kk)) & a.in_mask)) >> 2;
+                src[c][kk] = codecdev::extract4_at(w[c][kk], (uint32_t)(15 * quad) & 3u);
+            }
+        }
+    } else {
+#pragma unroll
+        for (int c = 0; c < COLS; c++) {
+#pragma unroll
+            for (int kk = 0; kk < 4; kk++) {
+                const uint32_t idx = low_of(piece_e(kk)) & a.in_mask;
+                src[c][kk] = idx < a.in_limit ? *reinterpret_cast<const uint4*>(in + (size_t)c * a.in_stride + idx) : make_uint4(0u, 0u, 0u, 0u);
+            }
         }
     }
     uint32_t pbase[NS];
@@ -489,7 +537,10 @@
                 radix16_stage(x, twd[s]);
 #pragma unroll
                 for (int r = 0; r < 16; r++) col[pad((uint32_t)r << lo)] = x[r];
-                __syncthreads();
+                if (s == 0)
+                    __syncthreads();
+                else
+                    __builtin_amdgcn_wave_barrier();
             }
             uint32_t* dst = out + (size_t)c * a.out_stride + gbase;
 #pragma unroll
@@ -497,7 +548,7 @@
                 const uint32_t e = piece_e(kk), p = pad(e);
                 *reinterpret_cast<uint4*>(dst + low_of(e)) = make_uint4(lds[p], lds[p + 1], lds[p + 2], lds[p + 3]);
             }
-            __syncthreads();
+            __builtin_amdgcn_wave_barrier();
         }
     }
 }
@@ -539,7 +590,7 @@
             }
         }
     }
-    auto piece_e = [&](int kk) { return 4u * g + 1024u * (uint32_t)kk; };
+    auto piece_e = [&](int kk) { return tile_piece<false>(g, kk); };
 
     uint4 pre[4];
 #pragma unroll
@@ -893,7 +944,7 @@
 namespace {
 uint32_t evaluate_plan(const Launch& L_, const uint32_t* d_coef, size_t coef_stride, uint32_t ncols, uint32_t L, uint32_t n, uint32_t out_log,
                        const uint32_t* d_tw, DomainScalars ds, uint32_t* d_out, size_t out_stride, const EncodeTreeSink* sink,
-                       const EncodeFoldSink* fsink = nullptr);
+                       const EncodeFoldSink* fsink = nullptr, const EncodeBlob* blob = nullptr);
 }
 
 void circle_evaluate(const Launch& L_, const uint32_t* d_coef, size_t coef_stride, uint32_t ncols, uint32_t L, uint32_t n,
@@ -907,8 +958,9 @@
 }
 
 uint32_t circle_evaluate_into_tree(const Launch& L_, const uint32_t* d_coef, size_t coef_stride, uint32_t ncols, uint32_t L, uint32_t n,
-                               const uint32_t* d_tw, DomainScalars ds, uint32_t* d_out, size_t out_stride, const EncodeTreeSink* sink) {
-    return evaluate_plan(L_, d_coef, coef_stride, ncols, L, n, n, d_tw, ds, d_out, out_stride, sink);
+                               const uint32_t* d_tw, DomainScalars ds, uint32_t* d_out, size_t out_stride, const EncodeTreeSink* sink,
+                               const EncodeBlob* blob) {
+    return evaluate_plan(L_, d_coef, coef_stride, ncols, L, n, n, d_tw, ds, d_out, out_stride, sink, nullptr, blob);
 }
 
 hipError_t ntt_opt_in_dynamic_lds() {
@@ -937,11 +989,17 @@
 namespace {
 uint32_t evaluate_plan(const Launch& L_, const uint32_t* d_coef, size_t coef_stride, uint32_t ncols, uint32_t L, uint32_t n, uint32_t out_log,
                        const uint32_t* d_tw, DomainScalars ds, uint32_t* d_out, size_t out_stride, const EncodeTreeSink* sink,
-                       const EncodeFoldSink* fsink) {
+                       const EncodeFoldSink* fsink, const EncodeBlob* blob) {
     const size_t N = (size_t)1 << out_log;
     hipStream_t s = L_.stream;
+    bool blob_pending = blob != nullptr;
+    auto unpack_pending_blob = [&] {
+        if (blob_pending) unpack30(L_, blob->bytes, blob->len, blob->coef, (size_t)ncols << L, blob->bstride);
+        blob_pending = false;
+    };
     const double enc_bytes = 4.0 * ncols * ((double)N + (double)((size_t)1 << L));
     if (L == 0) {
+        unpack_pending_blob();
         Scope scope(L_, "ntt_broadcast", enc_bytes);
         dim3 grid((unsigned)((N + 255) / 256), ncols, L_.batch);
         ntt_broadcast_kernel<<<grid, 256, 0, s>>>(d_coef, coef_stride, d_out, out_stride, N, L_.bstride / 4);
@@ -975,6 +1033,15 @@
     auto launch_pass = [&](uint32_t t, const char* name) {
         const bool aligned = ((a.in_stride | a.out_stride) & 3) == 0 && (a.in_mask & 3u) == 3u &&
                              ((reinterpret_cast<uintptr_t>(a.in) | reinterpret_cast<uintptr_t>(a.out) | L_.bstride) & 15) == 0;
+        const uint32_t hb_log = n - 1 - a.i_hi;
+        const uint64_t rep_wgs = (uint64_t)((N >> TILE_LOG) >> (hb_log < 3 ? hb_log : 3)) * (ncols / 2) * L_.batch;
+        const bool use_rep = L_.tune->ntt_rep == 1 || (L_.tune->ntt_rep == 2 && rep_wgs >= 1024);
+        const bool rep_pass = use_rep && out_log == n && aligned && t == 8 && a.log_w == MID_LOG_W && hb_log >= 1 &&
+                              ((uint64_t)a.in_mask >> (a.i_hi + 1)) == 0 && ncols % 2 == 0;
+        const bool from_blob = blob_pending && rep_pass && L_.tune->encode_from_blob && ncols == 4 && coef_stride == ((size_t)1 << L) && L >= 4 &&
+                               ((reinterpret_cast<uintptr_t>(blob->bytes) | blob->bstride) & 15) == 0;
+        if (!from_blob) unpack_pending_blob();
+        blob_pending = false;
         if (sink && aligned && a.log_w == 0 && t == 12 && ncols == 4 && n >= TILE_LOG && out_log == n) {
             NttTreeArgs ta{};
             ta.a = a;
@@ -1034,14 +1101,20 @@
             return;
         }
         Scope scope(L_, name, enc_bytes / ((n_mid_fast ? n_mid_fast : n_mid_generic) + 1));
-        const uint32_t hb_log = n - 1 - a.i_hi;
-        const uint64_t rep_wgs = (uint64_t)((N >> TILE_LOG) >> (hb_log < 3 ? hb_log : 3)) * (ncols / 2) * L_.batch;
-        const bool use_rep = L_.tune->ntt_rep == 1 || (L_.tune->ntt_rep == 2 && rep_wgs >= 1024);
-        if (use_rep && out_log == n && aligned && t == 8 && a.log_w == MID_LOG_W && hb_log >= 1 && ((uint64_t)a.in_mask >> (a.i_hi + 1)) == 0 && ncols % 2 == 0) {
+        if (rep_pass) {
             a.rep_log = hb_log < 3 ? hb_log : 3;
             a.ncols = 2;
             dim3 grid((unsigned)((N >> TILE_LOG) >> a.rep_log), ncols / 2, L_.batch);
-            ntt_tile12_rep_kernel<2><<<grid, NTT_THREADS, 0, s>>>(a);
+            if (from_blob) {
+                a.blob = blob->bytes;
+                a.blob_len = blob->len;
+                a.blob_bstride = blob->bstride;
+                a.blob_log = L;
+                ntt_tile12_rep_kernel<2, true><<<grid, NTT_THREADS, 0, s>>>(a);
+                a.blob = nullptr;
+            } else {
+                ntt_tile12_rep_kernel<2, false><<<grid, NTT_THREADS, 0, s>>>(a);
+            }
             a.rep_log = 0;
         } else if (aligned && t + a.log_w == TILE_LOG && (t == 12 || t == 8 || t == 4)) {
             a.ncols = cpw4;
diff --git a/frieda_amd/csrc/prover.cpp b/frieda_amd/csrc/prover.cpp
--- a/frieda_amd/csrc/prover.cpp
+++ b/frieda_amd/csrc/prover.cpp
@@ -122,9 +122,9 @@
         k::small_encode_and_first_tree(ctx->launch(), d_data, len, 0, sh.L, sh.n, tw.d_tw, tw.ds, nullptr, 0, nullptr, ctx->arena + o_scr, d_root,
                                        nullptr, nullptr, 0);
     } else {
-        k::unpack30(ctx->launch(), d_data, len, coef, sh.cs.n_padded);
+        const k::EncodeBlob blob{d_data, len, 0, coef};
         k::encode_and_first_tree(ctx->launch(), coef, (size_t)1 << sh.L, sh.L, sh.n, tw.d_tw, tw.ds, eval, sh.N, nullptr, ctx->arena + o_scr, d_root,
-                                 nullptr);
+                                 nullptr, nullptr, 0, &blob);
     }
     FR_HIP(ctx, hipGetLastError());
     return FRIEDA_OK;
@@ -228,8 +228,9 @@
         k::small_encode_and_first_tree(LN, d_data, len, d_stride, sh.L, sh.n, tw.d_tw, tw.ds, nullptr, 0, nullptr, A + o_scr, A + o_root, nullptr,
                                        nullptr, 0);
     } else {
-        k::unpack30(LN, d_data, len, coef, sh.cs.n_padded, d_stride);
-        k::encode_and_first_tree(LN, coef, (size_t)1 << sh.L, sh.L, sh.n, tw.d_tw, tw.ds, eval, sh.N, nullptr, A + o_scr, A + o_root, nullptr);
+        const k::EncodeBlob blob{d_data, len, d_stride, coef};
+        k::encode_and_first_tree(LN, coef, (size_t)1 << sh.L, sh.L, sh.n, tw.d_tw, tw.ds, eval, sh.N, nullptr, A + o_scr, A + o_root, nullptr, nullptr, 0,
+                                 &blob);
     }
     FR_HIP(ctx, hipMemcpy2DAsync(ctx->pinned, 32, A + o_root, bstride, 32, count, hipMemcpyDeviceToHost, s));
     FR_HIP(ctx, hipGetLastError());
@@ -600,7 +601,7 @@
     }
     uint32_t* coef = reinterpret_cast<uint32_t*>(A + o_coef);
     uint32_t* eval = enc ? const_cast<uint32_t*>(enc->eval()) : reinterpret_cast<uint32_t*>(A + first.o_vals);
-    if (!small && !enc) k::unpack30(LN, d_data, len, coef, sh.cs.n_padded, d_data_stride);
+    if (!small && !enc && !dev_channel) k::unpack30(LN, d_data, len, coef, sh.cs.n_padded, d_data_stride);
     ctx->phase_ms[5] = ms_since(t_entry);
 
     for (uint32_t b = 0; b < count; b++) {
@@ -631,9 +632,11 @@
         else if (small)
             k::small_encode_and_first_tree(LN, d_data, len, d_data_stride, sh.L, n, tw.d_tw, tw.ds, eval, N, A + first.o_tree, nullptr, nullptr, d_tr,
                                            reinterpret_cast<const DevTranscript*>(ctx->pinned), tr_host_pitch);
-        else
+        else {
+            const k::EncodeBlob blob{d_data, len, d_data_stride, coef};
             k::encode_and_first_tree(LN, coef, (size_t)1 << sh.L, sh.L, n, tw.d_tw, tw.ds, eval, N, A + first.o_tree, nullptr, nullptr, d_tr,
-                                     reinterpret_cast<const DevTranscript*>(ctx->pinned), tr_host_pitch);
+                                     reinterpret_cast<const DevTranscript*>(ctx->pinned), tr_host_pitch, &blob);
+        }
         const FriLayerDev* cur = &first;
         bool circle = true;
         uint32_t kx = 0;
@@ -1054,8 +1057,9 @@
                                        nullptr, 0);
     } else {
         uint32_t* coef = reinterpret_cast<uint32_t*>(A + o_coef);
-        k::unpack30(LN, d_data, len, coef, sh.cs.n_padded);
-        k::encode_and_first_tree(LN, coef, (size_t)1 << sh.L, sh.L, sh.n, tw.d_tw, tw.ds, eval, sh.N, e->d + e->o_tree, nullptr, e->d + e->o_root, nullptr);
+        const k::EncodeBlob blob{d_data, len, 0, coef};
+        k::encode_and_first_tree(LN, coef, (size_t)1 << sh.L, sh.L, sh.n, tw.d_tw, tw.ds, eval, sh.N, e->d + e->o_tree, nullptr, e->d + e->o_root, nullptr,
+                                 nullptr, 0, &blob);
     }
     FR_HIP(ctx, hipMemcpyAsync(ctx->pinned, e->d + e->o_root, 32, hipMemcpyDeviceToHost, s));
     FR_HIP(ctx, hipStreamSynchronize(s));
diff --git a/frieda_amd/csrc/tree.hip b/frieda_amd/csrc/tree.hip
--- a/frieda_amd/csrc/tree.hip
+++ b/frieda_amd/csrc/tree.hip
@@ -1244,13 +1244,13 @@
 
 void encode_and_first_tree(const Launch& L, const uint32_t* d_coef, size_t coef_stride, uint32_t Lc, uint32_t n, const uint32_t* d_tw,
                            DomainScalars ds, uint32_t* d_eval, size_t eval_stride, uint8_t* d_layers, uint8_t* d_scratch, uint8_t* d_root,
-                           DevTranscript* tr, const DevTranscript* tr_init, size_t tr_init_pitch) {
+                           DevTranscript* tr, const DevTranscript* tr_init, size_t tr_init_pitch, const EncodeBlob* blob) {
     const bool no_fuse = L.tune->no_encode_tree_fusion  || (((size_t)1 << (n > 12 ? n - 12 : 0)) * L.batch < 256) ||
                          (d_layers != nullptr && !L.tune->encode_tree_fusion_prove );
     uint8_t* s0 = d_scratch;
     uint8_t* s1 = d_scratch ? d_scratch + ((size_t)32 << (n > 4 ? n - 4 : 0)) : nullptr;
     EncodeTreeSink sink{d_layers, s0};
-    const uint32_t fused = circle_evaluate_into_tree(L, d_coef, coef_stride, 4, Lc, n, d_tw, ds, d_eval, eval_stride, no_fuse ? nullptr : &sink);
+    const uint32_t fused = circle_evaluate_into_tree(L, d_coef, coef_stride, 4, Lc, n, d_tw, ds, d_eval, eval_stride, no_fuse ? nullptr : &sink, blob);
     if (!fused) {
         TreeArgs a{};
         a.cols = d_eval;
```

Result: no change. 47.84 billion (median of 6 runs) (+0.6%).
